# ParBLiSS/kmerind

Measured on AMD Instinct MI355X. Metric: kmers_per_sec_indexed, higher is better.
Workload: dtype u64

## Files before the change

### kmerind_amd/csrc/kmi_api.hip

```cpp
#include <stdlib.h>

#include <algorithm>

#include "kmi_block.h"
#include <chrono>
#include <mutex>

#include "kmi_internal.h"

namespace kmi {

namespace {
struct CachedBlock { int device; void *p; size_t bytes; };
std::mutex g_cache_mu;
std::vector<CachedBlock> g_cache;
constexpr size_t kCacheMaxBytes = 96ull << 30, kCacheMaxBlocks = 64, kCacheMinBlock = 1ull << 20;
inline uint64_t now_us() { return (uint64_t)std::chrono::duration_cast<std::chrono::microseconds>(std::chrono::steady_clock::now().time_since_epoch()).count(); }
size_t cache_flush(int device) {
  std::lock_guard<std::mutex> lk(g_cache_mu);
  size_t freed = 0;
  for (size_t i = 0; i < g_cache.size();) {
    if (device < 0 || g_cache[i].device == device) { (void)hipFree(g_cache[i].p); freed += g_cache[i].bytes; g_cache.erase(g_cache.begin() + (long)i); }
    else ++i;
  }
// ... 136 lines not shown
        for (int w = 0; w < NW; ++w) k[w] ^= r[w]; }
      const uint64_t h = kmer_hash<NW>(k, shape, which, true, farm_ndebug, ceil_log2_u32(nranks));
      out32[i] = (nranks & (nranks - 1u)) == 0u ? (uint32_t)h & (nranks - 1u) : (uint32_t)(h % nranks);
    }
  }
}

template <int NW, int BITS>
static kmi_status array_op_impl(kmi_ctx *ctx, const kmi_config *cfg, KShape shape, int op, uint32_t which, bool prefix,
                                uint32_t nranks, const uint64_t *in_dev, size_t n, uint64_t *out64, uint32_t *out32) {
  unsigned grid = (unsigned)std::min<size_t>((n + 255) / 256, 2048);
  if (grid == 0) return KMI_OK;
  ProfScope ps(ctx, "kmer_array_op", n);
  hipLaunchKernelGGL((kmer_array_op_kernel<NW, BITS>), dim3(grid), dim3(256), 0, ctx->stream, in_dev, (uint64_t)n, shape, op,
                     which, prefix, cfg->farm_ndebug != 0, cfg->strand, cfg->dist_trans, nranks, out64, out32);
  KMI_HIP(ctx, hipGetLastError());
  return KMI_OK;
}

static kmi_status array_op_dev(kmi_ctx *ctx, const kmi_config *cfg, int op, uint32_t which, bool prefix, uint32_t nranks,
                               const uint64_t *in_dev, size_t n, uint64_t *out64, uint32_t *out32) {
  KShape shape;
  if (!valid_config(cfg, &shape)) return set_err(ctx, KMI_ERR_INVALID, "bad kmi_config");
  KMI_DISPATCH(shape, array_op_impl, ctx, cfg, shape, op, which, prefix, nranks, in_dev, n, out64, out32);
}

static kmi_status array_op_host(kmi_ctx *ctx, const kmi_config *cfg, int op, uint32_t which, bool prefix, uint32_t nranks,
                                const uint64_t *in, size_t n, void *out) {
  if (!ctx) return KMI_ERR_INVALID;
  KShape shape;
  if (!valid_config(cfg, &shape)) return set_err(ctx, KMI_ERR_INVALID, "bad kmi_config");
  if (n == 0) return KMI_OK;
  if (!in || !out) return set_err(ctx, KMI_ERR_INVALID, "null buffer");
  if (op == OP_RANK && nranks == 0) return set_err(ctx, KMI_ERR_INVALID, "nranks must be > 0");
  KMI_HIP(ctx, hipSetDevice(ctx->device));
  const size_t in_bytes = n * shape.n_words * sizeof(uint64_t);
  const size_t out_bytes = (op == OP_RANK) ? n * sizeof(uint32_t) : (op == OP_HASH ? n * sizeof(uint64_t) : in_bytes);
  void *din, *dout;
  KMI_TRY(ws_get(ctx, WS_INPUT, in_bytes, &din));
  KMI_TRY(ws_get(ctx, WS_OUTPUT, out_bytes, &dout));
  KMI_HIP(ctx, hipMemcpyAsync(din, in, in_bytes, hipMemcpyHostToDevice, ctx->stream));
  KMI_TRY(array_op_dev(ctx, cfg, op, which, prefix, nranks, (const uint64_t *)din, n, (uint64_t *)dout, (uint32_t *)dout));
  KMI_HIP(ctx, hipMemcpyAsync(out, dout, out_bytes, hipMemcpyDeviceToHost, ctx->stream));
  KMI_HIP(ctx, hipStreamSynchronize(ctx->stream));
  return KMI_OK;
}

}

using namespace kmi;

extern "C" {

kmi_status kmi_ctx_create(int device, int rank, int nranks, void *stream, kmi_ctx **out) {
  if (!out || nranks <= 0 || rank < 0 || rank >= nranks) return KMI_ERR_INVALID;
  *out = nullptr;
  int ndev = 0;
  if (hipGetDeviceCount(&ndev) != hipSuccess || ndev <= 0 || device < 0 || device >= ndev) return KMI_ERR_DEVICE;
  if (hipSetDevice(device) != hipSuccess) return KMI_ERR_DEVICE;
  kmi_ctx *ctx = new kmi_ctx();
  if (const char *fp = getenv("KMI_FUSED_PATH")) ctx->fused_superkmer = strcmp(fp, "kmer") != 0;
  if (const char *dg = getenv("KMI_SK_DBG")) ctx->sk_dbg = atoi(dg);
  if (const char *dc = getenv("KMI_DIST_CHUNKS")) { ctx->dist_chunks = (uint32_t)atoi(dc); if (ctx->dist_chunks < 1) ctx->dist_chunks = 1; if (ctx->dist_chunks > 64) ctx->dist_chunks = 64; }
  if (const char *sl = getenv("KMI_SK_SLACK")) ctx->sk_slack = atoi(sl) != 0;
  if (const char *tp = getenv("KMI_TUPLES")) ctx->tuples_from_parse = strcmp(tp, "extract") != 0;
  if (const char *ps = getenv("KMI_DIST_POOL_SLACK")) ctx->dist_pool_slack = strtoull(ps, nullptr, 10);
  if (const char *pp = getenv("KMI_DIST_POOL_PCT")) { ctx->dist_pool_pct = (uint32_t)atoi(pp); if (ctx->dist_pool_pct < 1) ctx->dist_pool_pct = 1; }
  if (const char *fr = getenv("KMI_FRONT")) ctx->front_fused = strcmp(fr, "general") != 0;
  if (const char *ho = getenv("KMI_HOST_OVERLAP")) ctx->host_overlap = atoi(ho) != 0;
  if (const char *lp2 = getenv("KMI_LINES_P2")) ctx->lines_p2 = atoi(lp2) != 0;
  if (const char *ds = getenv("KMI_DBG_SUPERKMER")) ctx->dbg_superkmer = atoi(ds) != 0;
  if (const char *hm = getenv("KMI_HOST_OVERLAP_MIN")) ctx->host_overlap_min = strtoull(hm, nullptr, 10);
  if (const char *fc = getenv("KMI_FEED_MIN_CHUNK")) { ctx->feed_min_chunk = strtoull(fc, nullptr, 10); if (ctx->feed_min_chunk < 4096) ctx->feed_min_chunk = 4096; }
  if (const char *mr = getenv("KMI_FRONT_MIN_RANGE")) { ctx->front_min_range = strtoull(mr, nullptr, 10); ctx->front_min_range = (ctx->front_min_range + 4095) / 4096 * 4096; if (!ctx->front_min_range) ctx->front_min_range = 4096; }
  if (const char *rw = getenv("KMI_FRONT_RANGES_PER_WAVE")) { ctx->front_ranges_per_wave = (uint32_t)strtoul(rw, nullptr, 10); if (ctx->front_ranges_per_wave < 1) ctx->front_ranges_per_wave = 1; if (ctx->front_ranges_per_wave > 16) ctx->front_ranges_per_wave = 16; }
  if (const char *mw = getenv("KMI_FRONT_MAX_WAVES")) ctx->front_max_waves = (uint32_t)strtoul(mw, nullptr, 10);
  if (const char *sm = getenv("KMI_SPARSE_MIN")) ctx->sparse_min = strtoull(sm, nullptr, 10);
  if (const char *fd = getenv("KMI_FORCE_DIST")) ctx->force_dist = atoi(fd) != 0;
  if (const char *lc = getenv("KMI_LOOKUP_CAP")) { ctx->lookup_cap = (uint32_t)strtoul(lc, nullptr, 10); if (ctx->lookup_cap < 64) ctx->lookup_cap = 64; }
  if (const char *pb = getenv("KMI_PROFILE_BATCH")) { ctx->profile_batch = strtoull(pb, nullptr, 10); if (ctx->profile_batch < 4096) ctx->profile_batch = 4096; }
  ctx->device = device; ctx->rank = rank; ctx->nranks = nranks; ctx->stream = (hipStream_t)stream;
  if (hipMalloc((void **)&ctx->d_flags, sizeof(uint32_t) * kmi::FLAG_NUM_WORDS) != hipSuccess ||
      hipMalloc((void **)&ctx->d_totals, sizeof(uint64_t) * kmi::TOT_NUM_WORDS) != hipSuccess ||
      hipHostMalloc((void **)&ctx->h_totals, sizeof(uint64_t) * kmi::H_NUM_WORDS, hipHostMallocDefault)    != hipSuccess) {
    delete ctx;
    return KMI_ERR_DEVICE;
  }
  (void)hipMemset(ctx->d_flags, 0, sizeof(uint32_t) * kmi::FLAG_NUM_WORDS);
  {
    hipDeviceProp_t prop;
    if (hipGetDeviceProperties(&prop, device) == hipSuccess && prop.multiProcessorCount > 0) ctx->n_cus = (uint32_t)prop.multiProcessorCount;
  }
  if (upload_quality_lut(ctx) != KMI_OK) { kmi_ctx_destroy(ctx); return KMI_ERR_DEVICE; }
  (void)hipMemset(ctx->d_totals, 0, sizeof(uint64_t) * kmi::TOT_NUM_WORDS);
  *out = ctx;
  return KMI_OK;
}

kmi_status kmi_ctx_reset_hints(kmi_ctx *ctx) {
  if (!ctx) return KMI_ERR_INVALID;
  ctx->sk_level_hint = 0; ctx->sk_inv_dup = 0.f;
  return KMI_OK;
}

kmi_status kmi_ctx_debug_counter(const kmi_ctx *ctx, uint32_t which, uint64_t *value) {
  if (!ctx || !value) return KMI_ERR_INVALID;
  switch (which) {
    case 0: *value = ctx->dist_pool_regrows; return KMI_OK;
    case 1: *value = ctx->alloc_us; return KMI_OK;
    case 2: *value = ctx->alloc_bytes; return KMI_OK;
    case 3: *value = ctx->alloc_calls; return KMI_OK;
    case 4: *value = ctx->alloc_reused; return KMI_OK;
    case 5: *value = ctx->unitig_dist_rounds; return KMI_OK;
    case 6: *value = ctx->unitig_dist_exchanges; return KMI_OK;
    case 7: *value = ctx->unitig_dist_bytes; return KMI_OK;
    case 8: *value = ctx->lookup_npass; return KMI_OK;
    case 9: *value = ctx->retain_fullest; return KMI_OK;
    case 10: *value = ctx->setops_npass; return KMI_OK;
    case 11: *value = (uint64_t)kmi::kSegCopyTile; return KMI_OK;
    case 12: *value = ctx->qd_answered; return KMI_OK;
    case 13: *value = ctx->prune_dist_bytes; return KMI_OK;
    case 14: *value = ctx->tips_dist_exchanges; return KMI_OK;
    case 15: *value = ctx->tips_dist_bytes; return KMI_OK;
    case 16: *value = ctx->bubbles_dist_exchanges; return KMI_OK;
    case 17: *value = ctx->bubbles_dist_bytes; return KMI_OK;
    case 18: *value = ctx->bubbles_dist_stage_exchanges; return KMI_OK;
    case 19: *value = ctx->bubbles_dist_stage_bytes; return KMI_OK;
    default: return KMI_ERR_INVALID;
  }
}

kmi_status kmi_release_cached_memory(int device, uint64_t *bytes_released) {
  const size_t n = cache_flush(device);
  if (bytes_released) *bytes_released = n;
  return KMI_OK;
}

kmi_status kmi_ctx_destroy(kmi_ctx *ctx) {
  if (!ctx) return KMI_OK;
  (void)hipSetDevice(ctx->device);
  (void)hipStreamSynchronize(ctx->stream);
  for (int s = 0; s < WS_NUM_SLOTS; ++s) if (ctx->ws[s].p) dev_retire(ctx, ctx->ws[s].p, ctx->ws[s].cap);
  for (auto &b : ctx->spare) dev_retire(ctx, b.p, b.bytes);
  ctx->spare.clear();
  for (ProfRec &r : ctx->prof_pending) { (void)hipEventDestroy(r.e0); (void)hipEventDestroy(r.e1); }
  for (hipEvent_t e : ctx->event_pool) (void)hipEventDestroy(e);
  if (ctx->d_flags) (void)hipFree(ctx->d_flags);
  if (ctx->d_totals) (void)hipFree(ctx->d_totals);
  if (ctx->ev_mail) (void)hipEventDestroy(ctx->ev_mail);
  for (hipEvent_t e : ctx->feed_ev) if (e) (void)hipEventDestroy(e);
  if (ctx->copy_stream) (void)hipStreamDestroy(ctx->copy_stream);
  if (ctx->h_totals) (void)hipHostFree(ctx->h_totals);
  delete ctx;
  return KMI_OK;
}

const char *kmi_last_error(const kmi_ctx *ctx) { return ctx ? ctx->err.c_str() : "null context"; }

kmi_status kmi_ctx_set_fasta_partition(kmi_ctx *ctx, const kmi_fasta_partition *part) {
  if (!ctx) return KMI_ERR_INVALID;
  if (!part) { ctx->fa_part_set = false; return KMI_OK; }
  if (part->start_state > KMI_FA_SEQUENCE || part->index_shift > 1u) return set_err(ctx, KMI_ERR_INVALID, "bad kmi_fasta_partition");
  ctx->fa_part = *part;
  ctx->fa_part_set = true;
  return KMI_OK;
}

// ... 201 lines not shown
```

### kmerind_amd/csrc/kmi_front.h

```cpp
#pragma once
#include "kmi_front_bytes.h"

namespace kmi {

constexpr int kFrWaves = 4, kFrThreads = kFrWaves * kWave;
constexpr uint32_t kFrRing = 512;
constexpr uint32_t kFrStepLines = 128;
constexpr uint32_t kFrPendEnds = kFrRing - kFrStepLines - 2u, kFrPendPairs = kFrRing / 2u - kFrStepLines;
#ifndef KMI_FR_PASS_RECORDS
#define KMI_FR_PASS_RECORDS 64
#endif
constexpr uint32_t kFrPassRecords = KMI_FR_PASS_RECORDS;
#ifdef KMI_FR_PAIRS_ONLY
constexpr bool kFrEndsOnly = false;
#else
constexpr bool kFrEndsOnly = true;
#endif
constexpr uint32_t kFrRunQ = 256;
constexpr uint32_t kFrStep = 4096;
constexpr uint32_t kFrRowDw = 12;
constexpr uint32_t kFrNone = 0xffu;
constexpr uint32_t kFrOverrun = 256u << 10;

struct FrRange { uint32_t l0, n_lines, n_runs, n_items; };
// ... 569 lines not shown
      const uint4 *rp = reinterpret_cast<const uint4 *>(rows + run * kFrRowDw);
      const uint4 q0 = rp[0], q1 = rp[1], q2 = rp[2];
      uint32_t *row = s_row + threadIdx.x * kFrRowLds;
      row[0] = q0.x; row[1] = q0.y; row[2] = q0.z; row[3] = q0.w; row[4] = q1.x; row[5] = q1.y; row[6] = q1.z; row[7] = q1.w;
      row[8] = q2.x; row[9] = q2.y; row[10] = 0;
      if (edges) s_runx[threadIdx.x] = (uint8_t)q2.w;
      const uint32_t *src = g_items + (q * item_cap + (ri & 0x3ffffffu));
      uint32_t woff = 0;
#pragma unroll
      for (int v4 = 0; v4 < CAP / 4; ++v4) {
        if ((uint32_t)(4 * v4) < cnt) {
          const FrU4 v = *reinterpret_cast<const FrU4 *>(src + 4 * v4);
          const uint32_t it[4] = {v.x, v.y, v.z, v.w};
#pragma unroll
          for (int e = 0; e < 4; ++e)
            if ((uint32_t)(4 * v4 + e) < cnt) {
              const uint32_t n1 = it[e] & 31u, h27 = it[e] >> 5;
              s_items[pre + 4 * v4 + e] = woff | (n1 << 7) | ((h27 >> 7) << 12);
              s_xbits[pre + 4 * v4 + e] = (uint8_t)(h27 & 127u);
              atomicAdd(&s_cnt[h27 >> 19], 1u);
              woff += n1 + 1u;
            }
        }
      }
    }
    s_ibase[threadIdx.x] = pre;
    if (edges) {
      uint32_t wsum = 0;
      for (uint32_t j = 0; j < cnt; ++j) wsum += ((s_items[pre + j] >> 7) & 31u) + 1u;
      s_runw[threadIdx.x] = (uint8_t)wsum;
    }
    lds_barrier();
    uint32_t c = 0, inc = 0;
    if (bl) {
      c = s_cnt[threadIdx.x];
      s_cnt[threadIdx.x] = 0;
      inc = wave_inclusive_sum_dpp(c);
      if (lane_id() == kWave - 1) s_part[wave_id()] = inc;
    }
    lds_barrier();
    if (bl) {
      uint32_t wpre = 0;
#pragma unroll
      for (uint32_t w = 0; w < kNumCoarse / kWave; ++w) wpre += (w < wave_id()) ? s_part[w] : 0u;
      const uint32_t lo = wpre + inc - c;
      s_cur[threadIdx.x] = lo;
      s_gbase[threadIdx.x] = cursor - lo;
      cursor += c;
    }
    lds_barrier();
    for (uint32_t j = 0; j < cnt; ++j) {
      const uint32_t item = s_items[pre + j];
      s_stage[atomicAdd(&s_cur[item >> 24], 1u)] = (uint16_t)((threadIdx.x << 5) | j);
    }
    lds_barrier();
    const uint32_t n_items = pre + cnt;
    const uint32_t round_items = (uint32_t)__builtin_amdgcn_readfirstlane((int)s_cur[kNumCoarse - 1]);
    (void)n_items;
    for (uint32_t s = threadIdx.x; s < round_items; s += NT) {
      const uint32_t e = s_stage[s], rl = e >> 5, j = e & 31u;
      const uint32_t item = s_items[s_ibase[rl] + j];
      const uint32_t h27 = ((item >> 12) << 7) | (uint32_t)s_xbits[s_ibase[rl] + j], n1 = (item >> 7) & 31u;
      const uint32_t hs = ((h27 << lp) & 0x7ffffffu) >> 9;
      uint64_t w0, w1;
      bool flipped = false;
      sk_assemble_row<CANON>(s_row + rl * kFrRowLds, 2u * (item & 127u), k + n1, n1, hs, w0, w1, &flipped);
      if (edges) {
        const uint32_t *row = s_row + rl * kFrRowLds;
        const uint32_t wfirst = item & 127u, after = wfirst + n1 + k;
        auto cc = [&](uint32_t i) -> uint32_t { return (row[i >> 4] >> (2u * (i & 15u))) & 3u; };
        const uint32_t runx = s_runx[rl];
        const uint32_t lc = wfirst ? 1u + (3u - cc(wfirst - 1u)) : (runx & 7u);
        const uint32_t rc = wfirst + n1 + 1u < (uint32_t)s_runw[rl] ? 1u + (3u - cc(after)) : (runx >> 3);
        const uint32_t left = flipped ? (rc ? 5u - rc : 0u) : lc, right = flipped ? (lc ? 5u - lc : 0u) : rc;
        w1 |= ((uint64_t)(left | (right << 3)) << kRecEdgeShift) | ((uint64_t)(flipped ? 1u : 0u) << kRecFlipShift);
      }
      reinterpret_cast<ulonglong2 *>(out)[s_gbase[h27 >> 19] + s] = make_ulonglong2(w0, w1);
    }
    rb += n_taken;
    lds_barrier();
  }
}

__global__ __launch_bounds__(1024) void sk_front_verify_kernel(const FrRange *__restrict__ info, uint32_t n_ranges, uint32_t ranges_per_group,
                                                             uint64_t *__restrict__ group_runs ,
                                                             uint64_t *__restrict__ totals , uint32_t *__restrict__ flags) {
  __shared__ uint64_t s_scan[1024 / 64 + 2];
  __shared__ uint32_t s_bad;
  if (threadIdx.x == 0) s_bad = 0;
  lds_barrier();
  const uint32_t per = (n_ranges + 1023u) / 1024u;
  const uint32_t r_lo = threadIdx.x * per < n_ranges ? threadIdx.x * per : n_ranges, r_hi = r_lo + per < n_ranges ? r_lo + per : n_ranges;
  uint64_t my_lines = 0, my_runs = 0, my_its = 0;
  for (uint32_t r = r_lo; r < r_hi; ++r) {
    const FrRange fr = info[r];
    my_lines += fr.n_lines; my_runs += fr.n_runs; my_its += fr.n_items;
  }
  uint64_t carry = 0, runs = 0, its = 0;
  uint64_t before = block_exclusive_scan<uint64_t>(my_lines, s_scan, &carry);
  for (uint32_t r = r_lo; r < r_hi; ++r) {
    const FrRange fr = info[r];
    if (fr.l0 != kFrNone && fr.n_lines && ((uint32_t)before & 3u) != fr.l0) s_bad = 1;
    before += fr.n_lines;
  }
  (void)block_exclusive_scan<uint64_t>(my_runs, s_scan, &runs);
  (void)block_exclusive_scan<uint64_t>(my_its, s_scan, &its);
  lds_barrier();
  if (threadIdx.x == 0) {
    totals[0] = carry; totals[1] = runs; totals[2] = its;
    if (s_bad) atomicOr(&flags[FLAG_SK_DECLINED], 4u);
  }
  const uint32_t groups = (n_ranges + ranges_per_group - 1) / ranges_per_group;
  for (uint32_t g = threadIdx.x; g < groups; g += blockDim.x) {
    uint64_t s = 0;
    for (uint32_t r = g * ranges_per_group; r < (g + 1) * ranges_per_group && r < n_ranges; ++r) s += info[r].n_runs;
    group_runs[g] = s;
  }
}

}
```

### kmerind_amd/csrc/kmi_index.hip

```cpp
#include <stdlib.h>

#include <algorithm>

#include "kmi_extract.h"
#include "kmi_minimizer.h"
#include <type_traits>

namespace kmi {

constexpr int kFineBits = 15;
constexpr int kNumFine = 1 << kFineBits;
constexpr int kCoarseBits = 8;
constexpr int kNumCoarse = 1 << kCoarseBits;
constexpr int kSubPerCoarse = kNumFine / kNumCoarse;
constexpr int kSlotBits = 32 - kFineBits;
constexpr int kPartThreads = 1024;
constexpr int kPartGroups = 512;
constexpr int kFineParts = 2;
template <int NW> constexpr int fused_groups() { return kPartGroups; }
constexpr int kListGroups = 2048;
constexpr int kLoadBatch = 8;

__host__ __device__ inline uint32_t fine_of(uint32_t h) { return h >> kSlotBits; }
__host__ __device__ inline uint32_t coarse_of(uint32_t h) { return h >> (32 - kCoarseBits); }

template <int RW> struct PartCfg {
  static constexpr int TILE = (RW == 1) ? 8192 : (RW == 2 ? 4096 : (RW <= 4 ? 2048 : 1024));
  static constexpr int CTILE = (RW == 3) ? 3072 : TILE;
  static constexpr int PER_THREAD = TILE / kPartThreads;
};

enum BucketMode { BUCKET_COARSE = 0, BUCKET_SUB = 1, BUCKET_RANK = 2, BUCKET_REC = 3, BUCKET_REC_COARSE = 4 };

struct BucketFn {
  int mode; KShape shape; uint32_t dist_hash; bool farm_ndebug; uint32_t nranks;
  uint32_t sub;
  uint32_t dist_trans = 0;
  uint32_t layout_w = 0;
  uint64_t rank_magic = 0;
  uint32_t owner_w = 0;
};
inline uint64_t rank_magic_of(uint32_t nranks) { return nranks > 1u ? (uint64_t)(((unsigned __int128)1 << 64) / nranks) : 0ull; }
__host__ __device__ inline uint32_t rank_of_hash(uint64_t h, uint32_t nranks, uint64_t magic) {
  if ((nranks & (nranks - 1u)) == 0u) return (uint32_t)h & (nranks - 1u);
#if defined(__HIP_DEVICE_COMPILE__)
  const uint64_t q = __umul64hi(h, magic);
#else
  const uint64_t q = (uint64_t)(((unsigned __int128)h * magic) >> 64);
#endif
  uint64_t r = h - q * nranks;
  r = r >= nranks ? r - nranks : r;
  return (uint32_t)r;
}
inline uint32_t rank_sub_buckets(uint32_t nranks) { uint32_t s = 1; while (s * 2u * nranks <= (uint32_t)kNumCoarse) s *= 2u; return s; }

template <int NW> __device__ __forceinline__ uint32_t fine15_of_key(const uint64_t (&key)[NW], uint32_t layout_w, uint32_t k) {
  if constexpr (NW == 1) {
    if (layout_w) {
      const uint32_t lp = layout_w >> 8;
      return ((sk_key_bucket18(key[0], k, layout_w & 0xffu) << lp) & 0x3ffffu) >> 3;
    }
  }
  return fine_of(place_hash<NW>(key));
}

template <int NW> __device__ __forceinline__ uint32_t bucket_of(const uint64_t (&key)[NW], const BucketFn &f) {
  if (f.mode == BUCKET_RANK) {
    if constexpr (NW == 1) {
      if (f.owner_w) {
        const uint32_t h18 = sk_key_bucket18(key[0], f.shape.k, f.owner_w);
        const uint32_t lp = 31u - (uint32_t)__builtin_clz(f.nranks);
        return (h18 >> (18u - lp)) * f.sub + ((h18 >> 3) & (f.sub - 1u));
      }
    }
    uint64_t t[NW];
#pragma unroll
    for (int w = 0; w < NW; ++w) t[w] = key[w];
    if (f.dist_trans) {
      uint64_t rc[NW];
      if (f.shape.bits == 2) revcomp_words<NW, 2>(key, rc, f.shape); else revcomp_words<NW, 3>(key, rc, f.shape);
      const bool use_rc = f.dist_trans == KMI_DIST_LEX && less_words<NW>(rc, key);
#pragma unroll
      for (int w = 0; w < NW; ++w) t[w] = f.dist_trans == KMI_DIST_XOR ? (key[w] ^ rc[w]) : (use_rc ? rc[w] : key[w]);
    }
    const uint64_t h = kmer_hash<NW>(t, f.shape, f.dist_hash, true, f.farm_ndebug, ceil_log2_u32(f.nranks));
    const uint32_t spread = (uint32_t)((h >> 40) ^ (h >> 13)) * 0x9E3779B1u;
    const uint32_t rank = rank_of_hash(h, f.nranks, f.rank_magic);
    return rank * f.sub + ((spread >> 16) & (f.sub - 1u));
// ... 49 lines not shown
    for (int u = 0; u < U; ++u) {
      if (ok[u]) {
        uint64_t k[NW];
        if (transform) strand_key<NW, BITS>(raw[u], k, shape, strand);
        else {
#pragma unroll
          for (int w = 0; w < NW; ++w) k[w] = raw[u][w];
        }
        atomicAdd(&s_hist[fine15_of_key<NW>(k, layout_w, shape.k)], 1u);
      }
    }
  }
  lds_barrier();
  uint32_t *part_hist = fine_hist + (uint64_t)(blockIdx.x / (gridDim.x / kFineParts)) * kNumFine;
  for (int i = threadIdx.x; i < kNumFine; i += kPartThreads) {
    uint32_t v = s_hist[i];
    if (v) atomicAdd(&part_hist[i], v);
  }
  if (threadIdx.x < kNumCoarse) {
    uint32_t s = 0;
    for (int i = 0; i < kSubPerCoarse; ++i) s += s_hist[threadIdx.x * kSubPerCoarse + ((i + threadIdx.x) & (kSubPerCoarse - 1))];
    wg_hist[(uint64_t)blockIdx.x * kNumCoarse + threadIdx.x] = s;
  }
}

template <int NW, int BITS, int VW = 0>
__global__ __launch_bounds__(kPartThreads) void hist_rank_kernel(const uint64_t *__restrict__ keys, uint64_t n, KShape shape,
                                                                uint32_t strand, BucketFn fn, uint32_t *__restrict__ wg_hist,
                                                                uint32_t in_rw = NW + VW ) {
  __shared__ uint32_t s_hist[kNumCoarse];
  if (threadIdx.x < kNumCoarse) s_hist[threadIdx.x] = 0;
  lds_barrier();
  const uint64_t chunk = part_chunk(n, gridDim.x, PartCfg<NW + VW>::CTILE);
  const uint64_t b = (uint64_t)blockIdx.x * chunk;
  const uint64_t e = (b + chunk < n) ? b + chunk : n;
  for (uint64_t i = b + threadIdx.x; i < e; i += kPartThreads) {
    uint64_t raw[NW], k[NW];
#pragma unroll
    for (int w = 0; w < NW; ++w) raw[w] = keys[i * in_rw + w];
    strand_key<NW, BITS>(raw, k, shape, strand);
    atomicAdd(&s_hist[bucket_of<NW>(k, fn)], 1u);
  }
  lds_barrier();
  if (threadIdx.x < kNumCoarse) wg_hist[(uint64_t)blockIdx.x * kNumCoarse + threadIdx.x] = s_hist[threadIdx.x];
}

__global__ __launch_bounds__(kSubPerCoarse) void fine_totals_kernel(const uint32_t *__restrict__ fine_hist, uint64_t *__restrict__ coarse_tot) {
  __shared__ uint64_t s_scan[kSubPerCoarse / 64 + 2];
  const uint32_t f = blockIdx.x * kSubPerCoarse + threadIdx.x;
  uint64_t v = 0;
#pragma unroll
  for (int h = 0; h < kFineParts; ++h) v += fine_hist[(uint64_t)h * kNumFine + f];
  uint64_t total;
  (void)block_exclusive_scan<uint64_t>(v, s_scan, &total);
  if (threadIdx.x == 0) coarse_tot[blockIdx.x] = total;
}
__global__ __launch_bounds__(kSubPerCoarse) void fine_offsets_spread_kernel(const uint32_t *__restrict__ fine_hist, const uint64_t *__restrict__ coarse_tot,
                                                                           uint64_t *__restrict__ fine_off, uint64_t *__restrict__ part_off,
                                                                           uint64_t *__restrict__ coarse_base) {
  static_assert(kNumCoarse == 2 * kSubPerCoarse, "two coarse totals per thread");
  __shared__ uint64_t s_scan[kSubPerCoarse / 64 + 2];
  const uint32_t c = blockIdx.x, f = c * kSubPerCoarse + threadIdx.x;
  const uint32_t c0 = 2u * threadIdx.x;
  const uint64_t t0 = coarse_tot[c0], t1 = coarse_tot[c0 + 1];
  uint64_t grand;
  (void)block_exclusive_scan<uint64_t>(t0 + t1, s_scan, &grand);
  const uint64_t below = (c0 < c ? t0 : 0ull) + (c0 + 1 < c ? t1 : 0ull);
  uint64_t base;
  (void)block_exclusive_scan<uint64_t>(below, s_scan, &base);
  uint32_t loc[kFineParts];
  uint64_t v = 0;
#pragma unroll
  for (int h = 0; h < kFineParts; ++h) { loc[h] = fine_hist[(uint64_t)h * kNumFine + f]; v += loc[h]; }
  uint64_t off = base + block_exclusive_scan<uint64_t>(v, s_scan, (uint64_t *)nullptr);
  if (threadIdx.x == 0) coarse_base[c] = base;
  fine_off[f] = off;
#pragma unroll
  for (int h = 0; h < kFineParts; ++h) {
    if (part_off) part_off[(uint64_t)h * kNumFine + f] = off;
    off += loc[h];
  }
  if (c == (uint32_t)kNumCoarse - 1 && threadIdx.x == 0) fine_off[kNumFine] = grand;
}
static void launch_fine_offsets(kmi_ctx *ctx, const uint32_t *fine_hist, uint64_t *fine_off, uint64_t *part_off, uint64_t *coarse_base) {
  uint64_t *tot = ctx->d_totals + TOT_COARSE;
  hipLaunchKernelGGL(fine_totals_kernel, dim3(kNumCoarse), dim3(kSubPerCoarse), 0, ctx->stream, fine_hist, tot);
  hipLaunchKernelGGL(fine_offsets_spread_kernel, dim3(kNumCoarse), dim3(kSubPerCoarse), 0, ctx->stream, fine_hist, (const uint64_t *)tot, fine_off, part_off,
                     coarse_base);
}

__global__ __launch_bounds__(256) void coarse_cursors_kernel(const uint32_t *__restrict__ wg_hist, uint32_t groups,
                                                            const uint64_t *__restrict__ coarse_base, uint64_t *__restrict__ wg_off) {
  const uint32_t c = blockIdx.x * (blockDim.x >> 6) + wave_id();
  if (c >= (uint32_t)kNumCoarse) return;
  uint64_t carry = coarse_base[c];
  for (uint32_t w0 = 0; w0 < groups; w0 += kWave) {
    const uint32_t w = w0 + lane_id();
    const uint64_t v = (w < groups) ? wg_hist[(uint64_t)w * kNumCoarse + c] : 0ull;
    const uint64_t inc = wave_inclusive_scan(v);
    if (w < groups) wg_off[(uint64_t)w * kNumCoarse + c] = carry + inc - v;
    carry += __shfl(inc, kWave - 1, kWave);
  }
}

__global__ __launch_bounds__(256) void rank_totals_kernel(const uint32_t *__restrict__ wg_hist, uint32_t groups, uint32_t nbuckets,
                                                         uint64_t *__restrict__ bucket_cnt) {
  const uint32_t c = blockIdx.x * (blockDim.x >> 6) + wave_id();
  if (c >= nbuckets) return;
  uint64_t v = 0;
  for (uint32_t w = lane_id(); w < groups; w += kWave) v += wg_hist[(uint64_t)w * kNumCoarse + c];
  v = wave_reduce_sum(v);
  if (lane_id() == 0) bucket_cnt[c] = v;
}
__global__ __launch_bounds__(256) void rank_bases_kernel(const uint64_t *__restrict__ bucket_cnt, uint32_t nbuckets, uint64_t *__restrict__ base) {
  __shared__ uint64_t s_scan[256 / 64 + 2];
  const uint64_t tot = (threadIdx.x < nbuckets) ? bucket_cnt[threadIdx.x] : 0ull;
  uint64_t total;
  const uint64_t off = block_exclusive_scan<uint64_t>(tot, s_scan, &total);
  base[threadIdx.x] = off;
}
static void launch_rank_offsets(hipStream_t stream, const uint32_t *wg_hist, uint32_t groups, uint32_t nbuckets, uint64_t *bucket_cnt,
                                uint64_t *base , uint64_t *wg_off) {
  hipLaunchKernelGGL(rank_totals_kernel, dim3(kNumCoarse / 4), dim3(256), 0, stream, wg_hist, groups, nbuckets, bucket_cnt);
  hipLaunchKernelGGL(rank_bases_kernel, dim3(1), dim3(256), 0, stream, (const uint64_t *)bucket_cnt, nbuckets, base);
  hipLaunchKernelGGL(coarse_cursors_kernel, dim3(kNumCoarse / 4), dim3(256), 0, stream, wg_hist, groups, (const uint64_t *)base, wg_off);
}

template <int NW, int BITS, int VW = 0, int TILE_ = PartCfg<NW + VW>::TILE>
__device__ __forceinline__ void scatter_range(const uint64_t *__restrict__ in, uint64_t begin, uint64_t end, uint64_t *__restrict__ out,
                                              const KShape &shape, uint32_t strand, bool transform, const BucketFn &fn,
                                              uint64_t cursor ,
                                              uint64_t *s_stage, uint8_t *s_bkt, uint32_t *s_cnt, uint32_t *s_lofs,
                                              uint64_t *s_gbase, uint32_t *s_part, uint64_t *__restrict__ out_vals = nullptr,
                                              const float *__restrict__ in_q = nullptr, const uint64_t *__restrict__ in_v = nullptr) {
  constexpr int RW = NW + VW;
  constexpr int TILE = TILE_;
  constexpr int PT = TILE_ / kPartThreads;
  if (threadIdx.x < kNumCoarse) s_cnt[threadIdx.x] = 0;
  lds_barrier();
  uint64_t raw[PT][RW];
  auto load_tile = [&](uint64_t t0) {
#pragma unroll
    for (int j = 0; j < PT; ++j) {
      uint64_t i = t0 + (uint64_t)j * kPartThreads + threadIdx.x;
      i = (i < end) ? i : end - 1;
      if (VW > 0 && in_v) {
#pragma unroll
        for (int w = 0; w < NW; ++w) raw[j][w] = in[i * NW + w];
        raw[j][NW] = in_v[i];
        if (VW > 1) raw[j][RW - 1] = in_q ? (uint64_t)__float_as_uint(in_q[i]) : 0ull;
      } else if (VW > 0 && in_q) {
#pragma unroll
        for (int w = 0; w < RW - 1; ++w) raw[j][w] = in[i * (RW - 1) + w];
        raw[j][RW - 1] = (uint64_t)__float_as_uint(in_q[i]);
      } else {
#pragma unroll
        for (int w = 0; w < RW; ++w) raw[j][w] = in[i * RW + w];
      }
    }
  };
  load_tile(begin);
  for (uint64_t t0 = begin; t0 < end; t0 += TILE) {
    const uint32_t nt = (uint32_t)((end - t0 < (uint64_t)TILE) ? (end - t0) : (uint64_t)TILE);
    uint64_t k[PT][NW];
    uint64_t v[PT][VW ? VW : 1];
    uint32_t bk[PT], rk[PT];
#pragma unroll
    for (int j = 0; j < PT; ++j) {
      const uint32_t li = j * kPartThreads + threadIdx.x;
      bk[j] = 0xffffffffu;
      if (li < nt) {
        uint64_t kr[NW];
#pragma unroll
        for (int w = 0; w < NW; ++w) kr[w] = raw[j][w];
#pragma unroll
        for (int w = 0; w < VW; ++w) v[j][w] = raw[j][NW + w];
        if (transform) strand_key<NW, BITS>(kr, k[j], shape, strand);
        else {
#pragma unroll
          for (int w = 0; w < NW; ++w) k[j][w] = kr[w];
        }
        if (VW > 0 && fn.mode == BUCKET_REC) bk[j] = (uint32_t)(v[j][0] >> 46) & (uint32_t)(kSubPerCoarse - 1);
        else if (VW > 0 && fn.mode == BUCKET_REC_COARSE) bk[j] = (uint32_t)(v[j][0] >> 53) & (uint32_t)(kNumCoarse - 1);
        else bk[j] = bucket_of<NW>(k[j], fn);
        rk[j] = atomicAdd(&s_cnt[bk[j]], 1u);
      }
    }
    if (t0 + TILE < end) load_tile(t0 + TILE);
    lds_barrier();
    uint32_t c = 0, inc = 0;
    if (threadIdx.x < kNumCoarse) {
      c = s_cnt[threadIdx.x];
      s_cnt[threadIdx.x] = 0;
      inc = wave_inclusive_scan(c);
      if (lane_id() == kWave - 1) s_part[wave_id()] = inc;
    }
    lds_barrier();
    if (threadIdx.x < kNumCoarse) {
      uint32_t pre = 0;
#pragma unroll
      for (uint32_t w = 0; w < kNumCoarse / kWave; ++w) pre += (w < wave_id()) ? s_part[w] : 0u;
      const uint32_t lo = pre + inc - c;
      s_lofs[threadIdx.x] = lo;
      s_gbase[threadIdx.x] = cursor - lo;
      cursor += c;
    }
    lds_barrier();
#pragma unroll
// ... 1694 lines not shown
  const uint32_t b = blockIdx.x;
  const uint64_t nb = new_off[b], ne = new_off[b + 1];
  const uint64_t ob = old_off ? old_off[b] : 0ull, oe = old_off ? old_off[b + 1] : 0ull;
  if (nb == ne && ob == oe) { if (threadIdx.x == 0) out_cnt[b] = 0; return; }
  const uint64_t tmp0 = nb + ob;
  uint32_t *s_out = &s_ctl[4];
  uint32_t npass = 1;
  while (true) {
    if (threadIdx.x == 0) *s_out = 0;
    bool failed = false;
    for (uint32_t pass = 0; pass < npass && !failed; ++pass) {
      table_clear<NW>(tab);
      lds_barrier();
      for_each_key<NW, BatchOf<NW>::U>(old_keys, ob, oe, [&](const uint64_t (&k)[NW], uint64_t i) {
        const uint32_t h = place_hash<NW>(k);
        if (pass_of(h, npass) != pass) return;
        int s = table_upsert<NW>(tab, k, h);
        if (s >= 0) count_add(&tab.vals[s], old_vals[i], sat);
        else if (s == -2) count_add(tab.special, old_vals[i], sat);
      });
      for (uint64_t i = nb + threadIdx.x; i < ne; i += blockDim.x) {
        uint64_t k[NW];
#pragma unroll
        for (int w = 0; w < NW; ++w) k[w] = recs[i * RW + w];
        const uint32_t v = (uint32_t)recs[i * RW + NW];
        const uint32_t h = place_hash<NW>(k);
        if (pass_of(h, npass) != pass) continue;
        int s = table_upsert<NW>(tab, k, h);
        if (s >= 0) count_add(&tab.vals[s], v, sat);
        else if (s == -2) count_add(tab.special, v, sat);
      }
      lds_barrier();
      if (*tab.overflow) { failed = true; break; }
      for (int s = threadIdx.x; s < TabCfg<NW>::SLOTS; s += blockDim.x) {
        const bool used = slot_used<NW>(tab, s);
        const uint32_t pos = wave_alloc(s_out, used);
        if (used) {
#pragma unroll
          for (int w = 0; w < NW; ++w) tmp_keys[(tmp0 + pos) * NW + w] = tab.keys[(uint64_t)s * NW + w];
          tmp_vals[tmp0 + pos] = tab.vals[s];
        }
      }
      lds_barrier();
      if (NW == 1 && threadIdx.x == 0 && *tab.special_set) {
        const uint32_t pos = atomicAdd(s_out, 1u);
        tmp_keys[(tmp0 + pos) * NW] = kEmptyKey;
        tmp_vals[tmp0 + pos] = *tab.special;
      }
      lds_barrier();
    }
    if (!failed) break;
    npass *= 2;
    if (npass > kMaxPasses) { if (threadIdx.x == 0) { atomicOr(&flags[FLAG_PASS_LIMIT], 1u); *s_out = 0; } lds_barrier(); break; }
    lds_barrier();
  }
  if (threadIdx.x == 0) out_cnt[b] = *s_out;
}

template <int NW>
__global__ __launch_bounds__(256) void unzip_pairs_kernel(const uint64_t *__restrict__ recs, uint64_t n, uint64_t *__restrict__ keys,
                                                         uint32_t *__restrict__ vals) {
  constexpr int RW = NW + 1;
  for (uint64_t i = (uint64_t)blockIdx.x * blockDim.x + threadIdx.x; i < n; i += (uint64_t)gridDim.x * blockDim.x) {
#pragma unroll
    for (int w = 0; w < NW; ++w) keys[i * NW + w] = recs[i * RW + w];
    vals[i] = (uint32_t)recs[i * RW + NW];
  }
}

__global__ __launch_bounds__(1024) void bucket_offsets_kernel(const uint32_t *__restrict__ cnt, uint64_t *__restrict__ off,
                                                             uint64_t *__restrict__ totals, int slot) {
  __shared__ uint64_t s_scan[1024 / 64 + 2];
  constexpr int PER = kNumFine / 1024;
  uint64_t loc[PER], sum = 0;
#pragma unroll
  for (int i = 0; i < PER; ++i) { loc[i] = cnt[threadIdx.x * PER + i]; sum += loc[i]; }
  uint64_t total;
  uint64_t o = block_exclusive_scan<uint64_t>(sum, s_scan, &total);
#pragma unroll
  for (int i = 0; i < PER; ++i) { off[threadIdx.x * PER + i] = o; o += loc[i]; }
  if (threadIdx.x == 0) { off[kNumFine] = total; totals[slot] = total; }
}

template <int NW, typename V>
__global__ __launch_bounds__(256) void bucket_compact_kernel(const uint64_t *__restrict__ tmp_keys, const V *__restrict__ tmp_vals,
                                                            const uint64_t *__restrict__ src_off_a, const uint64_t *__restrict__ src_off_b,
                                                            const uint64_t *__restrict__ dst_off, uint64_t *__restrict__ keys,
                                                            V *__restrict__ vals) {
  const uint32_t b = blockIdx.x;
  const uint64_t d0 = dst_off[b], n = dst_off[b + 1] - d0;
  const uint64_t s0 = src_off_a[b] + (src_off_b ? src_off_b[b] : 0ull);
  for (uint64_t i = threadIdx.x; i < n * NW; i += blockDim.x) keys[d0 * NW + i] = tmp_keys[s0 * NW + i];
  for (uint64_t i = threadIdx.x; i < n; i += blockDim.x) vals[d0 + i] = tmp_vals[s0 + i];
}

enum QueryMode { Q_COUNT = 0, Q_FIND = 1, Q_ERASE = 2, Q_HITS = 3  };

template <int NW, int VW>
__global__ __launch_bounds__((QTabCfg<NW>::NT)) void bucket_query_kernel(int mode, const uint64_t *__restrict__ q_keys, const uint64_t *__restrict__ q_off,
                                                                       const uint64_t *__restrict__ idx_keys, const uint32_t *__restrict__ idx_vals32,
                                                                       const uint64_t *__restrict__ idx_mvals,
                                                                       const uint64_t *__restrict__ idx_off, uint64_t *__restrict__ tmp_keys,
                                                                       uint64_t *__restrict__ tmp_vals64, uint32_t *__restrict__ tmp_vals32,
                                                                       uint32_t *__restrict__ out_cnt, uint32_t *__restrict__ flags,
                                                                       bool emit_index, const uint32_t *__restrict__ idx_cnt = nullptr,
                                                                       const uint64_t *__restrict__ out_off = nullptr) {
  KMI_TABLE_LDS_CFG(NW, QTabCfg<NW>)
  constexpr int OW = VW ? VW : 1;
  const uint32_t b = blockIdx.x;
  const uint64_t qb = q_off[b], qe = q_off[b + 1];
  const uint64_t ib = idx_off ? idx_off[b] : 0ull, ie = idx_off ? (idx_cnt ? ib + idx_cnt[b] : idx_off[b + 1]) : 0ull;
  const bool by_entries = (mode == Q_ERASE) || (VW > 0 && mode == Q_FIND);
  const uint64_t tmp0 = out_off ? out_off[b] : (by_entries ? ib : qb);
  uint32_t *s_out = &s_ctl[4];
  auto emit_entry = [&](uint32_t pos, const uint64_t (&k)[NW], uint64_t i) {
#pragma unroll
    for (int w = 0; w < NW; ++w) tmp_keys[(tmp0 + pos) * NW + w] = k[w];
    if constexpr (VW == 0) {
      if (mode == Q_ERASE) tmp_vals32[tmp0 + pos] = idx_vals32[i]; else tmp_vals64[tmp0 + pos] = emit_index ? i : (uint64_t)idx_vals32[i];
    } else {
#pragma unroll
      for (int w = 0; w < VW; ++w) tmp_vals64[(tmp0 + pos) * VW + w] = idx_mvals[i * VW + w];
    }
  };
  {
    uint32_t want = 2u * (uint32_t)((qe - qb) < (uint64_t)QTabCfg<NW>::CAP ? (qe - qb) : (uint64_t)QTabCfg<NW>::CAP);
    want = (want + 255u) & ~255u;
    want = want < 512u ? 512u : want;
    if (want < (uint32_t)QTabCfg<NW>::CAP) { tab.cap = want; tab.slots = want + QTabCfg<NW>::PAD; tab.limit = want * 3u / 4u; }
  }
  if (qb == qe) {
    if (mode == Q_ERASE) {
      for (uint64_t i = ib + threadIdx.x; i < ie; i += blockDim.x) {
        uint64_t k[NW];
#pragma unroll
        for (int w = 0; w < NW; ++w) k[w] = idx_keys[i * NW + w];
        emit_entry((uint32_t)(i - ib), k, i);
      }
      if (threadIdx.x == 0) out_cnt[b] = (uint32_t)(ie - ib);
    } else if (threadIdx.x == 0) out_cnt[b] = 0;
    return;
  }
  uint32_t npass = 1;
  while (true) {
    if (threadIdx.x == 0) *s_out = 0;
    bool failed = false;
    for (uint32_t pass = 0; pass < npass && !failed; ++pass) {
      table_clear<NW>(tab);
      lds_barrier();
      for_each_key<NW, BatchOf<NW>::U>(q_keys, qb, qe, [&](const uint64_t (&k)[NW], uint64_t) {
        const uint32_t h = place_hash<NW>(k);
        if (pass_of(h, npass) != pass) return;
        (void)table_upsert<NW>(tab, k, h);
      });
      lds_barrier();
      if (*tab.overflow) { failed = true; break; }
      for (uint64_t i = ib + threadIdx.x; i < ie; i += blockDim.x) {
        uint64_t k[NW];
#pragma unroll
        for (int w = 0; w < NW; ++w) k[w] = idx_keys[i * NW + w];
        const uint32_t h = place_hash<NW>(k);
        if (pass_of(h, npass) != pass) continue;
        const int s = table_find<NW>(tab, k, h);
        const bool hit = (s >= 0) || (s == -2);
        if (mode == Q_COUNT) {
          if (s >= 0) atomicAdd(&tab.vals[s], 1u); else if (s == -2) atomicAdd(tab.special, 1u);
// ... 122 lines not shown
  uint64_t *part_off;
  uint64_t *coarse_base;
  uint32_t *wg_hist;
  uint64_t *wg_off;
};

static kmi_status get_part_ws(kmi_ctx *ctx, size_t n, int nw, WsSlot slot_a, WsSlot slot_b, PartWs *w) {
  void *p;
  const size_t key_bytes = (n ? n : 1) * nw * sizeof(uint64_t);
  KMI_TRY(ws_get(ctx, slot_a, key_bytes, &p)); w->buf_a = (uint64_t *)p;
  KMI_TRY(ws_get(ctx, slot_b, key_bytes, &p)); w->buf_b = (uint64_t *)p;
  KMI_TRY(ws_get(ctx, WS_HIST, sizeof(uint32_t) * kNumFine * kFineParts + sizeof(uint64_t) * ((kNumFine + 1) * 2 + kNumFine * kFineParts + kNumCoarse) + 256, &p));
  w->fine_hist = (uint32_t *)p;
  uint64_t *off_base = (uint64_t *)((char *)p + sizeof(uint32_t) * kNumFine * kFineParts);
  w->fine_off = off_base + (slot_b == WS_QUERY_B ? (kNumFine + 1) : 0);
  w->part_off = off_base + 2 * (kNumFine + 1);
  w->coarse_base = w->part_off + (uint64_t)kNumFine * kFineParts;
  KMI_TRY(ws_get(ctx, WS_WGHIST, sizeof(uint32_t) * kPartGroups * kNumCoarse, &p)); w->wg_hist = (uint32_t *)p;
  KMI_TRY(ws_get(ctx, WS_CURSOR, sizeof(uint64_t) * kPartGroups * kNumCoarse, &p)); w->wg_off = (uint64_t *)p;
  return KMI_OK;
}

template <int NW, int BITS, int VW = 0>
static kmi_status partition_impl(kmi_ctx *ctx, const kmi_config *cfg, KShape shape, const uint64_t *keys_dev, size_t n, bool transform,
                                 WsSlot slot_a, WsSlot slot_b, Partitioned *out, uint32_t layout_w = 0, uint64_t *split_keys = nullptr,
                                 uint64_t *split_vals = nullptr, const float *in_q = nullptr, const uint64_t *in_v = nullptr) {
  PartWs w;
  KMI_TRY(get_part_ws(ctx, n, NW + VW, slot_a, slot_b, &w));
  KMI_HIP(ctx, hipMemsetAsync(w.fine_hist, 0, sizeof(uint32_t) * kNumFine * kFineParts, ctx->stream));
  {
    ProfScope ps(ctx, "hist_fine", n);
    hipLaunchKernelGGL((hist_fine_kernel<NW, BITS, VW>), dim3(kPartGroups), dim3(kPartThreads), 0, ctx->stream, keys_dev, (uint64_t)n, shape,
                       cfg->strand, transform, w.fine_hist, w.wg_hist, layout_w,
                       (VW > 0 && in_v) ? (uint32_t)NW : (uint32_t)(NW + VW) - ((VW > 0 && in_q) ? 1u : 0u));
  }
  {
    ProfScope ps(ctx, "fine_offsets", kNumFine);
    launch_fine_offsets(ctx, w.fine_hist, w.fine_off, w.part_off, w.coarse_base);
    hipLaunchKernelGGL(coarse_cursors_kernel, dim3(kNumCoarse / 4), dim3(256), 0, ctx->stream, (const uint32_t *)w.wg_hist, (uint32_t)kPartGroups,
                       (const uint64_t *)w.coarse_base, w.wg_off);
  }
  BucketFn fn; fn.mode = BUCKET_COARSE; fn.shape = shape; fn.dist_hash = 0; fn.farm_ndebug = false; fn.nranks = 1; fn.sub = 1; fn.layout_w = layout_w;
  {
    ProfScope ps(ctx, "scatter_coarse", n);
    hipLaunchKernelGGL((scatter_chunks_kernel<NW, BITS, VW>), dim3(kPartGroups), dim3(kPartThreads), 0, ctx->stream, keys_dev, (uint64_t)n, w.buf_a,
                       shape, cfg->strand, transform, fn, w.wg_off, (VW > 0) ? in_q : (const float *)nullptr,
                       (VW > 0) ? in_v : (const uint64_t *)nullptr);
  }
  {
    ProfScope ps(ctx, "scatter_fine", n);
    if (NW == 1 && VW == 0)
      hipLaunchKernelGGL(scatter_fine_lines_kernel, dim3(kNumCoarse * kFineParts), dim3(kPartThreads), 0, ctx->stream, (const uint64_t *)w.buf_a,
                         w.buf_b, (const uint64_t *)w.fine_off, (const uint64_t *)w.part_off, (const uint64_t *)w.wg_off, (uint32_t)kPartGroups,
                         layout_w, shape.k);
    else if (NW + VW <= 4 && ctx->lines_p2)
      hipLaunchKernelGGL((scatter_fine_records_lines_kernel<NW, BITS, VW>), dim3(kNumCoarse * kFineParts), dim3(kPartThreads), 0, ctx->stream,
                         (const uint64_t *)w.buf_a, (VW > 0 && split_keys) ? split_keys : w.buf_b, shape, (const uint64_t *)w.fine_off,
                         (const uint64_t *)w.part_off, (const uint64_t *)w.wg_off, (uint32_t)kPartGroups, layout_w,
                         (VW > 0 && split_keys) ? split_vals : (uint64_t *)nullptr);
    else
      hipLaunchKernelGGL((scatter_fine_kernel<NW, BITS, VW>), dim3(kNumCoarse * kFineParts), dim3(kPartThreads), 0, ctx->stream, w.buf_a,
                         (VW > 0 && split_keys) ? split_keys : w.buf_b, shape, (const uint64_t *)w.fine_off, (const uint64_t *)w.part_off,
                         (const uint64_t *)w.wg_off, (uint32_t)kPartGroups, (int)BUCKET_SUB, layout_w, (VW > 0 && split_keys) ? split_vals : (uint64_t *)nullptr);
  }
  KMI_HIP(ctx, hipGetLastError());
  out->keys = (VW > 0 && split_keys) ? split_keys : w.buf_b; out->fine_off = w.fine_off;
  out->scratch = (NW == 1 && VW == 0) ? w.buf_a : nullptr;
  return KMI_OK;
}

static kmi_status read_total(kmi_ctx *ctx, TotalWord slot, uint64_t *v) {
  uint32_t flag = 0;
  KMI_HIP(ctx, hipMemcpyAsync(ctx->h_totals + slot, ctx->d_totals + slot, sizeof(uint64_t), hipMemcpyDeviceToHost, ctx->stream));
  KMI_HIP(ctx, hipMemcpyAsync(&flag, ctx->d_flags + FLAG_PASS_LIMIT, sizeof(uint32_t), hipMemcpyDeviceToHost, ctx->stream));
  KMI_HIP(ctx, hipStreamSynchronize(ctx->stream));
  *v = ctx->h_totals[slot];
  if (flag) {
    KMI_HIP(ctx, hipMemsetAsync(ctx->d_flags + FLAG_PASS_LIMIT, 0, sizeof(uint32_t), ctx->stream));
    return set_err(ctx, KMI_ERR_OVERFLOW, "a bucket could not be reduced within the pass limit");
  }
  return KMI_OK;
}

template <int NW>
static kmi_status adopt_tmp(kmi_index *idx, const uint64_t *tmp_keys, const uint32_t *tmp_vals, const uint64_t *src_a, const uint64_t *src_b,
                            const uint32_t *out_cnt, bool fastq_verdict = false, uint64_t n_slots = 0, bool allow_sparse = false) {
  kmi_ctx *ctx = idx->ctx;
  uint64_t *new_off = nullptr;
  KMI_HIP(ctx, pool_alloc(ctx, (void **)&new_off, kOffBytes));
  {
    ProfScope ps(ctx, "bucket_offsets", kNumFine);
    hipLaunchKernelGGL(bucket_offsets_kernel, dim3(1), dim3(1024), 0, ctx->stream, out_cnt, new_off, ctx->d_totals, (int)TOT_ENTRIES);
  }
  uint64_t total = 0;
  kmi_status st_total = read_total(ctx, TOT_ENTRIES, &total);
  if (st_total == KMI_OK && fastq_verdict) st_total = fastq_length_verdict(ctx);
  if (st_total != KMI_OK) { pool_free(ctx, new_off, kOffBytes); return st_total; }
  if (n_slots && total == n_slots && !src_b && ctx->ws[WS_TMP_KEYS].p == (const void *)tmp_keys && ctx->ws[WS_TMP_VALS].p == (const void *)tmp_vals) {
    size_t kb0 = 0, vb0 = 0;
    (void)ws_detach(ctx, WS_TMP_KEYS, tmp_keys, &kb0);
    (void)ws_detach(ctx, WS_TMP_VALS, tmp_vals, &vb0);
    KMI_HIP(ctx, hipStreamSynchronize(ctx->stream));
    free_index_arrays(idx);
    idx->keys = const_cast<uint64_t *>(tmp_keys); idx->vals = const_cast<uint32_t *>(tmp_vals); idx->bucket_off = new_off;
    idx->n_entries = total; idx->has_data = true; idx->keys_bytes = kb0; idx->vals_bytes = vb0;
    return KMI_OK;
  }
  bool room = false;
  if (NW == 1 && allow_sparse && n_slots >= ctx->sparse_min) {
    size_t free_b = 0, total_b = 0;
    room = hipMemGetInfo(&free_b, &total_b) == hipSuccess && free_b >= ctx->ws[WS_TMP_KEYS].cap + ctx->ws[WS_TMP_VALS].cap + ((size_t)1 << 30);
  }
  if (NW == 1 && allow_sparse && room && n_slots >= ctx->sparse_min && !src_b && ctx->ws[WS_TMP_KEYS].p == (const void *)tmp_keys &&
      ctx->ws[WS_TMP_VALS].p == (const void *)tmp_vals) {
    uint64_t *off = nullptr; uint32_t *cnt = nullptr;
    hipError_t e1 = pool_alloc(ctx, (void **)&off, kOffBytes);
    hipError_t e2 = pool_alloc(ctx, (void **)&cnt, sizeof(uint32_t) * kNumFine);
    if (e1 == hipSuccess && e2 == hipSuccess) {
      KMI_HIP(ctx, hipMemcpyAsync(off, src_a, kOffBytes, hipMemcpyDeviceToDevice, ctx->stream));
      KMI_HIP(ctx, hipMemcpyAsync(cnt, out_cnt, sizeof(uint32_t) * kNumFine, hipMemcpyDeviceToDevice, ctx->stream));
      size_t kb0 = 0, vb0 = 0;
      (void)ws_detach(ctx, WS_TMP_KEYS, tmp_keys, &kb0);
      (void)ws_detach(ctx, WS_TMP_VALS, tmp_vals, &vb0);
      free_index_arrays(idx);
      idx->keys = const_cast<uint64_t *>(tmp_keys); idx->vals = const_cast<uint32_t *>(tmp_vals); idx->bucket_off = off; idx->bucket_cnt = cnt;
      idx->dense_off = new_off; idx->n_entries = total; idx->has_data = true; idx->keys_bytes = kb0; idx->vals_bytes = vb0;
      return KMI_OK;
    }
    if (off) pool_free(ctx, off, kOffBytes);
    if (cnt) pool_free(ctx, cnt, sizeof(uint32_t) * kNumFine);
  }
  uint64_t *nk = nullptr; uint32_t *nv = nullptr;
  const size_t kb = (total ? total : 1) * NW * sizeof(uint64_t), vb = (total ? total : 1) * sizeof(uint32_t);
  hipError_t e1 = pool_alloc(ctx, (void **)&nk, kb);
  hipError_t e2 = pool_alloc(ctx, (void **)&nv, vb);
  if (e1 != hipSuccess || e2 != hipSuccess) {
    if (nk) pool_free(ctx, nk, kb);
    if (nv) pool_free(ctx, nv, vb);
    pool_free(ctx, new_off, kOffBytes);
    return set_err(ctx, KMI_ERR_NOMEM, "hipMalloc failed for the index arrays");
  }
  {
    ProfScope ps(ctx, "bucket_compact", total);
    hipLaunchKernelGGL((bucket_compact_kernel<NW, uint32_t>), dim3(kNumFine), dim3(256), 0, ctx->stream, tmp_keys, tmp_vals, src_a, src_b,
                       (const uint64_t *)new_off, nk, nv);
  }
  KMI_HIP(ctx, hipGetLastError());
  KMI_HIP(ctx, hipStreamSynchronize(ctx->stream));
  free_index_arrays(idx);
  idx->keys = nk; idx->vals = nv; idx->bucket_off = new_off; idx->n_entries = total; idx->has_data = true;
  idx->keys_bytes = kb; idx->vals_bytes = vb;
  return KMI_OK;
}

template <int NW>
static kmi_status reduce_and_adopt(kmi_index *idx, const Partitioned &part, size_t n, bool fastq_verdict = false) {
  kmi_ctx *ctx = idx->ctx;
  void *p;
  const uint64_t cap = n + idx->n_entries;
  KMI_TRY(ws_get(ctx, WS_TMP_KEYS, cap * NW * sizeof(uint64_t), &p)); uint64_t *tmp_keys = (uint64_t *)p;
  KMI_TRY(ws_get(ctx, WS_TMP_VALS, cap * sizeof(uint32_t), &p)); uint32_t *tmp_vals = (uint32_t *)p;
  KMI_TRY(ws_get(ctx, WS_BUCKET_CNT, sizeof(uint32_t) * kNumFine, &p)); uint32_t *out_cnt = (uint32_t *)p;
  KMI_HIP(ctx, hipMemsetAsync(ctx->d_flags + FLAG_REDUCE_CHECK, 0, sizeof(uint32_t), ctx->stream));
  {
    ProfScope ps(ctx, "bucket_reduce", n);
    hipLaunchKernelGGL((bucket_reduce_kernel<NW>), dim3(kNumFine), dim3(TabCfg<NW>::NT), 0, ctx->stream, (const uint64_t *)part.keys,
                       (const uint64_t *)part.fine_off, (const uint64_t *)idx->keys, (const uint32_t *)idx->vals,
                       (const uint64_t *)(idx->has_data ? idx->bucket_off : nullptr), tmp_keys, tmp_vals, out_cnt, ctx->d_flags,
                       idx->shape.n_bits == 64u * NW, part.scratch, idx->saturating);
  }
  KMI_HIP(ctx, hipGetLastError());
  return adopt_tmp<NW>(idx, tmp_keys, tmp_vals, part.fine_off, idx->has_data ? idx->bucket_off : nullptr, out_cnt, fastq_verdict,
                       idx->has_data ? 0 : (uint64_t)n);
}

template <int NW, int BITS>
static kmi_status insert_impl(kmi_index *idx, const uint64_t *keys_dev, size_t n, bool transform) {
  kmi_ctx *ctx = idx->ctx;
  if (n == 0) return KMI_OK;
  KMI_TRY(ensure_layout(idx, 0u));
  Partitioned part;
  KMI_TRY((partition_impl<NW, BITS>(ctx, &idx->cfg, idx->shape, keys_dev, n, transform, WS_KEYS_A, WS_KEYS_B, &part)));
  return reduce_and_adopt<NW>(idx, part, n);
}

template <int NW, int BITS>
static kmi_status build_fused_impl(kmi_index *idx, const uint8_t *bytes_dev, size_t n_bytes) {
  kmi_ctx *ctx = idx->ctx;
  KMI_TRY(ensure_layout(idx, 0u));
  FastqScan sc;
  KMI_TRY(fastq_scan(ctx, &idx->cfg, bytes_dev, n_bytes, &sc, false));
  const uint64_t n = sc.n_tuples, n_tiles = sc.n_tiles;
  if (n == 0) return KMI_OK;
  PackedInput in; in.eol = sc.pk_eol; in.stream = sc.pk_stream; in.n_bytes = sc.n_bytes; in.n_cover = sc.n_cover; in.n_valid = sc.n_bytes; in.brk = sc.pk_brk;
  const bool split = sc.pk_brk != nullptr;
  const uint32_t *line_base = sc.line_base;
  const bool canonical = idx->cfg.strand != KMI_STRAND_SINGLE;
  PartWs w;
  KMI_TRY(get_part_ws(ctx, n, NW, WS_KEYS_A, WS_KEYS_B, &w));
  void *pl;
  using LPC = ListPassCfg<NW, BITS>;
  KMI_TRY(ws_get(ctx, WS_ENT_LIST, sizeof(uint16_t) * ((size_t)n_tiles * LPC::ent_stride(idx->shape.k, split) + 64), &pl));
  uint16_t *ent = (uint16_t *)pl;
  KMI_TRY(ws_get(ctx, WS_ENT_CNT, sizeof(uint32_t) * (n_tiles + 8), &pl));
  uint32_t *ent_cnt = (uint32_t *)pl;
  KMI_HIP(ctx, hipMemsetAsync(w.fine_hist, 0, sizeof(uint32_t) * kNumFine * kFineParts, ctx->stream));
  {
    ProfScope ps(ctx, "fastq_list", n);
    using LP = ListPassCfg<NW, BITS>;
    const uint32_t wave_lds = LP::wave_lds_bytes(idx->shape.k, split);
    hipLaunchKernelGGL((fastq_list_kernel<NW, BITS>), dim3(kListGroups), dim3(kListThreads), wave_lds * (kListThreads / kWave), ctx->stream, in,
                       n_tiles, idx->shape.k, LP::max_runs(idx->shape.k, split), wave_lds, line_base, ctx->d_flags, ent, ent_cnt,
                       LP::ent_stride(idx->shape.k, split));
  }
// ... 1399 lines not shown
```

### kmerind_amd/csrc/kmi_internal.h

```cpp
#pragma once
#include <hip/hip_runtime.h>
#include <stdint.h>
#include <stdio.h>
#include <string.h>

#include <string>
#include <vector>

#include "../../include/kmerind_hip.h"
#include "kmi_device.h"

namespace kmi {

constexpr int kSegCopyThreads = 256, kSegCopyPerThread = 8, kSegCopyTile = kSegCopyThreads * kSegCopyPerThread;

enum WsSlot {
  WS_TILE_INFO = 0,
  WS_TILE_BASE,
  WS_TILE_OFF,
  WS_KEYS_A,
  WS_KEYS_B,
  WS_HIST,
  WS_WGHIST,
  WS_CURSOR,
// ... 35 lines not shown
  WS_UNI_RANK,
  WS_UNI_NODE,
  WS_UNI_SCAN,
  WS_UNI_STAGE,
  WS_UNI_END,
  WS_UNI_CNT,
  WS_DBG_TIPS,
  WS_DBG_BUBBLES,
  WS_LOOKUP_RECS,
  WS_LOOKUP_CNT,
  WS_SPECTRUM,
  WS_LOCATE_POS,
  WS_LOCATE_SCAN,
  WS_LOCATE_OFF,
  WS_QD_PERM,
  WS_QD_SLOT,
  WS_QD_ANS,
  WS_QD_OFFS,
  WS_QD_VALS,
  WS_QD_RANS,
  WS_QD_ROFFS,
  WS_QD_RVALS,
  WS_NUM_SLOTS
};

enum FlagWord : uint32_t {
  FLAG_PARSE = 0,
  FLAG_OUT_OVERFLOW = 1,
  FLAG_PASS_LIMIT = 2,
  FLAG_ID_OVERFLOW = 3,
  FLAG_REDUCE_CHECK = 8,
  FLAG_SK_DECLINED = 9,
  FLAG_SK_WHY = 10,
  FLAG_FRONT_QUEUE = 12,
  FLAG_SK_LEVEL0 = 16,
  FLAG_SK_LEVEL_END = 34,
  FLAG_SK_ROOM = 34,
  FLAG_LOOKUP_NPASS = 36,
  FLAG_LOOKUP_OVER = 37,
  FLAG_REDUCE_QUEUE = 40,
  FLAG_REDUCE_QUEUE_END = 48,
  FLAG_CLOCKS = 48,
  FLAG_NUM_WORDS = 64,
  FZ_SCAN_0 = 0, FZ_SCAN_1 = 16, FZ_FRONT_0 = 0, FZ_FRONT_1 = 16, FZ_BACK_0 = 16, FZ_BACK_1 = 35, FZ_BACK_2 = 40, FZ_BACK_3 = 48
};
static_assert(FZ_SCAN_0 == FZ_FRONT_0 && FZ_SCAN_1 == FZ_FRONT_1 && FLAG_REDUCE_CHECK < FZ_SCAN_1,
              "a scan and the one-pass front end clear the same per-call words, and nothing of the back end or the lookup (below)");
static_assert(FZ_FRONT_0 <= FLAG_PARSE && FLAG_SK_DECLINED < FZ_FRONT_1 && FLAG_SK_WHY < FZ_FRONT_1 && FLAG_FRONT_QUEUE < FZ_FRONT_1,
              "the front end's launch clears the parse flags, its verdict words and its range queue");
static_assert(FZ_FRONT_1 <= FLAG_SK_LEVEL0, "... and none of the back end's words");
static_assert(FZ_BACK_0 == FLAG_SK_LEVEL0 && FZ_BACK_1 == FLAG_SK_ROOM + 1 && FLAG_SK_LEVEL_END == FLAG_SK_ROOM,
              "the back end's first range: the level votes and the room flag, nothing else");
static_assert(FZ_BACK_1 <= FLAG_LOOKUP_NPASS && FLAG_LOOKUP_OVER == FLAG_LOOKUP_NPASS + 1 && FLAG_LOOKUP_OVER < FZ_BACK_2,
              "the lookup's two words lie together (one fill, one read-back) and outside both ranges");
static_assert(FZ_BACK_2 == FLAG_REDUCE_QUEUE && FZ_BACK_3 == FLAG_REDUCE_QUEUE_END && FLAG_REDUCE_QUEUE_END <= FLAG_CLOCKS,
              "the back end's second range: the queue word and its spare words, not the clocks");
static_assert(FLAG_SK_LEVEL0 + 9 <= FLAG_SK_LEVEL_END && FLAG_CLOCKS + 16 <= FLAG_NUM_WORDS, "the votes and the clocks fit");

enum TotalWord : uint32_t {
  TOT_LINES = 0,
  TOT_FA_CHARS = 0,
  TOT_TUPLES = 1,
  TOT_FA_DROPPED = 1,
  TOT_SEQS = 2,
  TOT_FA_VALID = 3,
  TOT_SCAN_WORDS = 4,
  TOT_ENTRIES = 4,
  TOT_RESULTS = 5,
  TOT_SK_KMERS = 6,
  TOT_UPDATED = 7,
  TOT_BATCH_END = 8,
  TOT_LOCATE_HITS = 9,
  TOT_FRONT = 12,
  TOT_COARSE = 16,
  TOT_NUM_WORDS = 16 + 256
};
static_assert(TOT_FA_VALID + 1 == TOT_SCAN_WORDS && TOT_SCAN_WORDS == TOT_ENTRIES && TOT_ENTRIES + 1 == TOT_RESULTS &&
              TOT_RESULTS + 1 == TOT_SK_KMERS && TOT_SK_KMERS + 1 == TOT_UPDATED && TOT_UPDATED + 1 == TOT_BATCH_END &&
              TOT_BATCH_END + 1 == TOT_LOCATE_HITS && TOT_LOCATE_HITS < TOT_FRONT && TOT_FRONT + 3 <= TOT_COARSE && TOT_COARSE + 256 == TOT_NUM_WORDS,
              "one owner per total word");
enum HostWord : uint32_t {
  H_BATCH_END = 8,
  H_SK_LEVELS = 8,
  H_SK_ROOM = 14,
  H_MAIL = 16,
  H_MAIL_CNT = H_MAIL,
  H_MAIL_DECLINED = H_MAIL + 512,
  H_MAIL_FRONT = H_MAIL + 513,
  H_MAIL_KMERS = H_MAIL + 516,
  H_NUM_WORDS = 16 + 1024
};
static_assert(H_BATCH_END == (uint32_t)TOT_BATCH_END && H_SK_LEVELS > (uint32_t)TOT_RESULTS && H_SK_LEVELS + 5 <= H_SK_ROOM &&
              H_SK_ROOM < H_MAIL && H_MAIL == (uint32_t)TOT_COARSE && H_MAIL_KMERS < H_NUM_WORDS,
              "the read-backs of a build overlap neither each other nor the mirrored totals a build reads (entries, results)");

struct ProfRec {
  const char *name;
  hipEvent_t e0, e1;
  uint64_t units;
};

struct ProfAgg {
  const char *name;
  double total_ms;
  uint64_t launches, units;
};

}

struct kmi_ctx {
  int device = 0, rank = 0, nranks = 1;
  hipStream_t stream = nullptr;
  std::string err;
  struct Buf { void *p = nullptr; size_t cap = 0; } ws[kmi::WS_NUM_SLOTS];
  uint32_t *d_flags = nullptr;
  uint32_t n_cus = 0;
  uint64_t *d_totals = nullptr;
  hipEvent_t ev_mail = nullptr;
  const uint8_t *feed_host = nullptr; uint8_t *feed_dev = nullptr; size_t feed_bytes = 0;
  hipStream_t copy_stream = nullptr;
  hipEvent_t feed_ev[17] = {};
  bool edge_records = false;
  bool dbg_superkmer = true;
  struct { const uint64_t *recs = nullptr, *rec_off = nullptr, *region = nullptr; const uint32_t *cap = nullptr, *cnt = nullptr; bool valid = false; } sk_left;
  bool lines_p2 = true;
  bool host_overlap = true;
  size_t host_overlap_min = (size_t)64 << 20;
  size_t feed_min_chunk = (size_t)8 << 20;
  uint64_t *h_totals = nullptr;
  bool prof = false;
  std::vector<kmi::ProfRec> prof_pending;
  std::vector<kmi::ProfAgg> prof_agg;
  std::vector<hipEvent_t> event_pool;
  struct Spare { void *p; size_t bytes; };
  std::vector<Spare> spare;
  bool fused_superkmer = true;
  bool force_dist = false;
  uint32_t sk_level_hint = 0;
  float sk_inv_dup = 0.f;
  uint64_t alloc_us = 0, alloc_bytes = 0, alloc_calls = 0, alloc_reused = 0;
  uint32_t dist_pool_regrows = 0;
  uint64_t unitig_dist_rounds = 0, unitig_dist_exchanges = 0, unitig_dist_bytes = 0;
  uint32_t dist_pool_pct = 100;
  uint64_t dist_pool_slack = 65536;
  uint32_t dist_chunks = 4;
  bool tuples_from_parse = true;
  bool sk_slack = true;
  bool front_fused = true;
  uint32_t front_waves = 0;
  uint64_t front_min_range = 64ull << 10;
  uint32_t front_ranges_per_wave = 4;
  uint32_t front_max_waves = 0;
  uint64_t sparse_min = 1ull << 26;
  int sk_dbg = 0;
  bool fa_part_set = false;
  kmi_fasta_partition fa_part{};
  uint32_t lookup_cap = 0;
  size_t profile_batch = (size_t)256 << 20;
  uint64_t lookup_npass = 0;
  uint64_t bubbles_dist_exchanges = 0, bubbles_dist_bytes = 0;
  uint64_t bubbles_dist_stage_exchanges = 0, bubbles_dist_stage_bytes = 0;
  uint64_t tips_dist_exchanges = 0, tips_dist_bytes = 0;
  uint64_t prune_dist_bytes = 0;
  uint64_t retain_fullest = 0;
  uint64_t setops_npass = 0;
  uint64_t qd_answered = 0;
  int fa_left_carry = -1;
};

namespace kmi {

hipError_t dev_malloc(kmi_ctx *ctx, void **p, size_t bytes, size_t *got = nullptr);
void dev_free(kmi_ctx *ctx, void *p);
void dev_retire(kmi_ctx *ctx, void *p, size_t bytes);

inline hipError_t pool_alloc(kmi_ctx *ctx, void **p, size_t bytes) {
  if (bytes == 0) bytes = 256;
  for (size_t i = 0; i < ctx->spare.size(); ++i)
    if (ctx->spare[i].bytes == bytes) { *p = ctx->spare[i].p; ctx->spare.erase(ctx->spare.begin() + (long)i); return hipSuccess; }
  hipError_t e = dev_malloc(ctx, p, bytes);
  if (e != hipSuccess && !ctx->spare.empty()) {
    for (auto &b : ctx->spare) dev_free(ctx, b.p);
    ctx->spare.clear();
    e = dev_malloc(ctx, p, bytes);
  }
  return e;
}
inline void pool_free(kmi_ctx *ctx, void *p, size_t bytes) {
  if (!p) return;
  if (bytes == 0) bytes = 256;
  constexpr size_t kMaxSpare = 12;
  if (ctx->spare.size() >= kMaxSpare) {
    size_t m = 0;
    for (size_t i = 1; i < ctx->spare.size(); ++i) if (ctx->spare[i].bytes < ctx->spare[m].bytes) m = i;
    if (ctx->spare[m].bytes >= bytes) { dev_free(ctx, p); return; }
    dev_free(ctx, ctx->spare[m].p);
    ctx->spare.erase(ctx->spare.begin() + (long)m);
  }
  ctx->spare.push_back({p, bytes});
  constexpr size_t kMaxSpareBytes = 32ull << 30;
  size_t total = 0;
  for (const auto &b : ctx->spare) total += b.bytes;
  while (total > kMaxSpareBytes && !ctx->spare.empty()) {
    total -= ctx->spare.front().bytes;
    dev_free(ctx, ctx->spare.front().p);
    ctx->spare.erase(ctx->spare.begin());
  }
}

inline kmi_status set_err(kmi_ctx *ctx, kmi_status st, const char *fmt, const char *a = "", const char *b = "") {
  if (ctx) {
    char buf[512];
// ... 141 lines not shown
```

### kmerind_amd/csrc/kmi_sk_build.h

```cpp
#pragma once

namespace kmi {

template <typename Fn>
static kmi_status sk_dispatch_w(uint32_t w, Fn &&fn) {
  switch (w) {
    case 19: return fn(std::integral_constant<int, 19>{});
    case 13: return fn(std::integral_constant<int, 13>{});
    case 11: return fn(std::integral_constant<int, 11>{});
    default: return fn(std::integral_constant<int, 7>{});
  }
}

enum SkInput { SK_ANY_FORMAT, SK_FASTQ, SK_FASTQ_ONE_PASS };
static uint32_t sk_width_of_shape(const KShape &s) { return (s.n_words == 1 && s.bits == 2) ? sk_window_of(s.k) : 0u; }
static uint32_t sk_width(const kmi_index *idx, SkInput in) {
  const kmi_ctx *ctx = idx->ctx;
  if (idx->val_words != 0 || !ctx->fused_superkmer) return 0u;
  if (in != SK_ANY_FORMAT && idx->cfg.seq_format != KMI_FMT_FASTQ) return 0u;
  if (in == SK_FASTQ_ONE_PASS && !ctx->front_fused) return 0u;
  return sk_width_of_shape(idx->shape);
}
static uint32_t sk_width_of(const kmi_index *idx) { return sk_width(idx, SK_FASTQ); }
static uint32_t preferred_layout(const kmi_index *idx) { return sk_width(idx, SK_ANY_FORMAT); }
static bool sk_rank_count(uint32_t p) { return p == 1u || p == 2u || p == 4u || p == 8u; }

struct SkGroupWs {
  uint32_t *wg_hist;
  uint64_t *wg_off;
  uint64_t *cnt, *base, *cend;
};
static kmi_status sk_group_ws(kmi_ctx *ctx, SkGroupWs *g) {
  void *p;
  KMI_TRY(ws_get(ctx, WS_WGHIST, sizeof(uint32_t) * kPartGroups * kNumCoarse, &p)); g->wg_hist = (uint32_t *)p;
  KMI_TRY(ws_get(ctx, WS_CURSOR, sizeof(uint64_t) * kPartGroups * kNumCoarse, &p)); g->wg_off = (uint64_t *)p;
  KMI_TRY(ws_get(ctx, WS_MISC, sizeof(uint64_t) * kNumCoarse * 3, &p)); g->cnt = (uint64_t *)p; g->base = g->cnt + kNumCoarse; g->cend = g->base + kNumCoarse;
  return KMI_OK;
}

struct SkFront {
  bool ok = false;
  uint64_t *recs = nullptr;
  uint64_t n_records = 0, n_kmers = 0, n_seqs = 0;
  uint64_t h_cnt[kNumCoarse], h_base[kNumCoarse];
  uint64_t *wg_off = nullptr;
};

template <int W>
static kmi_status sk_front_end(kmi_ctx *ctx, const kmi_config *cfg, const KShape &shape, const FastqScan &sc, uint32_t lp, SkFront *f,
                               uint64_t *out = nullptr, size_t out_cap = 0 ,
                               const FastaScan *fa = nullptr ) {
  constexpr int NW = 1, BITS = 2;
  f->ok = false;
  uint64_t n = fa ? 0 : sc.n_tuples;
  const uint64_t n_tiles = fa ? (fa->n_chars + 8191) / 8192 : sc.n_tiles;
  const uint32_t k = shape.k;
  PackedInput in;
  if (fa) { in.eol = fa->pk_break; in.stream = fa->pk_stream; in.n_bytes = fa->n_chars; in.n_cover = fa->n_cover; in.n_valid = fa->n_valid; in.brk = nullptr; }
  else { in.eol = sc.pk_eol; in.stream = sc.pk_stream; in.n_bytes = sc.n_bytes; in.n_cover = sc.n_cover; in.n_valid = sc.n_bytes; in.brk = sc.pk_brk; }
  const bool split = !fa && sc.pk_brk != nullptr;
  const bool canonical = cfg->strand != KMI_STRAND_SINGLE;
  using LP = ListPassCfg<NW, BITS>;
  const uint32_t seg = sk_segment_of((uint32_t)W), ipt = sk_items_per_tile((uint32_t)W) * (fa ? 2u : 1u);
  const uint32_t stride = fa ? 8192u / seg + 72u : LP::run_stride(k, seg, split);
  void *p;
  KMI_TRY(ws_get(ctx, WS_ENT_LIST, sizeof(uint32_t) * ((size_t)n_tiles * stride + 64), &p)); uint32_t *ent = (uint32_t *)p;
  KMI_TRY(ws_get(ctx, WS_ENT_CNT, sizeof(uint32_t) * (n_tiles + 8), &p)); uint32_t *ent_cnt = (uint32_t *)p;
  KMI_TRY(ws_get(ctx, WS_ENT_BKT, sizeof(uint32_t) * ((size_t)n_tiles * stride + 64), &p)); uint32_t *run_items = (uint32_t *)p;
  KMI_TRY(ws_get(ctx, WS_SK_ITEMS, sizeof(uint32_t) * ((size_t)n_tiles * ipt + 64), &p)); uint32_t *items = (uint32_t *)p;
  SkGroupWs g;
  KMI_TRY(sk_group_ws(ctx, &g));
  KMI_HIP(ctx, hipMemsetAsync(ctx->d_flags + FLAG_SK_DECLINED, 0, sizeof(uint32_t), ctx->stream));
  if (fa) {
    ProfScope ps(ctx, "fasta_runs", fa->n_chars);
    KMI_HIP(ctx, hipMemsetAsync(ctx->d_totals + TOT_SK_KMERS, 0, sizeof(uint64_t), ctx->stream));
    hipLaunchKernelGGL(fasta_runs_kernel, dim3(2048), dim3(256), 0, ctx->stream, reinterpret_cast<const uint32_t *>(fa->pk_break), fa->n_chars, fa->n_valid,
                       fa->n_cover, n_tiles, k, seg, ent, ent_cnt, stride, (unsigned long long *)(ctx->d_totals + TOT_SK_KMERS), ctx->d_flags);
  } else {
    ProfScope ps(ctx, "fastq_list", n);
    const uint32_t wave_lds = LP::wave_lds_bytes(k, split);
    hipLaunchKernelGGL((fastq_list_kernel<NW, BITS, true>), dim3(kListGroups), dim3(kListThreads), wave_lds * (kListThreads / kWave), ctx->stream, in,
                       n_tiles, k, LP::max_runs(k, split), wave_lds, sc.line_base, ctx->d_flags, (void *)ent, ent_cnt, stride, seg);
  }
  {
    ProfScope ps(ctx, "sk_minimizer", n);
    hipLaunchKernelGGL((sk_minimizer_kernel<W>), dim3(kPartGroups), dim3(kSkThreads), 0, ctx->stream, in, n_tiles, k, (const uint32_t *)ent,
                       (const uint32_t *)ent_cnt, stride, ipt, items, run_items, g.wg_hist, ctx->d_flags);
  }
  {
    ProfScope ps(ctx, "sk_offsets", kNumCoarse);
    launch_rank_offsets(ctx->stream, (const uint32_t *)g.wg_hist, (uint32_t)kPartGroups, (uint32_t)kNumCoarse, g.cnt, g.base, g.wg_off);
  }
  KMI_HIP(ctx, hipGetLastError());
  uint64_t h_cnt[2 * kNumCoarse];
  uint32_t h_flags[FLAG_SK_DECLINED + 1] = {0};
  KMI_HIP(ctx, hipMemcpyAsync(h_cnt, g.cnt, sizeof(uint64_t) * 2 * kNumCoarse, hipMemcpyDeviceToHost, ctx->stream));
  KMI_HIP(ctx, hipMemcpyAsync(h_flags, ctx->d_flags, sizeof(h_flags), hipMemcpyDeviceToHost, ctx->stream));
  if (fa) KMI_HIP(ctx, hipMemcpyAsync(&n, ctx->d_totals + TOT_SK_KMERS, sizeof(uint64_t), hipMemcpyDeviceToHost, ctx->stream));
  KMI_HIP(ctx, hipStreamSynchronize(ctx->stream));
  if (!fa && (h_flags[FLAG_PARSE] & 4u)) return fastq_length_verdict(ctx);
  const uint32_t h_flag = h_flags[FLAG_SK_DECLINED];
  if (h_flag) return KMI_OK;
  uint64_t R = 0;
  for (int c = 0; c < kNumCoarse; ++c) { R += h_cnt[c]; f->h_cnt[c] = h_cnt[c]; f->h_base[c] = h_cnt[kNumCoarse + c]; }
  uint64_t *rec_a = out;
  if (!out || R + 64 > out_cap) { KMI_TRY(ws_get(ctx, WS_KEYS_A, (R + 64) * 16, &p)); rec_a = (uint64_t *)p; }
  {
    ProfScope ps(ctx, "sk_scatter", n);
#define KMI_SK_SCATTER(CANON)                                                                                                          \
    hipLaunchKernelGGL(sk_scatter_kernel<CANON>, dim3(kPartGroups), dim3(kSkThreads), 0, ctx->stream, in, n_tiles, k, (const uint32_t *)ent, \
                       (const uint32_t *)ent_cnt, stride, ipt, (const uint32_t *)items, (const uint32_t *)run_items, (const uint64_t *)g.wg_off, rec_a, lp)
    if (canonical) KMI_SK_SCATTER(true); else KMI_SK_SCATTER(false);
#undef KMI_SK_SCATTER
  }
  KMI_HIP(ctx, hipGetLastError());
  f->ok = true; f->recs = rec_a; f->n_records = R; f->n_kmers = n; f->wg_off = g.wg_off;
  return KMI_OK;
}

static kmi_status feed_flush(kmi_ctx *ctx) {
  if (!ctx->feed_host) return KMI_OK;
  const uint8_t *h = ctx->feed_host;
  ctx->feed_host = nullptr;
  KMI_HIP(ctx, hipMemcpyAsync(ctx->feed_dev, h, ctx->feed_bytes, hipMemcpyHostToDevice, ctx->stream));
  return KMI_OK;
}

static void sk_front_report_clocks(kmi_ctx *ctx) {
#ifdef KMI_FR_TIMING
  unsigned long long t[8];
  hipStreamSynchronize(ctx->stream);
  hipMemcpy(t, ctx->d_flags + FLAG_CLOCKS, sizeof(t), hipMemcpyDeviceToHost);
  fprintf(stderr, "sk_front wave clocks: wait-bytes %llu  eol %llu  lines %llu  load+pack %llu  walk %llu  final %llu  copy-out %llu  rest %llu\n", t[0], t[1], t[2], t[3], t[4], t[5], t[6], t[7]);
  hipMemset(ctx->d_flags + FLAG_CLOCKS, 0, sizeof(t));
#endif
}
static void sk_front_report_leave(kmi_ctx *ctx, bool fed, uint32_t front_launched_waves) {
#ifdef KMI_FR_LEAVE
  hipStreamSynchronize(ctx->stream);
  if (fed) return;
  const uint32_t nw = std::min<uint32_t>(front_launched_waves, kFrTimingWaves);
  std::vector<unsigned long long> wc(2 * (size_t)nw);
  hipMemcpyFromSymbol(wc.data(), HIP_SYMBOL(g_fr_wave_clock), sizeof(unsigned long long) * wc.size());
  unsigned long long first = ~0ull;
  for (uint32_t i = 0; i < nw; ++i) first = std::min(first, wc[2 * i]);
  std::vector<double> leave(nw);
  double by_simd[kFrWaves] = {0}, by_third[3] = {0}, enter_third[3] = {0}; uint32_t n_third[3] = {0};
  for (uint32_t i = 0; i < nw; ++i) {
    leave[i] = (double)(wc[2 * i + 1] - first) * 0.01;
    by_simd[i % kFrWaves] += leave[i] / (nw / kFrWaves);
    const uint32_t th = (uint32_t)((uint64_t)i * 3u / nw);
    by_third[th] += leave[i]; enter_third[th] += (double)(wc[2 * i] - first) * 0.01; ++n_third[th];
  }
  std::vector<double> so(leave);
  std::sort(so.begin(), so.end());
  double mean = 0; for (double v : so) mean += v / nw;
  fprintf(stderr, "sk_front wavefronts leave (us after the first entry): n %u  min %.1f  median %.1f  mean %.1f  max %.1f  | by SIMD %.1f %.1f %.1f %.1f"
                  "  | by workgroup third: leave %.1f %.1f %.1f  enter %.1f %.1f %.1f\n", nw, so[0], so[nw / 2], mean, so[nw - 1], by_simd[0], by_simd[1],
          by_simd[2], by_simd[3], by_third[0] / n_third[0], by_third[1] / n_third[1], by_third[2] / n_third[2], enter_third[0] / n_third[0],
          enter_third[1] / n_third[1], enter_third[2] / n_third[2]);
#endif
}
static void sk_front_report_decline(kmi_ctx *ctx) {
  if (!getenv("KMI_FRONT_DEBUG")) return;
  uint32_t why = 0;
  (void)hipMemcpy(&why, ctx->d_flags + FLAG_SK_WHY, sizeof(why), hipMemcpyDeviceToHost);
  fprintf(stderr, "sk_front declined: reasons 0x%x (2 first byte, 4 crowded lines, 8 inference, 16 marker / length, 32 run queue, 64 run capacity, 128 items per run, 256 item capacity, 512 / 1024 edge records: a read of several runs / a base that is not A C G T; 0 = the chain of line indices)\n", why);
}

template <int W>
static kmi_status sk_front_fast(kmi_ctx *ctx, const kmi_config *cfg, const KShape &shape, const uint8_t *bytes_dev, size_t n_bytes, uint32_t lp, SkFront *f,
                                bool *took, uint64_t *out = nullptr, size_t out_cap = 0) {
  *took = false;
  f->ok = false;
  const bool fed = ctx->feed_host != nullptr && bytes_dev == ctx->feed_dev && n_bytes == ctx->feed_bytes;
  if (!fed) KMI_TRY(feed_flush(ctx));
  if (!ctx->front_fused || cfg->seq_format != KMI_FMT_FASTQ || cfg->seq_filter != KMI_SEQ_ALL || n_bytes < 64) return feed_flush(ctx);
  const uint32_t k = shape.k;
  const bool canonical = cfg->strand != KMI_STRAND_SINGLE;
  if (!ctx->front_waves) {
    int per_cu = 0;
    if (hipOccupancyMaxActiveBlocksPerMultiprocessor(&per_cu, sk_front_kernel<19, false>, kFrThreads, 0) != hipSuccess || per_cu <= 0) per_cu = 2;
    ctx->front_waves = (uint32_t)per_cu * (ctx->n_cus ? ctx->n_cus : 256u) * (uint32_t)kFrWaves;
  }
  const uint32_t per_wave = fed ? 16u : ctx->front_ranges_per_wave;
  uint64_t range_bytes = (n_bytes + (uint64_t)ctx->front_waves * per_wave - 1) / ((uint64_t)ctx->front_waves * per_wave);
  range_bytes = (range_bytes + kFrStep - 1) / kFrStep * kFrStep;
  if (range_bytes < ctx->front_min_range) range_bytes = ctx->front_min_range;
  if (range_bytes > (8ull << 20)) range_bytes = 8ull << 20;
  const uint64_t n_ranges64 = (n_bytes + range_bytes - 1) / range_bytes;
  const uint32_t rpg = (uint32_t)((n_ranges64 + kPartGroups - 1) / kPartGroups);
  if (rpg > kFrMaxGroupRanges) return feed_flush(ctx);
  const uint32_t n_ranges = (uint32_t)n_ranges64;
  const uint32_t run_cap = (uint32_t)(range_bytes / 64) + 64u, item_cap = (uint32_t)(range_bytes / 8) + 64u;
  void *p;
  KMI_TRY(ws_get(ctx, WS_TILE_INFO, sizeof(FrRange) * (n_ranges + 1), &p)); FrRange *info = (FrRange *)p;
  KMI_TRY(ws_get(ctx, WS_TILE_BASE, sizeof(uint64_t) * (kPartGroups + 1), &p)); uint64_t *group_runs = (uint64_t *)p;
  KMI_TRY(ws_get(ctx, WS_ENT_LIST, sizeof(uint32_t) * ((size_t)n_ranges * run_cap + 64), &p)); uint32_t *run_items = (uint32_t *)p;
  KMI_TRY(ws_get(ctx, WS_PK_STREAM, sizeof(uint32_t) * kFrRowDw * ((size_t)n_ranges * run_cap + 64), &p)); uint32_t *rows = (uint32_t *)p;
  KMI_TRY(ws_get(ctx, WS_SK_ITEMS, sizeof(uint32_t) * ((size_t)n_ranges * item_cap + 64), &p)); uint32_t *items = (uint32_t *)p;
  SkGroupWs g;
  KMI_TRY(sk_group_ws(ctx, &g));
  hipLaunchKernelGGL(sk_zero_kernel, dim3(128), dim3(1024), 0, ctx->stream, g.wg_hist, (uint32_t)(kPartGroups * kNumCoarse),
                     reinterpret_cast<uint32_t *>(ctx->d_totals + TOT_SK_KMERS), 2u, (uint32_t *)nullptr, 0u, ctx->d_flags, (uint32_t)FZ_FRONT_0,
                     (uint32_t)FZ_FRONT_1, 0u, 0u);
  auto launch_front = [&](uint32_t wgs, uint32_t r0, uint32_t r1, uint32_t *queue) {
#define KMI_SK_FRONT(EDGES)                                                                                                            \
    hipLaunchKernelGGL((sk_front_kernel<W, EDGES>), dim3(wgs), dim3(kFrThreads), 0, ctx->stream, bytes_dev, (uint64_t)n_bytes, range_bytes, n_ranges, k, \
                       is_rna(cfg), run_cap, item_cap, rpg, info, run_items, rows, items, g.wg_hist, (unsigned long long *)(ctx->d_totals + TOT_SK_KMERS),  \
                       ctx->d_flags, r0, r1, queue)
    if (ctx->edge_records) KMI_SK_FRONT(true); else KMI_SK_FRONT(false);
#undef KMI_SK_FRONT
  };
  uint32_t front_launched_waves = 0;
  if (!fed) {
    ProfScope ps(ctx, "sk_front", n_bytes);
    uint32_t waves = ctx->front_max_waves ? std::min(ctx->front_waves, ctx->front_max_waves) : ctx->front_waves;
    waves = std::max<uint32_t>((uint32_t)kFrWaves, waves / (uint32_t)kFrWaves * (uint32_t)kFrWaves);
    const uint32_t wgs = std::min((n_ranges + kFrWaves - 1) / kFrWaves, waves / (uint32_t)kFrWaves);
    front_launched_waves = wgs * (uint32_t)kFrWaves;
    launch_front(wgs, 0u, 0xffffffffu, ctx->d_flags + FLAG_FRONT_QUEUE);
  } else {
    ProfScope ps(ctx, "sk_front_fed", n_bytes);
    const uint8_t *host = ctx->feed_host;
    ctx->feed_host = nullptr;
    constexpr size_t kMaxChunks = sizeof(ctx->feed_ev) / sizeof(ctx->feed_ev[0]) - 1;
    size_t cut[kMaxChunks + 1];
    size_t n_chunks = 0;
    {
      size_t ratio = 16;
      if (const char *e = getenv("KMI_FEED_RATIO")) { const long v = atol(e); if (v >= 2 && v <= 64) ratio = (size_t)v; }
      size_t at = 0;
      cut[0] = 0;
      while (n_chunks + 1 < kMaxChunks && n_bytes - at > ctx->feed_min_chunk) {
        size_t len = (n_bytes - at) - (n_bytes - at) / ratio;
        len = len / 4096 * 4096;
        at += len; cut[++n_chunks] = at;
      }
      cut[++n_chunks] = n_bytes;
    }
    if (!ctx->copy_stream) KMI_HIP(ctx, hipStreamCreateWithFlags(&ctx->copy_stream, hipStreamNonBlocking));
    for (size_t c = 0; c <= n_chunks; ++c) if (!ctx->feed_ev[c]) KMI_HIP(ctx, hipEventCreateWithFlags(&ctx->feed_ev[c], hipEventDisableTiming));
    KMI_HIP(ctx, hipEventRecord(ctx->feed_ev[n_chunks], ctx->stream));
    KMI_HIP(ctx, hipStreamWaitEvent(ctx->copy_stream, ctx->feed_ev[n_chunks], 0));
    for (size_t c = 0; c < n_chunks; ++c) {
      KMI_HIP(ctx, hipMemcpyAsync(const_cast<uint8_t *>(bytes_dev) + cut[c], host + cut[c], cut[c + 1] - cut[c], hipMemcpyHostToDevice, ctx->copy_stream));
      KMI_HIP(ctx, hipEventRecord(ctx->feed_ev[c], ctx->copy_stream));
    }
    const uint64_t margin = (uint64_t)kFrOverrun + 3ull * kFrStep;
    uint32_t r_done = 0;
    for (size_t c = 0; c < n_chunks; ++c) {
      KMI_HIP(ctx, hipStreamWaitEvent(ctx->stream, ctx->feed_ev[c], 0));
      const uint64_t arrived = cut[c + 1];
      uint32_t r_end = n_ranges;
      if (c + 1 < n_chunks) r_end = arrived > margin + range_bytes ? (uint32_t)((arrived - margin) / range_bytes) : 0u;
      if (r_end > n_ranges) r_end = n_ranges;
      if (r_end <= r_done) continue;
      launch_front((r_end - r_done + kFrWaves - 1) / kFrWaves, r_done, r_end, nullptr);
      r_done = r_end;
    }
  }
  {
    ProfScope ps(ctx, "sk_offsets", kNumCoarse);
    sk_front_report_clocks(ctx);
    sk_front_report_leave(ctx, fed, front_launched_waves);
    hipLaunchKernelGGL(sk_front_verify_kernel, dim3(1), dim3(1024), 0, ctx->stream, (const FrRange *)info, n_ranges, rpg, group_runs, ctx->d_totals + TOT_FRONT, ctx->d_flags);
    launch_rank_offsets(ctx->stream, (const uint32_t *)g.wg_hist, (uint32_t)kPartGroups, (uint32_t)kNumCoarse, g.cnt, g.base, g.wg_off);
  }
  KMI_HIP(ctx, hipGetLastError());
  const uint64_t r_bound = (uint64_t)n_ranges * item_cap;
  bool early = !out && n_bytes <= (8ull << 30);
  uint64_t *rec_a = out;
  if (early) {
    if (ws_get(ctx, WS_KEYS_A, (r_bound + 64) * 16, &p) == KMI_OK) rec_a = (uint64_t *)p; else { early = false; ctx->err.clear(); }
  }
  auto launch_scatter = [&]() {
    ProfScope ps(ctx, "sk_scatter", n_bytes);
#define KMI_SK_SCATTER_ROWS(CANON)                                                                                                     \
    hipLaunchKernelGGL(sk_scatter_rows_kernel<CANON>, dim3(kPartGroups), dim3(kFrScThreads), 0, ctx->stream, (const FrRange *)info, n_ranges, rpg, run_cap, \
                       item_cap, k, (const uint32_t *)run_items, (const uint32_t *)rows, (const uint32_t *)items, (const uint64_t *)g.wg_off, rec_a, lp,         \
                       (const uint32_t *)ctx->d_flags, ctx->edge_records ? 1u : 0u)
    if (canonical) KMI_SK_SCATTER_ROWS(true); else KMI_SK_SCATTER_ROWS(false);
#undef KMI_SK_SCATTER_ROWS
  };
  static_assert(H_MAIL_DECLINED == H_MAIL_CNT + 2 * kNumCoarse, "the mailbox holds the counts and starts of kNumCoarse groups");
  uint64_t *const h = ctx->h_totals;
  const uint64_t *const h_cnt = h + H_MAIL_CNT, *const h_tot = h + H_MAIL_FRONT;
  KMI_HIP(ctx, hipMemcpyAsync(h + H_MAIL_CNT, g.cnt, sizeof(uint64_t) * 2 * kNumCoarse, hipMemcpyDeviceToHost, ctx->stream));
  KMI_HIP(ctx, hipMemcpyAsync(h + H_MAIL_DECLINED, ctx->d_flags + FLAG_SK_DECLINED, sizeof(uint32_t), hipMemcpyDeviceToHost, ctx->stream));
  KMI_HIP(ctx, hipMemcpyAsync(h + H_MAIL_FRONT, ctx->d_totals + TOT_FRONT, sizeof(uint64_t) * 3, hipMemcpyDeviceToHost, ctx->stream));
  KMI_HIP(ctx, hipMemcpyAsync(h + H_MAIL_KMERS, ctx->d_totals + TOT_SK_KMERS, sizeof(uint64_t), hipMemcpyDeviceToHost, ctx->stream));
  if (early) {
    if (!ctx->ev_mail) KMI_HIP(ctx, hipEventCreateWithFlags(&ctx->ev_mail, hipEventDisableTiming));
    KMI_HIP(ctx, hipEventRecord(ctx->ev_mail, ctx->stream));
    launch_scatter();
    KMI_HIP(ctx, hipEventSynchronize(ctx->ev_mail));
  } else {
    KMI_HIP(ctx, hipStreamSynchronize(ctx->stream));
  }
  const uint32_t h_flag = *reinterpret_cast<const uint32_t *>(h + H_MAIL_DECLINED);
  const uint64_t n = h[H_MAIL_KMERS];
  if (h_flag) {
    sk_front_report_decline(ctx);
    static_assert(FLAG_SK_WHY == FLAG_SK_DECLINED + 1, "cleared together");
    KMI_HIP(ctx, hipMemsetAsync(ctx->d_flags + FLAG_SK_DECLINED, 0, 2 * sizeof(uint32_t), ctx->stream));
    return KMI_OK;
  }
  *took = true;
  uint64_t R = 0;
  for (int c = 0; c < kNumCoarse; ++c) { R += h_cnt[c]; f->h_cnt[c] = h_cnt[c]; f->h_base[c] = h_cnt[kNumCoarse + c]; }
  f->n_records = R; f->n_kmers = n; f->wg_off = g.wg_off; f->recs = nullptr; f->n_seqs = (h_tot[0] + 2) / 4;
  if (n == 0) { f->ok = true; return KMI_OK; }
  if (!early) {
    if (!out || R + 64 > out_cap) { KMI_TRY(ws_get(ctx, WS_KEYS_A, (R + 64) * 16, &p)); rec_a = (uint64_t *)p; }
    launch_scatter();
  }
  KMI_HIP(ctx, hipGetLastError());
  f->ok = true; f->recs = rec_a;
  return KMI_OK;
}

enum SkDoor { SK_RECORDS, SK_NO_KMERS, SK_NOT_THIS_PATH };
template <int W>
static kmi_status sk_front_door(kmi_ctx *ctx, const kmi_config *cfg, const KShape &shape, const uint8_t *bytes_dev, size_t n_bytes, uint32_t lp, SkFront *f,
                                SkDoor *door, uint64_t *out = nullptr, size_t out_cap = 0) {
  *door = SK_NOT_THIS_PATH;
  bool took = false;
  KMI_TRY((sk_front_fast<W>(ctx, cfg, shape, bytes_dev, n_bytes, lp, f, &took, out, out_cap)));
  if (took && f->ok) { *door = f->n_kmers ? SK_RECORDS : SK_NO_KMERS; return KMI_OK; }
  if (ctx->edge_records) return KMI_OK;
  FastqScan sc;
  KMI_TRY(align_input(ctx, &bytes_dev, n_bytes));
  KMI_TRY(fastq_scan(ctx, cfg, bytes_dev, n_bytes, &sc, false));
  if (sc.n_tuples == 0) { *door = SK_NO_KMERS; return fastq_length_verdict(ctx); }
  KMI_TRY((sk_front_end<W>(ctx, cfg, shape, sc, lp, f, out, out_cap)));
  if (f->ok) *door = SK_RECORDS;
  return KMI_OK;
}

static void sk_reduce_report_clocks(kmi_ctx *ctx) {
#ifdef KMI_SK_TIMING
  unsigned long long t[8];
  hipStreamSynchronize(ctx->stream);
  hipMemcpy(t, ctx->d_flags + FLAG_CLOCKS, sizeof(t), hipMemcpyDeviceToHost);
  fprintf(stderr, "sk_reduce wave clocks: A-T1 %llu  A-direct %llu  A-wait %llu  B-work %llu  B-wait %llu  emit %llu  between %llu\n", t[0], t[1], t[2], t[3], t[4], t[5], t[6]);
  hipMemset(ctx->d_flags + FLAG_CLOCKS, 0, sizeof(t));
#endif
}
static void sk_slack_report(const uint32_t *fine_cnt, const uint64_t *h_cnt, const uint32_t *h_cap, uint32_t lp, uint64_t R) {
  if (!getenv("KMI_SLACK_DEBUG")) return;
  std::vector<uint32_t> fc(kNumFine);
  (void)hipMemcpy(fc.data(), fine_cnt, sizeof(uint32_t) * kNumFine, hipMemcpyDeviceToHost);
  double worst = 0; uint32_t over = 0;
  for (int f = 0; f < kNumFine; ++f) {
    const double mean = (double)h_cnt[f / kSubPerCoarse] / kSubPerCoarse;
    if (mean > 0 && fc[f] / mean > worst) worst = fc[f] / mean;
    over += fc[f] > h_cap[f / kSubPerCoarse];
  }
  fprintf(stderr, "fine buckets with room: %u of %d outgrew it, the fullest holds %.3f x its coarse bucket's mean (lp %u, %llu records)\n", over,
          (int)kNumFine, worst, lp, (unsigned long long)R);
}

template <int W>
static kmi_status sk_back_end(kmi_index *idx, const uint64_t *rec_a, uint64_t R, const uint64_t *h_cnt, const uint64_t *h_base, const uint64_t *wg_off,
                              uint64_t n, uint32_t lp, bool exact = false) {
  constexpr int NW = 1;
  kmi_ctx *ctx = idx->ctx;
  const bool slack = !exact && ctx->sk_slack && (!idx->has_data || idx->n_entries == 0) && R >= 4096;
  ctx->sk_left.valid = false;
  const uint32_t k = idx->shape.k;
  const bool canonical = idx->cfg.strand != KMI_STRAND_SINGLE;
  void *p;
  SkGroupWs g;
  KMI_TRY(sk_group_ws(ctx, &g));
  uint64_t *const cend = g.cend;
  KMI_TRY(ws_get(ctx, WS_HIST, sizeof(uint32_t) * kNumFine * kFineParts + sizeof(uint64_t) * ((kNumFine + 1) * 2 + kNumFine * kFineParts + kNumCoarse) + 256, &p));
  uint32_t *fine_hist = (uint32_t *)p;
  uint64_t *fine_off = (uint64_t *)((char *)p + sizeof(uint32_t) * kNumFine * kFineParts);
  uint64_t *part_off = fine_off + 2 * (kNumFine + 1);
  uint64_t *coarse_base = part_off + (uint64_t)kNumFine * kFineParts;
  uint64_t h_end[kNumCoarse];
  for (int c = 0; c < kNumCoarse; ++c) h_end[c] = h_base[c] + h_cnt[c];
  KMI_HIP(ctx, hipMemcpyAsync(cend, h_end, sizeof(h_end), hipMemcpyHostToDevice, ctx->stream));
  const uint32_t m_len = idx->shape.k - (uint32_t)W + 1u;
  const uint64_t room_m = m_len <= 11u ? 26u : (m_len == 12u ? 18u : 14u);
  static const uint64_t room_lp[4] = {8, 10, 12, 15};
  const uint64_t room_x64 = room_m * room_lp[lp < 4u ? lp : 3u];
  uint64_t h_region[kNumCoarse], total_b = 0;
  uint32_t h_cap[kNumCoarse];
  for (int c = 0; c < kNumCoarse; ++c) {
    const uint64_t cap = ((h_cnt[c] * room_x64 / 64 + kSubPerCoarse - 1) / kSubPerCoarse + 64 + 7) / 8 * 8;
    h_cap[c] = (uint32_t)cap; h_region[c] = total_b; total_b += cap * kSubPerCoarse;
  }
  KMI_TRY(ws_get(ctx, WS_KEYS_B, ((slack ? total_b : R) + 64) * 16, &p)); uint64_t *rec_b = (uint64_t *)p;
  KMI_TRY(ws_get(ctx, WS_SPLIT_OFF, sizeof(uint32_t) * kNumFine * kFineParts + sizeof(uint64_t) * ((kNumFine + 1) + kNumFine * kFineParts + kNumCoarse) + 256, &p));
  uint32_t *fine_kmers = (uint32_t *)p;
  uint64_t *kmer_off = (uint64_t *)((char *)p + sizeof(uint32_t) * kNumFine * kFineParts);
  uint64_t *k_part = kmer_off + (kNumFine + 1), *k_base = k_part + (uint64_t)kNumFine * kFineParts;
  uint64_t *d_region = nullptr; uint32_t *d_cap = nullptr, *fine_cnt = nullptr;
  if (slack) {
    KMI_TRY(ws_get(ctx, WS_BUCKET_OFF, sizeof(uint64_t) * kNumCoarse + sizeof(uint32_t) * kNumCoarse + 64, &p));
    d_region = (uint64_t *)p; d_cap = (uint32_t *)(d_region + kNumCoarse);
    fine_cnt = fine_hist;
    KMI_HIP(ctx, hipMemcpyAsync(d_region, h_region, sizeof(h_region), hipMemcpyHostToDevice, ctx->stream));
    KMI_HIP(ctx, hipMemcpyAsync(d_cap, h_cap, sizeof(h_cap), hipMemcpyHostToDevice, ctx->stream));
    hipLaunchKernelGGL(sk_zero_kernel, dim3(96), dim3(1024), 0, ctx->stream, fine_cnt, (uint32_t)kNumFine, fine_kmers, (uint32_t)(kNumFine * kFineParts),
                       (uint32_t *)nullptr, 0u, ctx->d_flags, (uint32_t)FZ_BACK_0, (uint32_t)FZ_BACK_1, (uint32_t)FZ_BACK_2, (uint32_t)FZ_BACK_3);
    {
      ProfScope ps(ctx, "sk_scatter_fine", R);
      hipLaunchKernelGGL(sk_scatter_fine_slack_lines_kernel, dim3(kNumCoarse * kFineParts), dim3(kPartThreads), 0, ctx->stream, (const uint64_t *)rec_a, rec_b,
                         (const uint64_t *)wg_off, (const uint64_t *)cend, (uint32_t)kPartGroups, (const uint64_t *)d_region, (const uint32_t *)d_cap,
                         fine_cnt, fine_kmers, ctx->d_flags);
    }
    {
      ProfScope ps(ctx, "fine_offsets", kNumFine);
      launch_fine_offsets(ctx, fine_kmers, kmer_off, k_part, k_base);
    }
  } else {
    {
      ProfScope ps(ctx, "sk_fine_count", R);
      hipLaunchKernelGGL(sk_fine_count_kernel, dim3(kNumCoarse * kFineParts), dim3(1024), 0, ctx->stream, (const uint64_t *)rec_a,
                         (const uint64_t *)wg_off, (const uint64_t *)cend, (uint32_t)kPartGroups, fine_hist, fine_kmers);
    }
    {
      ProfScope ps(ctx, "fine_offsets", kNumFine);
      launch_fine_offsets(ctx, fine_hist, fine_off, part_off, coarse_base);
      launch_fine_offsets(ctx, fine_kmers, kmer_off, k_part, k_base);
    }
    {
      ProfScope ps(ctx, "sk_scatter_fine", R);
      hipLaunchKernelGGL((scatter_fine_kernel<1, 2, 1>), dim3(kNumCoarse * kFineParts), dim3(kPartThreads), 0, ctx->stream, (const uint64_t *)rec_a,
                         rec_b, idx->shape, (const uint64_t *)fine_off, (const uint64_t *)part_off, (const uint64_t *)wg_off,
                         (uint32_t)kPartGroups, (int)BUCKET_REC, 0u);
    }
  }
  KMI_TRY(ws_get(ctx, WS_TMP_KEYS, (n + 64) * sizeof(uint64_t), &p)); uint64_t *tmp_keys = (uint64_t *)p;
  KMI_TRY(ws_get(ctx, WS_TMP_VALS, (n + 64) * sizeof(uint32_t), &p)); uint32_t *tmp_vals = (uint32_t *)p;
  KMI_TRY(ws_get(ctx, WS_BUCKET_CNT, sizeof(uint32_t) * kNumFine, &p)); uint32_t *out_cnt = (uint32_t *)p;
  if (!slack) KMI_HIP(ctx, hipMemsetAsync(ctx->d_flags + FLAG_SK_LEVEL0, 0, sizeof(uint32_t) * (FLAG_SK_LEVEL_END - FLAG_SK_LEVEL0), ctx->stream));
  {
    const uint32_t nmax = sk_nmax_of(k);
    uint32_t *queue = ctx->d_flags + FLAG_REDUCE_QUEUE;
    if (!slack) KMI_HIP(ctx, hipMemsetAsync(queue, 0, sizeof(uint32_t) * (FLAG_REDUCE_QUEUE_END - FLAG_REDUCE_QUEUE), ctx->stream));
#ifndef KMI_SK_WGS_PER_CU
#define KMI_SK_WGS_PER_CU 1
#endif
    const uint32_t wgs = (ctx->n_cus ? ctx->n_cus : 256u) * KMI_SK_WGS_PER_CU;
    ProfScope ps(ctx, "sk_reduce", n);
#define KMI_SK_REDUCE(CANON, OWN, SPECIAL)                                                                                               \
    hipLaunchKernelGGL((sk_reduce_kernel<CANON, OWN, SPECIAL>), dim3(wgs), dim3(KMI_SK_NT), 0, ctx->stream, (const uint64_t *)rec_b,        \
                       (const uint64_t *)fine_off, k, (const uint64_t *)kmer_off, tmp_keys, tmp_vals, out_cnt, ctx->d_flags, queue, (uint32_t)kNumFine, \
                       ctx->sk_level_hint, lp, ctx->sk_inv_dup, (const uint64_t *)d_region, (const uint32_t *)d_cap, (const uint32_t *)fine_cnt)
    if (k == 32u) { if (canonical) KMI_SK_REDUCE(true, 64 * 21, true); else KMI_SK_REDUCE(false, 64 * 21, true); }
    else if (nmax <= 21u) { if (canonical) KMI_SK_REDUCE(true, 64 * 21, false); else KMI_SK_REDUCE(false, 64 * 21, false); }
    else if (nmax <= 24u) { if (canonical) KMI_SK_REDUCE(true, 64 * 24, false); else KMI_SK_REDUCE(false, 64 * 24, false); }
    else { if (canonical) KMI_SK_REDUCE(true, 64 * 32, false); else KMI_SK_REDUCE(false, 64 * 32, false); }
#undef KMI_SK_REDUCE
  }
  KMI_HIP(ctx, hipGetLastError());
  sk_reduce_report_clocks(ctx);
  if (slack) KMI_HIP(ctx, hipMemcpyAsync(ctx->h_totals + H_SK_ROOM, ctx->d_flags + FLAG_SK_ROOM, sizeof(uint32_t), hipMemcpyDeviceToHost, ctx->stream));
  KMI_HIP(ctx, hipMemcpyAsync(ctx->h_totals + H_SK_LEVELS , ctx->d_flags + FLAG_SK_LEVEL0, sizeof(uint32_t) * 9, hipMemcpyDeviceToHost, ctx->stream));
  auto read_levels = [&]() {
    const uint32_t *lv = reinterpret_cast<const uint32_t *>(ctx->h_totals + H_SK_LEVELS);
    uint64_t seen = 0; uint32_t best = 0;
    for (uint32_t l = 0; l < 9; ++l) { seen += lv[l]; if (lv[l] > lv[best]) best = l; }
    if (seen == 0) ctx->sk_level_hint = 0;
    else if (ctx->sk_level_hint == 0) { uint64_t up = seen; ctx->sk_level_hint = (up * 2 > (uint64_t)kNumFine) ? best : 0u; }
    else ctx->sk_level_hint = best;
  };
  const uint32_t layout = (uint32_t)W | (lp << 8);
  if (!idx->has_data || idx->n_entries == 0) {
    KMI_TRY((adopt_tmp<NW>(idx, tmp_keys, tmp_vals, kmer_off, nullptr, out_cnt, false, n, true)));
    if (slack) sk_slack_report(fine_cnt, h_cnt, h_cap, lp, R);
    if (slack && *reinterpret_cast<const uint32_t *>(ctx->h_totals + H_SK_ROOM)) {
      KMI_TRY(kmi_index_clear(idx));
      return sk_back_end<W>(idx, rec_a, R, h_cnt, h_base, wg_off, n, lp, true);
    }
    read_levels();
    idx->layout_w = layout;
    if (n) ctx->sk_inv_dup = (float)((double)idx->n_entries / (double)n);
    ctx->sk_left.recs = rec_b; ctx->sk_left.rec_off = slack ? nullptr : fine_off; ctx->sk_left.region = d_region; ctx->sk_left.cap = d_cap;
    ctx->sk_left.cnt = fine_cnt; ctx->sk_left.valid = true;
    return KMI_OK;
  }
  kmi_index scratch;
  scratch.ctx = ctx; scratch.cfg = idx->cfg; scratch.shape = idx->shape; scratch.val_words = 0; scratch.saturating = idx->saturating;
  kmi_status st = adopt_tmp<NW>(&scratch, tmp_keys, tmp_vals, kmer_off, nullptr, out_cnt);
  if (st == KMI_OK) read_levels();
  if (st == KMI_OK && n) ctx->sk_inv_dup = (float)((double)scratch.n_entries / (double)n);
  if (st == KMI_OK && scratch.n_entries) {
    st = ws_get(ctx, WS_OUTPUT, (scratch.n_entries + 64) * 2 * sizeof(uint64_t), &p);
    if (st == KMI_OK) {
      hipLaunchKernelGGL((zip_pairs_kernel<NW>), dim3(2048), dim3(256), 0, ctx->stream, (const uint64_t *)scratch.keys, (const uint32_t *)scratch.vals,
                         scratch.n_entries, (uint64_t *)p);
      st = index_insert_pairs(idx, (const uint64_t *)p, (size_t)scratch.n_entries, false, true);
    }
  }
  (void)hipStreamSynchronize(ctx->stream);
  free_index_arrays(&scratch);
  return st;
}
static kmi_status sk_back(kmi_index *idx, uint32_t w, const SkFront &f, uint32_t lp) {
  return sk_dispatch_w(w, [&](auto W) { return sk_back_end<W>(idx, f.recs, f.n_records, f.h_cnt, f.h_base, f.wg_off, f.n_kmers, lp); });
}

static kmi_status index_build_fused(kmi_index *idx, const uint8_t *bytes_dev, size_t n_bytes) {
  if (const uint32_t w = sk_width(idx, SK_FASTQ)) {
    SkFront f;
    SkDoor door;
    KMI_TRY(sk_dispatch_w(w, [&](auto W) { return sk_front_door<W>(idx->ctx, &idx->cfg, idx->shape, bytes_dev, n_bytes, 0u, &f, &door); }));
    if (door == SK_RECORDS) return sk_back(idx, w, f, 0u);
    if (door == SK_NO_KMERS) return KMI_OK;
  }
  KMI_DISPATCH(idx->shape, build_fused_impl, idx, bytes_dev, n_bytes);
}

static kmi_status sk_build_fasta(kmi_index *idx, uint32_t w, const FastaScan &fa, bool *done) {
  *done = false;
  SkFront f;
  FastqScan none{};
  KMI_TRY(sk_dispatch_w(w, [&](auto W) { return sk_front_end<W>(idx->ctx, &idx->cfg, idx->shape, none, 0u, &f, nullptr, 0, &fa); }));
  if (!f.ok) return KMI_OK;
  *done = true;
  if (f.n_records == 0) return KMI_OK;
  return sk_back(idx, w, f, 0u);
}

static kmi_status sk_produce(kmi_index *idx, uint32_t w, const uint8_t *bytes_dev, size_t n_bytes, uint32_t nranks, const uint64_t **recs_out, uint64_t *n_records,
                             uint64_t *send_counts, int *produced, uint64_t *out, size_t out_cap) {
  *produced = 0; *recs_out = nullptr; *n_records = 0;
  for (uint32_t r = 0; r < nranks; ++r) send_counts[r] = 0;
  if (n_bytes == 0) { *produced = 1; return KMI_OK; }
  const uint32_t lp = 31u - (uint32_t)__builtin_clz(nranks);
  SkFront f;
  SkDoor door;
  KMI_TRY(sk_dispatch_w(w, [&](auto W) { return sk_front_door<W>(idx->ctx, &idx->cfg, idx->shape, bytes_dev, n_bytes, lp, &f, &door, out, out_cap); }));
  if (door != SK_RECORDS) { *produced = door == SK_NO_KMERS; return KMI_OK; }
  const uint32_t per = (uint32_t)kNumCoarse / nranks;
  for (uint32_t c = 0; c < (uint32_t)kNumCoarse; ++c) send_counts[c / per] += f.h_cnt[c];
  *recs_out = f.recs; *n_records = f.n_records; *produced = 1;
  return KMI_OK;
}

static kmi_status sk_consume(kmi_index *idx, uint32_t w, const uint64_t *recs_dev, uint64_t R, uint32_t nranks) {
  kmi_ctx *ctx = idx->ctx;
  const uint32_t lp = 31u - (uint32_t)__builtin_clz(nranks);
  if (R == 0) { idx->owner_lp = lp; return KMI_OK; }
  void *p;
  SkGroupWs g;
  KMI_TRY(sk_group_ws(ctx, &g));
  KMI_TRY(ws_get(ctx, WS_KEYS_A, (R + 64) * 16, &p)); uint64_t *rec_a = (uint64_t *)p;
  KMI_HIP(ctx, hipMemsetAsync(ctx->d_totals + TOT_SK_KMERS, 0, sizeof(uint64_t), ctx->stream));
  {
    ProfScope ps(ctx, "sk_recv_hist", R);
    hipLaunchKernelGGL(sk_recv_hist_kernel, dim3(kPartGroups), dim3(kPartThreads), 0, ctx->stream, recs_dev, R, g.wg_hist,
                       (unsigned long long *)(ctx->d_totals + TOT_SK_KMERS));
  }
  {
    ProfScope ps(ctx, "sk_offsets", kNumCoarse);
    launch_rank_offsets(ctx->stream, (const uint32_t *)g.wg_hist, (uint32_t)kPartGroups, (uint32_t)kNumCoarse, g.cnt, g.base, g.wg_off);
  }
  BucketFn fn; fn.mode = BUCKET_REC_COARSE; fn.shape = idx->shape; fn.dist_hash = 0; fn.farm_ndebug = false; fn.nranks = 1; fn.sub = 1;
  {
    ProfScope ps(ctx, "sk_recv_scatter", R);
    hipLaunchKernelGGL((scatter_chunks_kernel<1, 2, 1>), dim3(kPartGroups), dim3(kPartThreads), 0, ctx->stream, recs_dev, R, rec_a, idx->shape, 0u, false, fn,
                       (const uint64_t *)g.wg_off);
  }
  KMI_HIP(ctx, hipGetLastError());
  uint64_t h[2 * kNumCoarse], n_kmers = 0;
  KMI_HIP(ctx, hipMemcpyAsync(h, g.cnt, sizeof(h), hipMemcpyDeviceToHost, ctx->stream));
  KMI_HIP(ctx, hipMemcpyAsync(&n_kmers, ctx->d_totals + TOT_SK_KMERS, sizeof(uint64_t), hipMemcpyDeviceToHost, ctx->stream));
  KMI_HIP(ctx, hipStreamSynchronize(ctx->stream));
  KMI_TRY(sk_dispatch_w(w, [&](auto W) { return sk_back_end<W>(idx, rec_a, R, h, h + kNumCoarse, g.wg_off, n_kmers, lp); }));
  idx->owner_lp = lp;
  return KMI_OK;
}

}
```

### kmerind_amd/csrc/kmi_superkmer.h

```cpp
#pragma once

namespace kmi {

constexpr int kRecNShift = 38, kRecHashShift = 43;
constexpr uint64_t kSkPadW1 = ~0ull;
constexpr int kRecEdgeShift = 32, kRecFlipShift = 61;
constexpr uint32_t kSkEdgeWindows = 3;
__device__ __forceinline__ uint32_t rec_hash18(uint64_t w1) { return (uint32_t)(w1 >> kRecHashShift) & 0x3ffffu; }
__device__ __forceinline__ uint32_t rec_fine_sub(uint64_t w1) { return (rec_hash18(w1) >> 3) & 127u; }

constexpr int kSkThreads = 512;
constexpr int kSkRoundTiles = 24;
constexpr int kSkListCap = 32;

struct SkRound {
  uint64_t t; uint32_t ei, total; uint32_t eo[kSkRoundTiles + 1]; uint64_t nt; uint32_t nei;
};
__device__ __forceinline__ bool sk_plan(const uint32_t *__restrict__ ent_cnt, uint64_t te, uint64_t t, uint32_t ei, SkRound &r) {
  while (t < te && ei >= ent_cnt[t]) { ++t; ei = 0; }
  if (t >= te) return false;
  r.t = t; r.ei = ei; r.eo[0] = 0;
  r.nt = t + kSkRoundTiles; r.nei = 0;
  bool cut = false;
#pragma unroll
  for (int i = 0; i < kSkRoundTiles; ++i) {
    uint32_t avail = (t + i < te) ? ent_cnt[t + i] : 0u;
    if (i == 0) avail -= ei;
    uint32_t take = avail;
    if (r.eo[i] + take > (uint32_t)kSkThreads) take = (uint32_t)kSkThreads - r.eo[i];
    if (cut) take = 0;
    if (!cut && take < avail) { cut = true; r.nt = t + i; r.nei = (i == 0 ? ei : 0u) + take; }
    r.eo[i + 1] = r.eo[i] + take;
  }
  r.total = r.eo[kSkRoundTiles];
  return true;
}
__device__ __forceinline__ void sk_locate(const SkRound &r, uint32_t e, uint32_t ent_stride, uint32_t &tr, uint64_t &idx) {
  tr = 0;
#pragma unroll
  for (int i = 1; i < kSkRoundTiles; ++i) tr += (e >= r.eo[i]) ? 1u : 0u;
  uint32_t base = 0;
#pragma unroll
  for (int i = 1; i < kSkRoundTiles; ++i) base = (tr == (uint32_t)i) ? r.eo[i] : base;
  idx = (r.t + tr) * ent_stride + (tr == 0u ? r.ei : 0u) + (e - base);
}
struct SkWin { uint32_t r0, r1, r2, sh; };
__device__ __forceinline__ SkWin sk_fetch(const uint32_t *__restrict__ st, uint64_t last_dw, uint64_t ip) {
  uint64_t d = ip >> 4;
  d = d < last_dw ? d : last_dw;
  SkWin w;
  w.r0 = st[d]; w.r1 = st[d + 1]; w.r2 = st[d + 2]; w.sh = (uint32_t)(ip & 15u) * 2u;
  return w;
}
__device__ __forceinline__ uint32_t sk_lo(const SkWin &w) { return __builtin_amdgcn_alignbit(w.r1, w.r0, w.sh); }
__device__ __forceinline__ uint32_t sk_hi(const SkWin &w) { return __builtin_amdgcn_alignbit(w.r2, w.r1, w.sh); }

__global__ __launch_bounds__(256) void fasta_runs_kernel(const uint32_t *__restrict__ brk, uint64_t n_chars, uint64_t n_valid, uint64_t n_cover,
                                                        uint64_t n_tiles, uint32_t k, uint32_t seg, uint32_t *__restrict__ ent,
                                                        uint32_t *__restrict__ ent_cnt, uint32_t stride, unsigned long long *__restrict__ n_windows,
                                                        uint32_t *__restrict__ flags) {
  const uint32_t lane = lane_id();
  const uint64_t n_words = n_cover / 32;
  const uint64_t n_waves = (uint64_t)gridDim.x * (blockDim.x / kWave);
  for (uint64_t t = (uint64_t)blockIdx.x * (blockDim.x / kWave) + wave_id(); t < n_tiles; t += n_waves) {
    const uint64_t p0 = t * 8192ull + (uint64_t)lane * 128ull;
    uint64_t x[3];
    {
      uint32_t w[7];
      const uint64_t w0 = p0 >> 5;
#pragma unroll
      for (int i = 0; i < 7; ++i) w[i] = (w0 + i < n_words) ? brk[w0 + i] : 0u;
#pragma unroll
      for (int j = 0; j < 3; ++j) {
        const uint64_t lo = (uint64_t)w[2 * j] | ((uint64_t)w[2 * j + 1] << 32), hi = (uint64_t)w[2 * j + 2];
        x[j] = (lo >> 1) | (hi << 63);
      }
    }
    smear_right<3>(x, k - 1u);
    uint64_t v0 = ~x[0], v1 = ~x[1];
    {
      const uint64_t lim_a = n_chars >= k ? n_chars - k + 1u : 0u, lim = lim_a < n_valid ? lim_a : n_valid;
      const uint64_t room = lim > p0 ? lim - p0 : 0u;
      v0 &= room >= 64 ? ~0ull : ((1ull << room) - 1ull);
// ... 269 lines not shown
      d0 = d0 + 16 <= last_dw + 16 ? d0 : 0;
      const uint4 q0 = *reinterpret_cast<const uint4 *>(st + d0), q1 = *reinterpret_cast<const uint4 *>(st + d0 + 4),
                  q2 = *reinterpret_cast<const uint4 *>(st + d0 + 8), q3 = *reinterpret_cast<const uint4 *>(st + d0 + 12);
      uint32_t *row = s_row + threadIdx.x * kSkRowDw;
      row[0] = q0.x; row[1] = q0.y; row[2] = q0.z; row[3] = q0.w; row[4] = q1.x; row[5] = q1.y; row[6] = q1.z; row[7] = q1.w;
      row[8] = q2.x; row[9] = q2.y; row[10] = q2.z; row[11] = q2.w; row[12] = q3.x; row[13] = q3.y; row[14] = q3.z; row[15] = q3.w;
      row[16] = 0;
      s_bit0[threadIdx.x] = (uint32_t)(ip0 - d0 * 16) * 2u;
      s_ioff[threadIdx.x] = ri & 0x3ffffffu;
    }
#pragma unroll
    for (int j = 0; j < CAP; ++j)
      if ((uint32_t)j < cnt) atomicAdd(&s_cnt[(it[j] >> 22) & 255u], 1u);
    lds_barrier();
    uint32_t c = 0, inc = 0;
    if (threadIdx.x < kNumCoarse) {
      c = s_cnt[threadIdx.x];
      s_cnt[threadIdx.x] = 0;
      inc = wave_inclusive_sum_dpp(c);
      if (lane_id() == kWave - 1) s_part[wave_id()] = inc;
    }
    lds_barrier();
    if (threadIdx.x < kNumCoarse) {
      uint32_t pre = 0;
#pragma unroll
      for (uint32_t w = 0; w < kNumCoarse / kWave; ++w) pre += (w < wave_id()) ? s_part[w] : 0u;
      const uint32_t lo = pre + inc - c;
      s_cur[threadIdx.x] = lo;
      s_gbase[threadIdx.x] = cursor - lo;
      cursor += c;
      if (threadIdx.x == kNumCoarse - 1) s_total = pre + inc;
    }
    lds_barrier();
#pragma unroll
    for (int j = 0; j < CAP; ++j)
      if ((uint32_t)j < cnt) s_stage[atomicAdd(&s_cur[(it[j] >> 22) & 255u], 1u)] = (uint16_t)((threadIdx.x << 5) | (uint32_t)j);
    lds_barrier();
    const uint32_t total = s_total;
    for (uint32_t s = threadIdx.x; s < total; s += NT) {
      const uint32_t e = s_stage[s], rl = e >> 5, j = e & 31u;
      const uint32_t item = wg_items[s_ioff[rl] + j];
      const uint32_t h18 = (item >> 12) & 0x3ffffu, n1 = (item >> 7) & 31u, extra = item >> 30;
      const uint32_t hs = ((h18 << lp) & 0x3ffffu) | (lp <= 2u ? extra >> (2u - lp) : extra << (lp - 2u));
      uint64_t w0, w1;
      sk_assemble_row<CANON>(s_row + rl * kSkRowDw, s_bit0[rl] + 2u * (item & 127u), k + n1, n1, hs, w0, w1);
      reinterpret_cast<ulonglong2 *>(out)[s_gbase[h18 >> 10] + s] = make_ulonglong2(w0, w1);
    }
    SkRound nxt;
    have = sk_plan(ent_cnt, te, cur.nt, cur.nei, nxt);
    cur = nxt;
  }
}

__global__ __launch_bounds__(1024) void sk_fine_count_kernel(const uint64_t *__restrict__ recs, const uint64_t *__restrict__ wg_off,
                                                            const uint64_t *__restrict__ coarse_end ,
                                                            uint32_t groups, uint32_t *__restrict__ fine_hist ,
                                                            uint32_t *__restrict__ fine_kmers ) {
  __shared__ uint32_t s_h[kSubPerCoarse], s_k[kSubPerCoarse];
  const uint32_t gpp = groups / kFineParts;
  const uint32_t c = blockIdx.x / kFineParts, h = blockIdx.x % kFineParts;
  if (threadIdx.x < kSubPerCoarse) { s_h[threadIdx.x] = 0; s_k[threadIdx.x] = 0; }
  lds_barrier();
  const uint64_t b = wg_off[(uint64_t)(h * gpp) * kNumCoarse + c];
  const uint64_t e = (h + 1 < (uint32_t)kFineParts) ? wg_off[(uint64_t)((h + 1) * gpp) * kNumCoarse + c] : coarse_end[c];
  for (uint64_t i = b + threadIdx.x; i < e; i += blockDim.x) {
    const uint64_t w1 = recs[2 * i + 1];
    atomicAdd(&s_h[rec_fine_sub(w1)], 1u);
    atomicAdd(&s_k[rec_fine_sub(w1)], ((uint32_t)(w1 >> kRecNShift) & 31u) + 1u);
  }
  lds_barrier();
  if (threadIdx.x < kSubPerCoarse) {
    fine_hist[(uint64_t)h * kNumFine + c * kSubPerCoarse + threadIdx.x] = s_h[threadIdx.x];
    fine_kmers[(uint64_t)h * kNumFine + c * kSubPerCoarse + threadIdx.x] = s_k[threadIdx.x];
  }
}

constexpr int kSlackLineRecs = 8;
constexpr int kSlackLT = 3072;
constexpr int kSlackLCap = kSlackLT + (kSlackLineRecs - 1) * kSubPerCoarse;
__global__ __launch_bounds__(kPartThreads) void sk_scatter_fine_slack_lines_kernel(const uint64_t *__restrict__ recs, uint64_t *__restrict__ out,
                                                                                 const uint64_t *__restrict__ wg_off, const uint64_t *__restrict__ coarse_end,
                                                                                 uint32_t groups, const uint64_t *__restrict__ fine_region,
                                                                                 const uint32_t *__restrict__ fine_cap, uint32_t *__restrict__ fine_cnt,
                                                                                 uint32_t *__restrict__ fine_kmers, uint32_t *__restrict__ flags) {
  constexpr int NB = kSubPerCoarse, T = kSlackLT, PT = T / kPartThreads, SCAP = kSlackLCap, L = kSlackLineRecs, MAXG = SCAP / L + NB;
  static_assert(kPartThreads / NB == L && T % kPartThreads == 0, "one carry slot per thread: eight threads per bucket");
  __shared__ ulonglong2 s_stage[SCAP];
  __shared__ uint32_t s_cnt[NB];
  __shared__ uint32_t s_k[NB];
  __shared__ uint32_t s_lofs[NB];
  __shared__ uint32_t s_emit[NB];
  __shared__ uint32_t s_old[NB];
  __shared__ uint32_t s_lbase[NB];
  __shared__ uint64_t s_dst[NB];
  __shared__ uint32_t s_part[NB / kWave];
  __shared__ uint32_t s_ng;
  __shared__ uint8_t s_linebkt[MAXG];
  const uint32_t gpp = groups / kFineParts;
  const uint32_t c = blockIdx.x / kFineParts, h = blockIdx.x % kFineParts;
  const uint64_t b = wg_off[(uint64_t)(h * gpp) * kNumCoarse + c];
  const uint64_t e = (h + 1 < (uint32_t)kFineParts) ? wg_off[(uint64_t)((h + 1) * gpp) * kNumCoarse + c] : coarse_end[c];
  if (b >= e) return;
  const uint64_t region = fine_region[c];
  const uint32_t cap = fine_cap[c];
  if (threadIdx.x < NB) { s_cnt[threadIdx.x] = 0; s_k[threadIdx.x] = 0; }
  const uint32_t cb = threadIdx.x / L, cj = threadIdx.x % L;
  ulonglong2 carry = make_ulonglong2(0, 0);
  uint32_t my_carry = 0;
  lds_barrier();
  const ulonglong2 *src = reinterpret_cast<const ulonglong2 *>(recs);
  ulonglong2 raw[PT];
  auto load_tile = [&](uint64_t t0) {
#pragma unroll
    for (int j = 0; j < PT; ++j) {
      uint64_t i = t0 + (uint64_t)j * kPartThreads + threadIdx.x;
      i = (i < e) ? i : e - 1;
      raw[j] = src[i];
    }
  };
  auto take = [&](uint32_t f, uint32_t n) -> uint64_t {
    const uint32_t at = atomicAdd(&fine_cnt[c * NB + f], n);
    if ((uint64_t)at + n > (uint64_t)cap) { atomicOr(&flags[FLAG_SK_ROOM], 1u); return ~0ull; }
    return region + (uint64_t)f * cap + at;
  };
  load_tile(b);
  for (uint64_t t0 = b; t0 < e; t0 += T) {
    const uint32_t nt = (uint32_t)((e - t0 < (uint64_t)T) ? (e - t0) : (uint64_t)T);
    ulonglong2 rec[PT];
    uint32_t bk[PT], rk[PT];
#pragma unroll
    for (int j = 0; j < PT; ++j) {
      const uint32_t li = j * kPartThreads + threadIdx.x;
      rec[j] = raw[j];
      bk[j] = 0xffffffffu;
      if (li < nt) {
        bk[j] = rec_fine_sub(rec[j].y);
        rk[j] = atomicAdd(&s_cnt[bk[j]], 1u);
        atomicAdd(&s_k[bk[j]], ((uint32_t)(rec[j].y >> kRecNShift) & 31u) + 1u);
      }
    }
    if (t0 + T < e) load_tile(t0 + T);
    lds_barrier();
    uint32_t cnt = 0, emit = 0, ng = 0, inc = 0;
    if (threadIdx.x < NB) {
      cnt = s_cnt[threadIdx.x];
      const uint32_t km = s_k[threadIdx.x];
      s_k[threadIdx.x] = 0;
      emit = cnt & ~(uint32_t)(L - 1);
      ng = emit / L;
      inc = wave_inclusive_sum_dpp(cnt | (ng << 16));
      if (lane_id() == kWave - 1) s_part[wave_id()] = inc;
      if (km) atomicAdd(&fine_kmers[c * NB + threadIdx.x], km);
      s_dst[threadIdx.x] = emit ? take(threadIdx.x, emit) : ~0ull;
    }
    lds_barrier();
    if (threadIdx.x < NB) {
      const uint32_t pre = wave_id() ? s_part[0] : 0u;
      const uint32_t ex = pre + inc - (cnt | (ng << 16));
      const uint32_t lo = ex & 0xffffu, lb = ex >> 16;
      s_lofs[threadIdx.x] = lo; s_emit[threadIdx.x] = emit; s_old[threadIdx.x] = my_carry; s_lbase[threadIdx.x] = lb;
      for (uint32_t i = 0; i < ng; ++i) s_linebkt[lb + i] = (uint8_t)threadIdx.x;
      if (threadIdx.x == NB - 1) s_ng = lb + ng;
      s_cnt[threadIdx.x] = cnt - emit;
      my_carry = cnt - emit;
    }
    lds_barrier();
    if (cj < s_old[cb]) s_stage[s_lofs[cb] + cj] = carry;
#pragma unroll
    for (int j = 0; j < PT; ++j)
      if (bk[j] != 0xffffffffu) s_stage[s_lofs[bk[j]] + rk[j]] = rec[j];
    lds_barrier();
    {
      const uint32_t n_groups = s_ng, l8 = threadIdx.x & (uint32_t)(L - 1);
      for (uint32_t g = threadIdx.x / L; g < n_groups; g += kPartThreads / L) {
        const uint32_t f = s_linebkt[g];
        const uint64_t d = s_dst[f];
        const uint32_t i = (g - s_lbase[f]) * L + l8;
        if (d != ~0ull) reinterpret_cast<ulonglong2 *>(out)[d + i] = s_stage[s_lofs[f] + i];
      }
      const uint32_t rem = s_cnt[cb], base = s_lofs[cb] + s_emit[cb];
      if (cj < rem) carry = s_stage[base + cj];
    }
    lds_barrier();
  }
  {
    if (threadIdx.x < NB) s_dst[threadIdx.x] = my_carry ? take(threadIdx.x, (uint32_t)L) : ~0ull;
    lds_barrier();
    const uint32_t rem = s_cnt[cb];
    const uint64_t d = s_dst[cb];
    if (rem && d != ~0ull) reinterpret_cast<ulonglong2 *>(out)[d + cj] = cj < rem ? carry : make_ulonglong2(kEmptyKey, kSkPadW1);
  }
}

__global__ __launch_bounds__(1024) void sk_zero_kernel(uint32_t *__restrict__ a, uint32_t na, uint32_t *__restrict__ b, uint32_t nb,
                                                     uint32_t *__restrict__ c, uint32_t nc, uint32_t *__restrict__ flags, uint32_t f0, uint32_t f1,
                                                     uint32_t g0, uint32_t g1) {
  const uint32_t i = blockIdx.x * blockDim.x + threadIdx.x, stride = gridDim.x * blockDim.x;
  for (uint32_t x = i; x < na; x += stride) a[x] = 0;
  for (uint32_t x = i; x < nb; x += stride) b[x] = 0;
  for (uint32_t x = i; x < nc; x += stride) c[x] = 0;
  if (i >= f0 && i < f1) flags[i] = 0;
  if (i >= g0 && i < g1) flags[i] = 0;
}

__global__ __launch_bounds__(kPartThreads) void sk_recv_hist_kernel(const uint64_t *__restrict__ recs, uint64_t n, uint32_t *__restrict__ wg_hist,
                                                                   unsigned long long *__restrict__ n_kmers) {
  __shared__ uint32_t s_h[kNumCoarse];
  __shared__ unsigned long long s_k;
  if (threadIdx.x < kNumCoarse) s_h[threadIdx.x] = 0;
  if (threadIdx.x == 0) s_k = 0ull;
  lds_barrier();
  const uint64_t chunk = part_chunk(n, gridDim.x, PartCfg<2>::TILE);
  const uint64_t b = (uint64_t)blockIdx.x * chunk, e = (b + chunk < n) ? b + chunk : n;
  unsigned long long km = 0;
  for (uint64_t i = b + threadIdx.x; i < e; i += blockDim.x) {
    const uint64_t w1 = recs[2 * i + 1];
    atomicAdd(&s_h[rec_hash18(w1) >> 10], 1u);
    km += ((uint32_t)(w1 >> kRecNShift) & 31u) + 1u;
  }
  km = wave_reduce_sum(km);
  if (lane_id() == 0 && km) atomicAdd(&s_k, km);
  lds_barrier();
  if (threadIdx.x < kNumCoarse) wg_hist[(uint64_t)blockIdx.x * kNumCoarse + threadIdx.x] = s_h[threadIdx.x];
  if (threadIdx.x == 0 && s_k) atomicAdd(n_kmers, s_k);
}

#ifndef KMI_SK_H1
#define KMI_SK_H1 1536
#endif
#ifndef KMI_SK_T1_DUP
#define KMI_SK_T1_DUP 0.5f
#endif
#ifndef KMI_SK_FILL
#define KMI_SK_FILL 80
#endif
#ifndef KMI_SK_NT
#define KMI_SK_NT 1024
#endif
#ifndef KMI_SK_LDS_KB
#define KMI_SK_LDS_KB 160
#endif
#ifndef KMI_SK_HASH24
#define KMI_SK_HASH24 1
#endif
__device__ __forceinline__ uint32_t sk_slot_hash(uint64_t key) {
#if KMI_SK_HASH24
  const uint32_t lo = (uint32_t)key, hi = (uint32_t)(key >> 32);
  uint32_t h = __umul24(lo, 0x9E3779u);
  h += __umul24(__builtin_amdgcn_alignbit(hi, lo, 24), 0x85EBCBu);
  h += __umul24(hi >> 16, 0xC2B2AFu);
#else
  uint32_t h = ((uint32_t)key ^ ((uint32_t)(key >> 32) * 0x85EBCA6Bu)) * 0x9E3779B1u;
#endif
  h ^= h >> 15;
  return h;
}
__device__ __forceinline__ uint32_t sk_slot_of(uint32_t h, uint32_t cap) { return __umul24(h >> 16, cap) >> 16; }

#ifndef KMI_SK_PROBE_ATTR
#define KMI_SK_PROBE_ATTR __forceinline__
#endif
__device__ KMI_SK_PROBE_ATTR uint32_t sk_probe_insert(lds_u64_t *tkeys, lds_u32_t *tvals, lds_u32_t *distinct, lds_u32_t *overflow,
                                                         const lds_u64_t *q, const lds_u32_t *qw, uint32_t first, uint32_t cnt,
                                                         uint32_t cap, uint32_t last, uint32_t limit, uint32_t pending) {
  const uint32_t lane = lane_id();
  bool claimed = false;
  if (lane < cnt) {
    const uint64_t key = q[first + lane];
    const uint32_t wt = qw[first + lane];
    const uint32_t s0 = sk_slot_of(sk_slot_hash(key), cap);
    uint32_t s = s0;
    uint64_t c = __atomic_load_n(&tkeys[s], __ATOMIC_RELAXED);
    for (;;) {
      while (c != key && c != kEmptyKey && s - s0 < 64u) { ++s; c = __atomic_load_n(&tkeys[s], __ATOMIC_RELAXED); }
      if (c == key) break;
      if (c != kEmptyKey || s >= last) { *overflow = 1; s = last; break; }
      uint64_t expected = kEmptyKey;
      if (__atomic_compare_exchange_n(&tkeys[s], &expected, key, false, __ATOMIC_RELAXED, __ATOMIC_RELAXED)) { claimed = true; break; }
      c = expected;
    }
    __atomic_fetch_add(&tvals[s], wt, __ATOMIC_RELAXED);
  }
  const unsigned long long cm = __ballot(claimed);
  const uint32_t add = (uint32_t)__popcll(cm) + pending;
  if (add >= 16u || (add && cnt < 64u)) {
// ... 497 lines not shown
```

Baseline: 197.9 billion.

## Fuse small bookkeeping kernels and use mapped host mailbox to cut launches and copies

Maps the host totals buffer into device space so kernels can write their readbacks straight to pinned host memory, replacing several small device-to-host copies. Folds several small kernels into fewer launches: rank totals go into the verify kernel, rank bases and cursors become one kernel, and layout computation moves into the zero kernel. It also pre-allocates adopt buffers and copies offsets inside the bucket-offsets kernel, so separate device-to-device copies are no longer needed. The aim is to cut launch and synchronisation overhead on the build path. The cost is more complex control flow and reliance on coherent system-memory writes with fences.

```diff
diff --git a/kmerind_amd/csrc/kmi_api.hip b/kmerind_amd/csrc/kmi_api.hip
--- a/kmerind_amd/csrc/kmi_api.hip
+++ b/kmerind_amd/csrc/kmi_api.hip
@@ -242,7 +242,8 @@
   ctx->device = device; ctx->rank = rank; ctx->nranks = nranks; ctx->stream = (hipStream_t)stream;
   if (hipMalloc((void **)&ctx->d_flags, sizeof(uint32_t) * kmi::FLAG_NUM_WORDS) != hipSuccess ||
       hipMalloc((void **)&ctx->d_totals, sizeof(uint64_t) * kmi::TOT_NUM_WORDS) != hipSuccess ||
-      hipHostMalloc((void **)&ctx->h_totals, sizeof(uint64_t) * kmi::H_NUM_WORDS, hipHostMallocDefault)    != hipSuccess) {
+      hipHostMalloc((void **)&ctx->h_totals, sizeof(uint64_t) * kmi::H_NUM_WORDS, hipHostMallocMapped | hipHostMallocCoherent)    != hipSuccess ||
+      hipHostGetDevicePointer((void **)&ctx->d_mail, ctx->h_totals, 0) != hipSuccess) {
     delete ctx;
     return KMI_ERR_DEVICE;
   }
diff --git a/kmerind_amd/csrc/kmi_front.h b/kmerind_amd/csrc/kmi_front.h
--- a/kmerind_amd/csrc/kmi_front.h
+++ b/kmerind_amd/csrc/kmi_front.h
@@ -675,9 +675,20 @@
   }
 }
 
+constexpr uint32_t kFrVerifyBlocks = 1u + (uint32_t)kNumCoarse / (1024u / (uint32_t)kWave);
 __global__ __launch_bounds__(1024) void sk_front_verify_kernel(const FrRange *__restrict__ info, uint32_t n_ranges, uint32_t ranges_per_group,
                                                              uint64_t *__restrict__ group_runs ,
-                                                             uint64_t *__restrict__ totals , uint32_t *__restrict__ flags) {
+                                                             uint64_t *__restrict__ totals , uint32_t *__restrict__ flags,
+                                                             const uint32_t *__restrict__ wg_hist, uint32_t hist_groups, uint64_t *__restrict__ bucket_cnt) {
+  if (blockIdx.x != 0) {
+    const uint32_t c = (blockIdx.x - 1) * (blockDim.x >> 6) + wave_id();
+    if (c >= (uint32_t)kNumCoarse) return;
+    uint64_t v = 0;
+    for (uint32_t w = lane_id(); w < hist_groups; w += kWave) v += wg_hist[(uint64_t)w * kNumCoarse + c];
+    v = wave_reduce_sum(v);
+    if (lane_id() == 0) bucket_cnt[c] = v;
+    return;
+  }
   __shared__ uint64_t s_scan[1024 / 64 + 2];
   __shared__ uint32_t s_bad;
   if (threadIdx.x == 0) s_bad = 0;
diff --git a/kmerind_amd/csrc/kmi_index.hip b/kmerind_amd/csrc/kmi_index.hip
--- a/kmerind_amd/csrc/kmi_index.hip
+++ b/kmerind_amd/csrc/kmi_index.hip
@@ -4,6 +4,7 @@
 
 #include "kmi_extract.h"
 #include "kmi_minimizer.h"
+#include "kmi_sk_room.h"
 #include <type_traits>
 
 namespace kmi {
@@ -219,9 +220,10 @@
   }
   if (c == (uint32_t)kNumCoarse - 1 && threadIdx.x == 0) fine_off[kNumFine] = grand;
 }
-static void launch_fine_offsets(kmi_ctx *ctx, const uint32_t *fine_hist, uint64_t *fine_off, uint64_t *part_off, uint64_t *coarse_base) {
+static void launch_fine_offsets(kmi_ctx *ctx, const uint32_t *fine_hist, uint64_t *fine_off, uint64_t *part_off, uint64_t *coarse_base,
+                                bool have_totals = false) {
   uint64_t *tot = ctx->d_totals + TOT_COARSE;
-  hipLaunchKernelGGL(fine_totals_kernel, dim3(kNumCoarse), dim3(kSubPerCoarse), 0, ctx->stream, fine_hist, tot);
+  if (!have_totals) hipLaunchKernelGGL(fine_totals_kernel, dim3(kNumCoarse), dim3(kSubPerCoarse), 0, ctx->stream, fine_hist, tot);
   hipLaunchKernelGGL(fine_offsets_spread_kernel, dim3(kNumCoarse), dim3(kSubPerCoarse), 0, ctx->stream, fine_hist, (const uint64_t *)tot, fine_off, part_off,
                      coarse_base);
 }
@@ -249,18 +251,56 @@
   v = wave_reduce_sum(v);
   if (lane_id() == 0) bucket_cnt[c] = v;
 }
-__global__ __launch_bounds__(256) void rank_bases_kernel(const uint64_t *__restrict__ bucket_cnt, uint32_t nbuckets, uint64_t *__restrict__ base) {
+struct FrontMail {
+  uint64_t *mail;
+  const uint32_t *flags;
+  const uint64_t *totals;
+  SkLayout lay;
+};
+__global__ __launch_bounds__(256) void rank_cursors_kernel(const uint32_t *__restrict__ wg_hist, uint32_t groups, const uint64_t *__restrict__ bucket_cnt,
+                                                          uint32_t nbuckets, uint64_t *__restrict__ base, uint64_t *__restrict__ wg_off, FrontMail fm) {
+  static_assert(kNumCoarse == 256, "one thread per coarse bucket");
   __shared__ uint64_t s_scan[256 / 64 + 2];
+  __shared__ uint64_t s_base[kNumCoarse];
   const uint64_t tot = (threadIdx.x < nbuckets) ? bucket_cnt[threadIdx.x] : 0ull;
-  uint64_t total;
-  const uint64_t off = block_exclusive_scan<uint64_t>(tot, s_scan, &total);
-  base[threadIdx.x] = off;
+  const uint64_t off = block_exclusive_scan<uint64_t>(tot, s_scan, (uint64_t *)nullptr);
+  s_base[threadIdx.x] = off;
+  if (blockIdx.x == 0) {
+    base[threadIdx.x] = off;
+    if (fm.mail) {
+      fm.mail[H_MAIL_CNT + threadIdx.x] = tot;
+      fm.mail[H_MAIL_CNT + kNumCoarse + threadIdx.x] = off;
+      if (threadIdx.x == 0) fm.mail[H_MAIL_DECLINED] = fm.flags[FLAG_SK_DECLINED];
+      if (threadIdx.x >= 1 && threadIdx.x <= 3) fm.mail[H_MAIL_FRONT + threadIdx.x - 1] = fm.totals[TOT_FRONT + threadIdx.x - 1];
+      if (threadIdx.x == 4) fm.mail[H_MAIL_KMERS] = fm.totals[TOT_SK_KMERS];
+      __threadfence_system();
+    }
+    if (fm.lay.cend) {
+      const uint64_t cap = sk_fine_cap(tot, fm.lay.room_x64, (uint64_t)kSubPerCoarse);
+      const uint64_t at = block_exclusive_scan<uint64_t>(cap * kSubPerCoarse, s_scan, (uint64_t *)nullptr);
+      fm.lay.cend[threadIdx.x] = off + tot; fm.lay.cap[threadIdx.x] = (uint32_t)cap; fm.lay.region[threadIdx.x] = at;
+    }
+  }
+  lds_barrier();
+  const uint32_t c = blockIdx.x * (blockDim.x >> 6) + wave_id();
+  if (c >= (uint32_t)kNumCoarse) return;
+  uint64_t carry = s_base[c];
+  for (uint32_t w0 = 0; w0 < groups; w0 += kWave) {
+    const uint32_t w = w0 + lane_id();
+    const uint64_t v = (w < groups) ? wg_hist[(uint64_t)w * kNumCoarse + c] : 0ull;
+    const uint64_t inc = wave_inclusive_scan(v);
+    if (w < groups) wg_off[(uint64_t)w * kNumCoarse + c] = carry + inc - v;
+    carry += __shfl(inc, kWave - 1, kWave);
+  }
+}
+static void launch_rank_cursors(hipStream_t stream, const uint32_t *wg_hist, uint32_t groups, uint32_t nbuckets, const uint64_t *bucket_cnt,
+                                uint64_t *base , uint64_t *wg_off, FrontMail fm = FrontMail{nullptr, nullptr, nullptr, SkLayout{}}) {
+  hipLaunchKernelGGL(rank_cursors_kernel, dim3(kNumCoarse / 4), dim3(256), 0, stream, wg_hist, groups, bucket_cnt, nbuckets, base, wg_off, fm);
 }
 static void launch_rank_offsets(hipStream_t stream, const uint32_t *wg_hist, uint32_t groups, uint32_t nbuckets, uint64_t *bucket_cnt,
                                 uint64_t *base , uint64_t *wg_off) {
   hipLaunchKernelGGL(rank_totals_kernel, dim3(kNumCoarse / 4), dim3(256), 0, stream, wg_hist, groups, nbuckets, bucket_cnt);
-  hipLaunchKernelGGL(rank_bases_kernel, dim3(1), dim3(256), 0, stream, (const uint64_t *)bucket_cnt, nbuckets, base);
-  hipLaunchKernelGGL(coarse_cursors_kernel, dim3(kNumCoarse / 4), dim3(256), 0, stream, wg_hist, groups, (const uint64_t *)base, wg_off);
+  launch_rank_cursors(stream, wg_hist, groups, nbuckets, (const uint64_t *)bucket_cnt, base, wg_off);
 }
 
 template <int NW, int BITS, int VW = 0, int TILE_ = PartCfg<NW + VW>::TILE>
@@ -2121,6 +2161,44 @@
   if (threadIdx.x == 0) { off[kNumFine] = total; totals[slot] = total; }
 }
 
+struct BackMail {
+  uint64_t *mail;
+  uint32_t *flags;
+  const uint64_t *src_off;
+  uint64_t *off_copy;
+  uint32_t *cnt_copy;
+};
+__global__ __launch_bounds__(1024) void bucket_offsets_mail_kernel(const uint32_t *__restrict__ cnt, uint64_t *__restrict__ off,
+                                                                  uint64_t *__restrict__ totals, int slot, BackMail bm) {
+  if (blockIdx.x != 0) {
+    if (!bm.off_copy) return;
+    const uint32_t i0 = (blockIdx.x - 1) * blockDim.x + threadIdx.x, stride = (gridDim.x - 1) * blockDim.x;
+    for (uint32_t i = i0; i <= (uint32_t)kNumFine; i += stride) {
+      bm.off_copy[i] = bm.src_off[i];
+      if (i < (uint32_t)kNumFine) bm.cnt_copy[i] = cnt[i];
+    }
+    return;
+  }
+  __shared__ uint64_t s_scan[1024 / 64 + 2];
+  constexpr int PER = kNumFine / 1024;
+  uint64_t loc[PER], sum = 0;
+#pragma unroll
+  for (int i = 0; i < PER; ++i) { loc[i] = cnt[threadIdx.x * PER + i]; sum += loc[i]; }
+  uint64_t total;
+  uint64_t o = block_exclusive_scan<uint64_t>(sum, s_scan, &total);
+#pragma unroll
+  for (int i = 0; i < PER; ++i) { off[threadIdx.x * PER + i] = o; o += loc[i]; }
+  if (threadIdx.x == 0) { off[kNumFine] = total; totals[slot] = total; bm.mail[slot] = total; }
+  if (threadIdx.x >= 64 && threadIdx.x < 64 + 9) reinterpret_cast<uint32_t *>(bm.mail + H_SK_LEVELS)[threadIdx.x - 64] = bm.flags[FLAG_SK_LEVEL0 + threadIdx.x - 64];
+  if (threadIdx.x == 128) bm.mail[H_SK_ROOM] = bm.flags[FLAG_SK_ROOM];
+  if (threadIdx.x == 192) {
+    const uint32_t over = bm.flags[FLAG_PASS_LIMIT];
+    bm.mail[H_SK_PASS_LIMIT] = over;
+    if (over) bm.flags[FLAG_PASS_LIMIT] = 0;
+  }
+  __threadfence_system();
+}
+
 template <int NW, typename V>
 __global__ __launch_bounds__(256) void bucket_compact_kernel(const uint64_t *__restrict__ tmp_keys, const V *__restrict__ tmp_vals,
                                                             const uint64_t *__restrict__ src_off_a, const uint64_t *__restrict__ src_off_b,
@@ -2409,43 +2487,94 @@
   return KMI_OK;
 }
 
+struct AdoptAhead {
+  uint64_t *new_off = nullptr, *off = nullptr;
+  uint32_t *cnt = nullptr;
+  bool room = false;
+};
+static bool sparse_room(kmi_ctx *ctx) {
+  size_t free_b = 0, total_b = 0;
+  return hipMemGetInfo(&free_b, &total_b) == hipSuccess && free_b >= ctx->ws[WS_TMP_KEYS].cap + ctx->ws[WS_TMP_VALS].cap + ((size_t)1 << 30);
+}
+static kmi_status adopt_ahead_alloc(kmi_ctx *ctx, uint64_t n_slots, bool allow_sparse, AdoptAhead *a) {
+  KMI_HIP(ctx, pool_alloc(ctx, (void **)&a->new_off, kOffBytes));
+  if (allow_sparse && n_slots >= ctx->sparse_min) {
+    const hipError_t e1 = pool_alloc(ctx, (void **)&a->off, kOffBytes), e2 = pool_alloc(ctx, (void **)&a->cnt, sizeof(uint32_t) * kNumFine);
+    if (e1 != hipSuccess || e2 != hipSuccess) {
+      (void)hipGetLastError();
+      if (a->off) pool_free(ctx, a->off, kOffBytes);
+      if (a->cnt) pool_free(ctx, a->cnt, sizeof(uint32_t) * kNumFine);
+      a->off = nullptr; a->cnt = nullptr;
+    }
+  }
+  return KMI_OK;
+}
+static void adopt_ahead_release(kmi_ctx *ctx, AdoptAhead *a) {
+  if (a->off) pool_free(ctx, a->off, kOffBytes);
+  if (a->cnt) pool_free(ctx, a->cnt, sizeof(uint32_t) * kNumFine);
+  a->off = nullptr; a->cnt = nullptr;
+}
+
 template <int NW>
 static kmi_status adopt_tmp(kmi_index *idx, const uint64_t *tmp_keys, const uint32_t *tmp_vals, const uint64_t *src_a, const uint64_t *src_b,
-                            const uint32_t *out_cnt, bool fastq_verdict = false, uint64_t n_slots = 0, bool allow_sparse = false) {
+                            const uint32_t *out_cnt, bool fastq_verdict = false, uint64_t n_slots = 0, bool allow_sparse = false,
+                            AdoptAhead *ahead = nullptr) {
   kmi_ctx *ctx = idx->ctx;
-  uint64_t *new_off = nullptr;
-  KMI_HIP(ctx, pool_alloc(ctx, (void **)&new_off, kOffBytes));
-  {
-    ProfScope ps(ctx, "bucket_offsets", kNumFine);
-    hipLaunchKernelGGL(bucket_offsets_kernel, dim3(1), dim3(1024), 0, ctx->stream, out_cnt, new_off, ctx->d_totals, (int)TOT_ENTRIES);
-  }
+  uint64_t *new_off = ahead ? ahead->new_off : nullptr;
+  if (!ahead) KMI_HIP(ctx, pool_alloc(ctx, (void **)&new_off, kOffBytes));
   uint64_t total = 0;
-  kmi_status st_total = read_total(ctx, TOT_ENTRIES, &total);
+  kmi_status st_total = KMI_OK;
+  if (ahead) {
+    {
+      ProfScope ps(ctx, "bucket_offsets", kNumFine);
+      const BackMail bm{ctx->d_mail, ctx->d_flags, src_a, ahead->off, ahead->cnt};
+      hipLaunchKernelGGL(bucket_offsets_mail_kernel, dim3(ahead->off ? 9 : 1), dim3(1024), 0, ctx->stream, out_cnt, new_off, ctx->d_totals, (int)TOT_ENTRIES, bm);
+    }
+    const hipError_t e = hipStreamSynchronize(ctx->stream);
+    if (e != hipSuccess) {
+      pool_free(ctx, new_off, kOffBytes); adopt_ahead_release(ctx, ahead);
+      return set_err(ctx, KMI_ERR_DEVICE, "%s failed: %s", "hipStreamSynchronize(ctx->stream)", hipGetErrorString(e));
+    }
+    total = ctx->h_totals[TOT_ENTRIES];
+    if (ctx->h_totals[H_SK_PASS_LIMIT]) st_total = set_err(ctx, KMI_ERR_OVERFLOW, "a bucket could not be reduced within the pass limit");
+  } else {
+    {
+      ProfScope ps(ctx, "bucket_offsets", kNumFine);
+      hipLaunchKernelGGL(bucket_offsets_kernel, dim3(1), dim3(1024), 0, ctx->stream, out_cnt, new_off, ctx->d_totals, (int)TOT_ENTRIES);
+    }
+    st_total = read_total(ctx, TOT_ENTRIES, &total);
+  }
   if (st_total == KMI_OK && fastq_verdict) st_total = fastq_length_verdict(ctx);
-  if (st_total != KMI_OK) { pool_free(ctx, new_off, kOffBytes); return st_total; }
+  if (st_total != KMI_OK) { pool_free(ctx, new_off, kOffBytes); if (ahead) adopt_ahead_release(ctx, ahead); return st_total; }
   if (n_slots && total == n_slots && !src_b && ctx->ws[WS_TMP_KEYS].p == (const void *)tmp_keys && ctx->ws[WS_TMP_VALS].p == (const void *)tmp_vals) {
     size_t kb0 = 0, vb0 = 0;
     (void)ws_detach(ctx, WS_TMP_KEYS, tmp_keys, &kb0);
     (void)ws_detach(ctx, WS_TMP_VALS, tmp_vals, &vb0);
     KMI_HIP(ctx, hipStreamSynchronize(ctx->stream));
+    if (ahead) adopt_ahead_release(ctx, ahead);
     free_index_arrays(idx);
     idx->keys = const_cast<uint64_t *>(tmp_keys); idx->vals = const_cast<uint32_t *>(tmp_vals); idx->bucket_off = new_off;
     idx->n_entries = total; idx->has_data = true; idx->keys_bytes = kb0; idx->vals_bytes = vb0;
     return KMI_OK;
   }
   bool room = false;
-  if (NW == 1 && allow_sparse && n_slots >= ctx->sparse_min) {
-    size_t free_b = 0, total_b = 0;
-    room = hipMemGetInfo(&free_b, &total_b) == hipSuccess && free_b >= ctx->ws[WS_TMP_KEYS].cap + ctx->ws[WS_TMP_VALS].cap + ((size_t)1 << 30);
-  }
+  if (NW == 1 && allow_sparse && n_slots >= ctx->sparse_min) room = ahead ? ahead->room : sparse_room(ctx);
   if (NW == 1 && allow_sparse && room && n_slots >= ctx->sparse_min && !src_b && ctx->ws[WS_TMP_KEYS].p == (const void *)tmp_keys &&
       ctx->ws[WS_TMP_VALS].p == (const void *)tmp_vals) {
     uint64_t *off = nullptr; uint32_t *cnt = nullptr;
-    hipError_t e1 = pool_alloc(ctx, (void **)&off, kOffBytes);
-    hipError_t e2 = pool_alloc(ctx, (void **)&cnt, sizeof(uint32_t) * kNumFine);
+    hipError_t e1 = hipSuccess, e2 = hipSuccess;
+    if (ahead) {
+      off = ahead->off; cnt = ahead->cnt; ahead->off = nullptr; ahead->cnt = nullptr;
+      if (!off) e1 = e2 = hipErrorOutOfMemory;
+    } else {
+      e1 = pool_alloc(ctx, (void **)&off, kOffBytes);
+      e2 = pool_alloc(ctx, (void **)&cnt, sizeof(uint32_t) * kNumFine);
+    }
     if (e1 == hipSuccess && e2 == hipSuccess) {
-      KMI_HIP(ctx, hipMemcpyAsync(off, src_a, kOffBytes, hipMemcpyDeviceToDevice, ctx->stream));
-      KMI_HIP(ctx, hipMemcpyAsync(cnt, out_cnt, sizeof(uint32_t) * kNumFine, hipMemcpyDeviceToDevice, ctx->stream));
+      if (!ahead) {
+        KMI_HIP(ctx, hipMemcpyAsync(off, src_a, kOffBytes, hipMemcpyDeviceToDevice, ctx->stream));
+        KMI_HIP(ctx, hipMemcpyAsync(cnt, out_cnt, sizeof(uint32_t) * kNumFine, hipMemcpyDeviceToDevice, ctx->stream));
+      }
       size_t kb0 = 0, vb0 = 0;
       (void)ws_detach(ctx, WS_TMP_KEYS, tmp_keys, &kb0);
       (void)ws_detach(ctx, WS_TMP_VALS, tmp_vals, &vb0);
@@ -2457,6 +2586,7 @@
     if (off) pool_free(ctx, off, kOffBytes);
     if (cnt) pool_free(ctx, cnt, sizeof(uint32_t) * kNumFine);
   }
+  if (ahead) adopt_ahead_release(ctx, ahead);
   uint64_t *nk = nullptr; uint32_t *nv = nullptr;
   const size_t kb = (total ? total : 1) * NW * sizeof(uint64_t), vb = (total ? total : 1) * sizeof(uint32_t);
   hipError_t e1 = pool_alloc(ctx, (void **)&nk, kb);
diff --git a/kmerind_amd/csrc/kmi_internal.h b/kmerind_amd/csrc/kmi_internal.h
--- a/kmerind_amd/csrc/kmi_internal.h
+++ b/kmerind_amd/csrc/kmi_internal.h
@@ -141,6 +141,7 @@
 enum HostWord : uint32_t {
   H_BATCH_END = 8,
   H_SK_LEVELS = 8,
+  H_SK_PASS_LIMIT = 13,
   H_SK_ROOM = 14,
   H_MAIL = 16,
   H_MAIL_CNT = H_MAIL,
@@ -149,7 +150,7 @@
   H_MAIL_KMERS = H_MAIL + 516,
   H_NUM_WORDS = 16 + 1024
 };
-static_assert(H_BATCH_END == (uint32_t)TOT_BATCH_END && H_SK_LEVELS > (uint32_t)TOT_RESULTS && H_SK_LEVELS + 5 <= H_SK_ROOM &&
+static_assert(H_BATCH_END == (uint32_t)TOT_BATCH_END && H_SK_LEVELS > (uint32_t)TOT_RESULTS && H_SK_LEVELS + 5 <= H_SK_PASS_LIMIT && H_SK_PASS_LIMIT < H_SK_ROOM &&
               H_SK_ROOM < H_MAIL && H_MAIL == (uint32_t)TOT_COARSE && H_MAIL_KMERS < H_NUM_WORDS,
               "the read-backs of a build overlap neither each other nor the mirrored totals a build reads (entries, results)");
 
@@ -187,6 +188,7 @@
   size_t host_overlap_min = (size_t)64 << 20;
   size_t feed_min_chunk = (size_t)8 << 20;
   uint64_t *h_totals = nullptr;
+  uint64_t *d_mail = nullptr;
   bool prof = false;
   std::vector<kmi::ProfRec> prof_pending;
   std::vector<kmi::ProfAgg> prof_agg;
diff --git a/kmerind_amd/csrc/kmi_sk_build.h b/kmerind_amd/csrc/kmi_sk_build.h
--- a/kmerind_amd/csrc/kmi_sk_build.h
+++ b/kmerind_amd/csrc/kmi_sk_build.h
@@ -38,12 +38,39 @@
   return KMI_OK;
 }
 
+struct SkBackWs {
+  uint32_t *fine_hist;
+  uint64_t *fine_off, *part_off, *coarse_base;
+  uint32_t *fine_kmers;
+  uint64_t *kmer_off, *k_part, *k_base;
+  uint64_t *d_region; uint32_t *d_cap;
+};
+static kmi_status sk_back_ws(kmi_ctx *ctx, SkBackWs *t) {
+  void *p;
+  KMI_TRY(ws_get(ctx, WS_HIST, sizeof(uint32_t) * kNumFine * kFineParts + sizeof(uint64_t) * ((kNumFine + 1) * 2 + kNumFine * kFineParts + kNumCoarse) + 256, &p));
+  t->fine_hist = (uint32_t *)p;
+  t->fine_off = (uint64_t *)((char *)p + sizeof(uint32_t) * kNumFine * kFineParts);
+  t->part_off = t->fine_off + 2 * (kNumFine + 1);
+  t->coarse_base = t->part_off + (uint64_t)kNumFine * kFineParts;
+  KMI_TRY(ws_get(ctx, WS_SPLIT_OFF, sizeof(uint32_t) * kNumFine * kFineParts + sizeof(uint64_t) * ((kNumFine + 1) + kNumFine * kFineParts + kNumCoarse) + 256, &p));
+  t->fine_kmers = (uint32_t *)p;
+  t->kmer_off = (uint64_t *)((char *)p + sizeof(uint32_t) * kNumFine * kFineParts);
+  t->k_part = t->kmer_off + (kNumFine + 1); t->k_base = t->k_part + (uint64_t)kNumFine * kFineParts;
+  KMI_TRY(ws_get(ctx, WS_BUCKET_OFF, sizeof(uint64_t) * kNumCoarse + sizeof(uint32_t) * kNumCoarse + 64, &p));
+  t->d_region = (uint64_t *)p; t->d_cap = (uint32_t *)(t->d_region + kNumCoarse);
+  return KMI_OK;
+}
+#define KMI_SK_BACK_ZEROES(ctx, t)                                                                                                     \
+  (t).fine_hist, (uint32_t)kNumFine, (t).fine_kmers, (uint32_t)(kNumFine * kFineParts), reinterpret_cast<uint32_t *>((ctx)->d_totals + TOT_COARSE), \
+  2u * (uint32_t)kNumCoarse
+
 struct SkFront {
   bool ok = false;
   uint64_t *recs = nullptr;
   uint64_t n_records = 0, n_kmers = 0, n_seqs = 0;
   uint64_t h_cnt[kNumCoarse], h_base[kNumCoarse];
   uint64_t *wg_off = nullptr;
+  bool back_ready = false;
 };
 
 template <int W>
@@ -172,7 +199,7 @@
 static kmi_status sk_front_fast(kmi_ctx *ctx, const kmi_config *cfg, const KShape &shape, const uint8_t *bytes_dev, size_t n_bytes, uint32_t lp, SkFront *f,
                                 bool *took, uint64_t *out = nullptr, size_t out_cap = 0) {
   *took = false;
-  f->ok = false;
+  f->ok = false; f->back_ready = false;
   const bool fed = ctx->feed_host != nullptr && bytes_dev == ctx->feed_dev && n_bytes == ctx->feed_bytes;
   if (!fed) KMI_TRY(feed_flush(ctx));
   if (!ctx->front_fused || cfg->seq_format != KMI_FMT_FASTQ || cfg->seq_filter != KMI_SEQ_ALL || n_bytes < 64) return feed_flush(ctx);
@@ -201,9 +228,11 @@
   KMI_TRY(ws_get(ctx, WS_SK_ITEMS, sizeof(uint32_t) * ((size_t)n_ranges * item_cap + 64), &p)); uint32_t *items = (uint32_t *)p;
   SkGroupWs g;
   KMI_TRY(sk_group_ws(ctx, &g));
+  SkBackWs bt;
+  KMI_TRY(sk_back_ws(ctx, &bt));
   hipLaunchKernelGGL(sk_zero_kernel, dim3(128), dim3(1024), 0, ctx->stream, g.wg_hist, (uint32_t)(kPartGroups * kNumCoarse),
-                     reinterpret_cast<uint32_t *>(ctx->d_totals + TOT_SK_KMERS), 2u, (uint32_t *)nullptr, 0u, ctx->d_flags, (uint32_t)FZ_FRONT_0,
-                     (uint32_t)FZ_FRONT_1, 0u, 0u);
+                     reinterpret_cast<uint32_t *>(ctx->d_totals + TOT_SK_KMERS), 2u, KMI_SK_BACK_ZEROES(ctx, bt), ctx->d_flags, (uint32_t)FZ_FRONT_0,
+                     (uint32_t)FZ_FRONT_1, (uint32_t)FZ_BACK_0, (uint32_t)FZ_BACK_1, (uint32_t)FZ_BACK_2, (uint32_t)FZ_BACK_3, SkLayout{});
   auto launch_front = [&](uint32_t wgs, uint32_t r0, uint32_t r1, uint32_t *queue) {
 #define KMI_SK_FRONT(EDGES)                                                                                                            \
     hipLaunchKernelGGL((sk_front_kernel<W, EDGES>), dim3(wgs), dim3(kFrThreads), 0, ctx->stream, bytes_dev, (uint64_t)n_bytes, range_bytes, n_ranges, k, \
@@ -264,8 +293,11 @@
     ProfScope ps(ctx, "sk_offsets", kNumCoarse);
     sk_front_report_clocks(ctx);
     sk_front_report_leave(ctx, fed, front_launched_waves);
-    hipLaunchKernelGGL(sk_front_verify_kernel, dim3(1), dim3(1024), 0, ctx->stream, (const FrRange *)info, n_ranges, rpg, group_runs, ctx->d_totals + TOT_FRONT, ctx->d_flags);
-    launch_rank_offsets(ctx->stream, (const uint32_t *)g.wg_hist, (uint32_t)kPartGroups, (uint32_t)kNumCoarse, g.cnt, g.base, g.wg_off);
+    hipLaunchKernelGGL(sk_front_verify_kernel, dim3(kFrVerifyBlocks), dim3(1024), 0, ctx->stream, (const FrRange *)info, n_ranges, rpg, group_runs,
+                       ctx->d_totals + TOT_FRONT, ctx->d_flags, (const uint32_t *)g.wg_hist, (uint32_t)kPartGroups, g.cnt);
+    launch_rank_cursors(ctx->stream, (const uint32_t *)g.wg_hist, (uint32_t)kPartGroups, (uint32_t)kNumCoarse, (const uint64_t *)g.cnt, g.base, g.wg_off,
+                        FrontMail{ctx->d_mail, ctx->d_flags, ctx->d_totals,
+                                  SkLayout{nullptr, nullptr, g.cend, bt.d_region, bt.d_cap, sk_room_x64(k - (uint32_t)W + 1u, lp)}});
   }
   KMI_HIP(ctx, hipGetLastError());
   const uint64_t r_bound = (uint64_t)n_ranges * item_cap;
@@ -286,10 +318,6 @@
   static_assert(H_MAIL_DECLINED == H_MAIL_CNT + 2 * kNumCoarse, "the mailbox holds the counts and starts of kNumCoarse groups");
   uint64_t *const h = ctx->h_totals;
   const uint64_t *const h_cnt = h + H_MAIL_CNT, *const h_tot = h + H_MAIL_FRONT;
-  KMI_HIP(ctx, hipMemcpyAsync(h + H_MAIL_CNT, g.cnt, sizeof(uint64_t) * 2 * kNumCoarse, hipMemcpyDeviceToHost, ctx->stream));
-  KMI_HIP(ctx, hipMemcpyAsync(h + H_MAIL_DECLINED, ctx->d_flags + FLAG_SK_DECLINED, sizeof(uint32_t), hipMemcpyDeviceToHost, ctx->stream));
-  KMI_HIP(ctx, hipMemcpyAsync(h + H_MAIL_FRONT, ctx->d_totals + TOT_FRONT, sizeof(uint64_t) * 3, hipMemcpyDeviceToHost, ctx->stream));
-  KMI_HIP(ctx, hipMemcpyAsync(h + H_MAIL_KMERS, ctx->d_totals + TOT_SK_KMERS, sizeof(uint64_t), hipMemcpyDeviceToHost, ctx->stream));
   if (early) {
     if (!ctx->ev_mail) KMI_HIP(ctx, hipEventCreateWithFlags(&ctx->ev_mail, hipEventDisableTiming));
     KMI_HIP(ctx, hipEventRecord(ctx->ev_mail, ctx->stream));
@@ -310,6 +338,7 @@
   uint64_t R = 0;
   for (int c = 0; c < kNumCoarse; ++c) { R += h_cnt[c]; f->h_cnt[c] = h_cnt[c]; f->h_base[c] = h_cnt[kNumCoarse + c]; }
   f->n_records = R; f->n_kmers = n; f->wg_off = g.wg_off; f->recs = nullptr; f->n_seqs = (h_tot[0] + 2) / 4;
+  f->back_ready = true;
   if (n == 0) { f->ok = true; return KMI_OK; }
   if (!early) {
     if (!out || R + 64 > out_cap) { KMI_TRY(ws_get(ctx, WS_KEYS_A, (R + 64) * 16, &p)); rec_a = (uint64_t *)p; }
@@ -363,7 +392,7 @@
 
 template <int W>
 static kmi_status sk_back_end(kmi_index *idx, const uint64_t *rec_a, uint64_t R, const uint64_t *h_cnt, const uint64_t *h_base, const uint64_t *wg_off,
-                              uint64_t n, uint32_t lp, bool exact = false) {
+                              uint64_t n, uint32_t lp, bool exact = false, bool prepared = false) {
   constexpr int NW = 1;
   kmi_ctx *ctx = idx->ctx;
   const bool slack = !exact && ctx->sk_slack && (!idx->has_data || idx->n_entries == 0) && R >= 4096;
@@ -374,47 +403,41 @@
   SkGroupWs g;
   KMI_TRY(sk_group_ws(ctx, &g));
   uint64_t *const cend = g.cend;
-  KMI_TRY(ws_get(ctx, WS_HIST, sizeof(uint32_t) * kNumFine * kFineParts + sizeof(uint64_t) * ((kNumFine + 1) * 2 + kNumFine * kFineParts + kNumCoarse) + 256, &p));
-  uint32_t *fine_hist = (uint32_t *)p;
-  uint64_t *fine_off = (uint64_t *)((char *)p + sizeof(uint32_t) * kNumFine * kFineParts);
-  uint64_t *part_off = fine_off + 2 * (kNumFine + 1);
-  uint64_t *coarse_base = part_off + (uint64_t)kNumFine * kFineParts;
-  uint64_t h_end[kNumCoarse];
-  for (int c = 0; c < kNumCoarse; ++c) h_end[c] = h_base[c] + h_cnt[c];
-  KMI_HIP(ctx, hipMemcpyAsync(cend, h_end, sizeof(h_end), hipMemcpyHostToDevice, ctx->stream));
-  const uint32_t m_len = idx->shape.k - (uint32_t)W + 1u;
-  const uint64_t room_m = m_len <= 11u ? 26u : (m_len == 12u ? 18u : 14u);
-  static const uint64_t room_lp[4] = {8, 10, 12, 15};
-  const uint64_t room_x64 = room_m * room_lp[lp < 4u ? lp : 3u];
-  uint64_t h_region[kNumCoarse], total_b = 0;
+  SkBackWs bt;
+  KMI_TRY(sk_back_ws(ctx, &bt));
+  uint32_t *const fine_hist = bt.fine_hist, *const fine_kmers = bt.fine_kmers;
+  uint64_t *const fine_off = bt.fine_off, *const part_off = bt.part_off, *const coarse_base = bt.coarse_base;
+  uint64_t *const kmer_off = bt.kmer_off, *const k_part = bt.k_part, *const k_base = bt.k_base;
+  const uint64_t room_x64 = sk_room_x64(idx->shape.k - (uint32_t)W + 1u, lp);
+  uint64_t total_b = 0;
   uint32_t h_cap[kNumCoarse];
   for (int c = 0; c < kNumCoarse; ++c) {
-    const uint64_t cap = ((h_cnt[c] * room_x64 / 64 + kSubPerCoarse - 1) / kSubPerCoarse + 64 + 7) / 8 * 8;
-    h_cap[c] = (uint32_t)cap; h_region[c] = total_b; total_b += cap * kSubPerCoarse;
+    h_cap[c] = (uint32_t)sk_fine_cap(h_cnt[c], room_x64, (uint64_t)kSubPerCoarse);
+    total_b += sk_region_records(h_cnt[c], room_x64, (uint64_t)kSubPerCoarse);
+  }
+  uint64_t h_end[kNumCoarse];
+  if (!slack) {
+    for (int c = 0; c < kNumCoarse; ++c) h_end[c] = h_base[c] + h_cnt[c];
+    KMI_HIP(ctx, hipMemcpyAsync(cend, h_end, sizeof(h_end), hipMemcpyHostToDevice, ctx->stream));
   }
   KMI_TRY(ws_get(ctx, WS_KEYS_B, ((slack ? total_b : R) + 64) * 16, &p)); uint64_t *rec_b = (uint64_t *)p;
-  KMI_TRY(ws_get(ctx, WS_SPLIT_OFF, sizeof(uint32_t) * kNumFine * kFineParts + sizeof(uint64_t) * ((kNumFine + 1) + kNumFine * kFineParts + kNumCoarse) + 256, &p));
-  uint32_t *fine_kmers = (uint32_t *)p;
-  uint64_t *kmer_off = (uint64_t *)((char *)p + sizeof(uint32_t) * kNumFine * kFineParts);
-  uint64_t *k_part = kmer_off + (kNumFine + 1), *k_base = k_part + (uint64_t)kNumFine * kFineParts;
   uint64_t *d_region = nullptr; uint32_t *d_cap = nullptr, *fine_cnt = nullptr;
   if (slack) {
-    KMI_TRY(ws_get(ctx, WS_BUCKET_OFF, sizeof(uint64_t) * kNumCoarse + sizeof(uint32_t) * kNumCoarse + 64, &p));
-    d_region = (uint64_t *)p; d_cap = (uint32_t *)(d_region + kNumCoarse);
+    d_region = bt.d_region; d_cap = bt.d_cap;
     fine_cnt = fine_hist;
-    KMI_HIP(ctx, hipMemcpyAsync(d_region, h_region, sizeof(h_region), hipMemcpyHostToDevice, ctx->stream));
-    KMI_HIP(ctx, hipMemcpyAsync(d_cap, h_cap, sizeof(h_cap), hipMemcpyHostToDevice, ctx->stream));
-    hipLaunchKernelGGL(sk_zero_kernel, dim3(96), dim3(1024), 0, ctx->stream, fine_cnt, (uint32_t)kNumFine, fine_kmers, (uint32_t)(kNumFine * kFineParts),
-                       (uint32_t *)nullptr, 0u, ctx->d_flags, (uint32_t)FZ_BACK_0, (uint32_t)FZ_BACK_1, (uint32_t)FZ_BACK_2, (uint32_t)FZ_BACK_3);
+    if (!prepared)
+      hipLaunchKernelGGL(sk_zero_kernel, dim3(96), dim3(1024), 0, ctx->stream, KMI_SK_BACK_ZEROES(ctx, bt), (uint32_t *)nullptr, 0u, (uint32_t *)nullptr, 0u,
+                         ctx->d_flags, (uint32_t)FZ_BACK_0, (uint32_t)FZ_BACK_1, (uint32_t)FZ_BACK_2, (uint32_t)FZ_BACK_3, 0u, 0u,
+                         SkLayout{(const uint64_t *)g.cnt, (const uint64_t *)g.base, cend, d_region, d_cap, room_x64});
     {
       ProfScope ps(ctx, "sk_scatter_fine", R);
       hipLaunchKernelGGL(sk_scatter_fine_slack_lines_kernel, dim3(kNumCoarse * kFineParts), dim3(kPartThreads), 0, ctx->stream, (const uint64_t *)rec_a, rec_b,
                          (const uint64_t *)wg_off, (const uint64_t *)cend, (uint32_t)kPartGroups, (const uint64_t *)d_region, (const uint32_t *)d_cap,
-                         fine_cnt, fine_kmers, ctx->d_flags);
+                         fine_cnt, fine_kmers, ctx->d_flags, (unsigned long long *)(ctx->d_totals + TOT_COARSE));
     }
     {
       ProfScope ps(ctx, "fine_offsets", kNumFine);
-      launch_fine_offsets(ctx, fine_kmers, kmer_off, k_part, k_base);
+      launch_fine_offsets(ctx, fine_kmers, kmer_off, k_part, k_base, true);
     }
   } else {
     {
@@ -437,11 +460,20 @@
   KMI_TRY(ws_get(ctx, WS_TMP_KEYS, (n + 64) * sizeof(uint64_t), &p)); uint64_t *tmp_keys = (uint64_t *)p;
   KMI_TRY(ws_get(ctx, WS_TMP_VALS, (n + 64) * sizeof(uint32_t), &p)); uint32_t *tmp_vals = (uint32_t *)p;
   KMI_TRY(ws_get(ctx, WS_BUCKET_CNT, sizeof(uint32_t) * kNumFine, &p)); uint32_t *out_cnt = (uint32_t *)p;
-  if (!slack) KMI_HIP(ctx, hipMemsetAsync(ctx->d_flags + FLAG_SK_LEVEL0, 0, sizeof(uint32_t) * (FLAG_SK_LEVEL_END - FLAG_SK_LEVEL0), ctx->stream));
+  const bool fresh = !idx->has_data || idx->n_entries == 0;
+  AdoptAhead ahead;
+  KMI_TRY(adopt_ahead_alloc(ctx, n, fresh, &ahead));
+  auto drop_ahead = [&](hipError_t e, const char *what) {
+    pool_free(ctx, ahead.new_off, kOffBytes); ahead.new_off = nullptr;
+    adopt_ahead_release(ctx, &ahead);
+    return set_err(ctx, KMI_ERR_DEVICE, "%s failed: %s", what, hipGetErrorString(e));
+  };
+#define KMI_HIP_AHEAD(call) do { const hipError_t e__ = (call); if (e__ != hipSuccess) return drop_ahead(e__, #call); } while (0)
+  if (!slack) KMI_HIP_AHEAD(hipMemsetAsync(ctx->d_flags + FLAG_SK_LEVEL0, 0, sizeof(uint32_t) * (FLAG_SK_LEVEL_END - FLAG_SK_LEVEL0), ctx->stream));
   {
     const uint32_t nmax = sk_nmax_of(k);
     uint32_t *queue = ctx->d_flags + FLAG_REDUCE_QUEUE;
-    if (!slack) KMI_HIP(ctx, hipMemsetAsync(queue, 0, sizeof(uint32_t) * (FLAG_REDUCE_QUEUE_END - FLAG_REDUCE_QUEUE), ctx->stream));
+    if (!slack) KMI_HIP_AHEAD(hipMemsetAsync(queue, 0, sizeof(uint32_t) * (FLAG_REDUCE_QUEUE_END - FLAG_REDUCE_QUEUE), ctx->stream));
 #ifndef KMI_SK_WGS_PER_CU
 #define KMI_SK_WGS_PER_CU 1
 #endif
@@ -457,10 +489,10 @@
     else { if (canonical) KMI_SK_REDUCE(true, 64 * 32, false); else KMI_SK_REDUCE(false, 64 * 32, false); }
 #undef KMI_SK_REDUCE
   }
-  KMI_HIP(ctx, hipGetLastError());
+  KMI_HIP_AHEAD(hipGetLastError());
+#undef KMI_HIP_AHEAD
+  if (ahead.off) ahead.room = sparse_room(ctx);
   sk_reduce_report_clocks(ctx);
-  if (slack) KMI_HIP(ctx, hipMemcpyAsync(ctx->h_totals + H_SK_ROOM, ctx->d_flags + FLAG_SK_ROOM, sizeof(uint32_t), hipMemcpyDeviceToHost, ctx->stream));
-  KMI_HIP(ctx, hipMemcpyAsync(ctx->h_totals + H_SK_LEVELS , ctx->d_flags + FLAG_SK_LEVEL0, sizeof(uint32_t) * 9, hipMemcpyDeviceToHost, ctx->stream));
   auto read_levels = [&]() {
     const uint32_t *lv = reinterpret_cast<const uint32_t *>(ctx->h_totals + H_SK_LEVELS);
     uint64_t seen = 0; uint32_t best = 0;
@@ -471,7 +503,7 @@
   };
   const uint32_t layout = (uint32_t)W | (lp << 8);
   if (!idx->has_data || idx->n_entries == 0) {
-    KMI_TRY((adopt_tmp<NW>(idx, tmp_keys, tmp_vals, kmer_off, nullptr, out_cnt, false, n, true)));
+    KMI_TRY((adopt_tmp<NW>(idx, tmp_keys, tmp_vals, kmer_off, nullptr, out_cnt, false, n, true, &ahead)));
     if (slack) sk_slack_report(fine_cnt, h_cnt, h_cap, lp, R);
     if (slack && *reinterpret_cast<const uint32_t *>(ctx->h_totals + H_SK_ROOM)) {
       KMI_TRY(kmi_index_clear(idx));
@@ -486,7 +518,7 @@
   }
   kmi_index scratch;
   scratch.ctx = ctx; scratch.cfg = idx->cfg; scratch.shape = idx->shape; scratch.val_words = 0; scratch.saturating = idx->saturating;
-  kmi_status st = adopt_tmp<NW>(&scratch, tmp_keys, tmp_vals, kmer_off, nullptr, out_cnt);
+  kmi_status st = adopt_tmp<NW>(&scratch, tmp_keys, tmp_vals, kmer_off, nullptr, out_cnt, false, 0, false, &ahead);
   if (st == KMI_OK) read_levels();
   if (st == KMI_OK && n) ctx->sk_inv_dup = (float)((double)scratch.n_entries / (double)n);
   if (st == KMI_OK && scratch.n_entries) {
@@ -502,7 +534,7 @@
   return st;
 }
 static kmi_status sk_back(kmi_index *idx, uint32_t w, const SkFront &f, uint32_t lp) {
-  return sk_dispatch_w(w, [&](auto W) { return sk_back_end<W>(idx, f.recs, f.n_records, f.h_cnt, f.h_base, f.wg_off, f.n_kmers, lp); });
+  return sk_dispatch_w(w, [&](auto W) { return sk_back_end<W>(idx, f.recs, f.n_records, f.h_cnt, f.h_base, f.wg_off, f.n_kmers, lp, false, f.back_ready); });
 }
 
 static kmi_status index_build_fused(kmi_index *idx, const uint8_t *bytes_dev, size_t n_bytes) {
diff --git a/kmerind_amd/csrc/kmi_sk_room.h b/kmerind_amd/csrc/kmi_sk_room.h
--- /dev/null
+++ b/kmerind_amd/csrc/kmi_sk_room.h
@@ -0,0 +1,30 @@
+#pragma once
+#include <stdint.h>
+
+#if defined(__HIPCC__)
+#define KMI_HD __host__ __device__
+#else
+#define KMI_HD
+#endif
+
+namespace kmi {
+
+KMI_HD inline uint64_t sk_room_x64(uint32_t m_len, uint32_t lp) {
+  const uint64_t room_m = m_len <= 11u ? 26u : (m_len == 12u ? 18u : 14u);
+  const uint64_t room_lp = lp == 0u ? 8u : (lp == 1u ? 10u : (lp == 2u ? 12u : 15u));
+  return room_m * room_lp;
+}
+KMI_HD inline uint64_t sk_fine_cap(uint64_t cnt, uint64_t room_x64, uint64_t sub) {
+  return ((cnt * room_x64 / 64 + sub - 1) / sub + 64 + 7) / 8 * 8;
+}
+KMI_HD inline uint64_t sk_region_records(uint64_t cnt, uint64_t room_x64, uint64_t sub) { return sk_fine_cap(cnt, room_x64, sub) * sub; }
+
+
+struct SkLayout {
+  const uint64_t *cnt = nullptr, *base = nullptr;
+  uint64_t *cend = nullptr, *region = nullptr;
+  uint32_t *cap = nullptr;
+  uint64_t room_x64 = 0;
+};
+
+}
diff --git a/kmerind_amd/csrc/kmi_superkmer.h b/kmerind_amd/csrc/kmi_superkmer.h
--- a/kmerind_amd/csrc/kmi_superkmer.h
+++ b/kmerind_amd/csrc/kmi_superkmer.h
@@ -1,4 +1,5 @@
 #pragma once
+#include "kmi_sk_room.h"
 
 namespace kmi {
 
@@ -434,7 +435,8 @@
                                                                                  const uint64_t *__restrict__ wg_off, const uint64_t *__restrict__ coarse_end,
                                                                                  uint32_t groups, const uint64_t *__restrict__ fine_region,
                                                                                  const uint32_t *__restrict__ fine_cap, uint32_t *__restrict__ fine_cnt,
-                                                                                 uint32_t *__restrict__ fine_kmers, uint32_t *__restrict__ flags) {
+                                                                                 uint32_t *__restrict__ fine_kmers, uint32_t *__restrict__ flags,
+                                                                                 unsigned long long *__restrict__ coarse_kmers ) {
   constexpr int NB = kSubPerCoarse, T = kSlackLT, PT = T / kPartThreads, SCAP = kSlackLCap, L = kSlackLineRecs, MAXG = SCAP / L + NB;
   static_assert(kPartThreads / NB == L && T % kPartThreads == 0, "one carry slot per thread: eight threads per bucket");
   __shared__ ulonglong2 s_stage[SCAP];
@@ -448,6 +450,7 @@
   __shared__ uint32_t s_part[NB / kWave];
   __shared__ uint32_t s_ng;
   __shared__ uint8_t s_linebkt[MAXG];
+  __shared__ unsigned long long s_ksum[NB / kWave];
   const uint32_t gpp = groups / kFineParts;
   const uint32_t c = blockIdx.x / kFineParts, h = blockIdx.x % kFineParts;
   const uint64_t b = wg_off[(uint64_t)(h * gpp) * kNumCoarse + c];
@@ -459,6 +462,7 @@
   const uint32_t cb = threadIdx.x / L, cj = threadIdx.x % L;
   ulonglong2 carry = make_ulonglong2(0, 0);
   uint32_t my_carry = 0;
+  unsigned long long my_km = 0;
   lds_barrier();
   const ulonglong2 *src = reinterpret_cast<const ulonglong2 *>(recs);
   ulonglong2 raw[PT];
@@ -503,6 +507,7 @@
       inc = wave_inclusive_sum_dpp(cnt | (ng << 16));
       if (lane_id() == kWave - 1) s_part[wave_id()] = inc;
       if (km) atomicAdd(&fine_kmers[c * NB + threadIdx.x], km);
+      my_km += km;
       s_dst[threadIdx.x] = emit ? take(threadIdx.x, emit) : ~0ull;
     }
     lds_barrier();
@@ -536,8 +541,18 @@
     lds_barrier();
   }
   {
-    if (threadIdx.x < NB) s_dst[threadIdx.x] = my_carry ? take(threadIdx.x, (uint32_t)L) : ~0ull;
-    lds_barrier();
+    if (threadIdx.x < NB) {
+      s_dst[threadIdx.x] = my_carry ? take(threadIdx.x, (uint32_t)L) : ~0ull;
+      const unsigned long long wk = wave_reduce_sum(my_km);
+      if (lane_id() == 0) s_ksum[wave_id()] = wk;
+    }
+    lds_barrier();
+    if (threadIdx.x == 0) {
+      unsigned long long wk = 0;
+#pragma unroll
+      for (int w = 0; w < NB / kWave; ++w) wk += s_ksum[w];
+      atomicAdd(&coarse_kmers[c], wk);
+    }
     const uint32_t rem = s_cnt[cb];
     const uint64_t d = s_dst[cb];
     if (rem && d != ~0ull) reinterpret_cast<ulonglong2 *>(out)[d + cj] = cj < rem ? carry : make_ulonglong2(kEmptyKey, kSkPadW1);
@@ -545,14 +560,26 @@
 }
 
 __global__ __launch_bounds__(1024) void sk_zero_kernel(uint32_t *__restrict__ a, uint32_t na, uint32_t *__restrict__ b, uint32_t nb,
-                                                     uint32_t *__restrict__ c, uint32_t nc, uint32_t *__restrict__ flags, uint32_t f0, uint32_t f1,
-                                                     uint32_t g0, uint32_t g1) {
+                                                     uint32_t *__restrict__ c, uint32_t nc, uint32_t *__restrict__ d, uint32_t nd,
+                                                     uint32_t *__restrict__ e, uint32_t ne, uint32_t *__restrict__ flags, uint32_t f0, uint32_t f1,
+                                                     uint32_t g0, uint32_t g1, uint32_t h0, uint32_t h1, SkLayout lay) {
   const uint32_t i = blockIdx.x * blockDim.x + threadIdx.x, stride = gridDim.x * blockDim.x;
   for (uint32_t x = i; x < na; x += stride) a[x] = 0;
   for (uint32_t x = i; x < nb; x += stride) b[x] = 0;
   for (uint32_t x = i; x < nc; x += stride) c[x] = 0;
+  for (uint32_t x = i; x < nd; x += stride) d[x] = 0;
+  for (uint32_t x = i; x < ne; x += stride) e[x] = 0;
   if (i >= f0 && i < f1) flags[i] = 0;
   if (i >= g0 && i < g1) flags[i] = 0;
+  if (i >= h0 && i < h1) flags[i] = 0;
+  if (blockIdx.x == 0 && lay.cnt) {
+    __shared__ uint64_t s_scan[1024 / 64 + 2];
+    const bool mine = threadIdx.x < (uint32_t)kNumCoarse;
+    const uint64_t n = mine ? lay.cnt[threadIdx.x] : 0ull;
+    const uint64_t cap = sk_fine_cap(n, lay.room_x64, (uint64_t)kSubPerCoarse);
+    const uint64_t at = block_exclusive_scan<uint64_t>(mine ? cap * kSubPerCoarse : 0ull, s_scan, (uint64_t *)nullptr);
+    if (mine) { lay.cend[threadIdx.x] = lay.base[threadIdx.x] + n; lay.cap[threadIdx.x] = (uint32_t)cap; lay.region[threadIdx.x] = at; }
+  }
 }
 
 __global__ __launch_bounds__(kPartThreads) void sk_recv_hist_kernel(const uint64_t *__restrict__ recs, uint64_t n, uint32_t *__restrict__ wg_hist,
```

Result: slower. 194.6 billion (-1.6%).
